# marian42/shapegan

Measured on AMD Instinct MI355X. Metric: GAN train steps/sec @32^3 voxels (train_wgan.py 5 critic + 1 generator updates, batch 64/GPU), higher is better.
Workload: dtype f32; 1 GPU; train_wgan.py 32^3 voxel WGAN, fp32, batch=64 synthetic SDF grids (BASELINE configs[1]); global_batch=64, per_gpu_batch=64, parallelism=dp1

## Files before the change

### include/shapegan_hip.h

```cpp
#ifndef SHAPEGAN_HIP_H
#define SHAPEGAN_HIP_H

#include <stddef.h>
#include <stdint.h>

#ifdef __cplusplus
extern "C" {
#endif

#define SG_ABI_VERSION 8

typedef struct ihipStream_t* hipStream_t;

#define SG_ACT_NONE_C 0
#define SG_ACT_LEAKY_C 1
#define SG_ACT_RELU_C 2
#define SG_ACT_TANH_C 3
#define SG_ACT_SIGMOID_C 4

int sg_abi_version(void);
const char* sg_last_error(void);

size_t sg_conv3d_k4s2p1_fwd_workspace_bytes(int batch, int Cin, int Cout, int OD, int OH, int OW);
int sg_conv3d_k4s2p1_fwd(const float* x, const float* w, const float* bias, float* y, int batch, int Cin, int Cin_total,
                         int Cx, int Cout, int ID, int IH, int IW, int act, float slope, void* workspace,
                         size_t workspace_bytes, hipStream_t stream);
int sg_conv3d_k4s2p1_fwd_keep(const float* x, const float* w, const float* bias, float* y, int batch, int Cin, int Cin_total,
                              int Cx, int Cout, int ID, int IH, int IW, int act, float slope, void* workspace,
                              size_t workspace_bytes, int weights_unchanged, hipStream_t stream);
long long sg_conv3d_k4s2p1_image_layout(int kind, const int* dims, size_t workspace_bytes);
int sg_conv3d_k4s2p1_pack_images(int n, const int* kinds, const float* const* weights, void* const* workspaces,
                                 const size_t* workspace_bytes, const int* dims, int* served, hipStream_t stream);
int sg_conv3d_k4s2p1_fwd_impl(const float* x, const float* w, const float* bias, float* y, int batch, int Cin,
                              int Cin_total, int Cx, int Cout, int ID, int IH, int IW, int act, float slope,
                              void* workspace, size_t workspace_bytes, int impl, int debug, hipStream_t stream);
size_t sg_conv3d_k4s2p1_dgrad_workspace_bytes(int Cout, int Cin);
size_t sg_conv3d_k4s2p1_dgrad_workspace_bytes_for(int batch, int Cin, int Cout, int OD, int OH, int OW);
int sg_conv3d_k4s2p1_dgrad(const float* dy, const float* w, const float* bias, float* dx, int batch, int Cin,
                           int Cin_total, int Cx, int Cout, int ID, int IH, int IW, int act, float slope,
                           void* workspace, size_t workspace_bytes, hipStream_t stream);
int sg_conv3d_k4s2p1_dgrad_keep(const float* dy, const float* w, const float* bias, float* dx, int batch, int Cin,
                                int Cin_total, int Cx, int Cout, int ID, int IH, int IW, int act, float slope,
                                void* workspace, size_t workspace_bytes, int weights_unchanged, hipStream_t stream);
int sg_conv3d_k4s2p1_dgrad_impl(const float* dy, const float* w, const float* bias, float* dx, int batch, int Cin,
                                int Cin_total, int Cx, int Cout, int ID, int IH, int IW, int act, float slope,
                                void* workspace, size_t workspace_bytes, int impl, hipStream_t stream);
#define SG_DGRAD_FORM_NONE 0
#define SG_DGRAD_FORM_DSKIP4 1
#define SG_DGRAD_FORM_ROWS32_4 2
#define SG_DGRAD_FORM_ROWS64_4 3
#define SG_DGRAD_FORM_ROWS32 4
#define SG_DGRAD_FORM_ROWS64 5
#define SG_DGRAD_FORM_DEPTH_WALK 6
int sg_conv3d_k4s2p1_dgrad_form(int batch, int Cin, int Cout, int OD, int OH, int OW, size_t workspace_bytes);
size_t sg_conv3d_k4s2p1_wgrad_workspace_bytes(int batch, int Cin, int Cout, int OD, int OH, int OW);
int sg_conv3d_k4s2p1_wgrad_impl(const float* dy, const float* x, float* dw, int batch, int Cin, int Cin_total, int Cx,
                                int Cout, int ID, int IH, int IW, void* workspace, size_t workspace_bytes, int impl,
                                hipStream_t stream);
int sg_conv3d_k4s2p1_wgrad(const float* dy, const float* x, float* dw, int batch, int Cin, int Cin_total, int Cx,
                           int Cout, int ID, int IH, int IW, void* workspace, size_t workspace_bytes,
                           hipStream_t stream);
int sg_conv3d_k4s2p1_wgrad_dy_image(int batch, int Cin, int Cout, int OD, int OH, int OW, size_t workspace_bytes, int* mt_total,
                                    long* nslice);
int sg_act_bwd_rowsum_pack8(const float* y, const float* dy, float* dz, float* rowsum, void* dz_image, long N, int C, long nslice,
                            int act, float slope, hipStream_t stream);
int sg_conv3d_k4s2p1_wgrad_prepacked(const float* dy, const float* x, float* dw, int batch, int Cin, int Cin_total, int Cx,
                                     int Cout, int ID, int IH, int IW, void* workspace, size_t workspace_bytes, hipStream_t stream);
int sg_conv3d_k4s2p1_wgrad_act_eligible(int batch, int Cin, int Cout, int OD, int OH, int OW, int act);
int sg_conv3d_k4s2p1_wgrad_act(const float* dy, const float* y, const float* x, float* dw, float* db, int batch, int Cin,
                               int Cin_total, int Cx, int Cout, int ID, int IH, int IW, int act, float slope, void* workspace,
                               size_t workspace_bytes, hipStream_t stream);

int sg_convT3d_k4s2p1_fwd(const float* x, const float* w, const float* bias, float* y, int batch, int Cin_T, int Cout_T,
                          int ID, int IH, int IW, int act, float slope, void* workspace, size_t workspace_bytes,
                          hipStream_t stream);
int sg_convT3d_k4s2p1_to1_pre_eligible(int batch, int C, int ID, int IH, int IW);
int sg_convT3d_k4s2p1_to1_pre(const float* x, const float* w, const float* bias, float* y, const float* in_scale,
                              const float* in_shift, int in_act, float in_slope, int batch, int C, int ID, int IH, int IW, int act,
                              float slope, hipStream_t stream);
int sg_convT3d_k4s2p1_to1_pre_impl(const float* x, const float* w, const float* bias, float* y, const float* in_scale,
                                   const float* in_shift, int in_act, float in_slope, int batch, int C, int ID, int IH, int IW,
                                   int act, float slope, int form, hipStream_t stream);
int sg_convT3d_k4s2p1_to1_pre_grouped(const float* x, const float* w, const float* bias, float* y, const float* in_scale,
                                      const float* in_shift, int in_act, float in_slope, int batch, int C, int ID, int IH, int IW,
                                      int act, float slope, int samples_per_group, long y_group_stride, hipStream_t stream);
int sg_convT3d_k4s2p1_dgrad(const float* dy, const float* w, float* dx, int batch, int Cin_T, int Cout_T, int ID, int IH,
                            int IW, void* workspace, size_t workspace_bytes, hipStream_t stream);
int sg_convT3d_k4s2p1_wgrad(const float* dy, const float* x, float* dw, int batch, int Cin_T, int Cout_T, int ID, int IH,
                            int IW, void* workspace, size_t workspace_bytes, hipStream_t stream);

size_t sg_gemm_workspace_bytes(int M, int N);
int sg_gemm(const float* A, long sai, long sak, const float* B, long sbk, long sbj, float* C, long sci, long scj,
            const float* bias_i, const float* bias_j, int bias_j_shift, int M, int N, int K, int act, float slope,
            void* workspace, size_t workspace_bytes, hipStream_t stream);
#define SG_GEMM_KIND_SKELETON 0
#define SG_GEMM_KIND_GEMM128 1
#define SG_GEMM_KIND_GEMM128_SPLIT 2
#define SG_GEMM_KIND_PERSISTENT 3
#define SG_GEMM_FINALIZE_NONE 0
#define SG_GEMM_FINALIZE_FLAT 1
#define SG_GEMM_FINALIZE_DEEP 2
int sg_gemm_plan(const void* A, long sai, long sak, const void* B, long sbk, long sbj, long sci, long scj, int has_bias_i, int M, int N,
                 int K, const void* workspace, size_t workspace_bytes, long* plan);
int sg_gemm_nt_plan(int batch, int M, int N, long K, long* plan);
size_t sg_gemm_nt_workspace_bytes(int M, int N, long K);
int sg_gemm_nt(const float* A, long lda, const float* B, long ldb, float* C, long ldc, int M, int N, long K, void* workspace,
               size_t workspace_bytes, hipStream_t stream);
size_t sg_gemm_nt_batched_workspace_bytes(int batch, int M, int N, long K);
int sg_gemm_nt_batched(const float* A, const long* a_off, long lda, const float* B, const long* b_off, long ldb, float* C,
                       const long* c_off, const long* ldc, int batch, int M, int N, long K, void* workspace,
                       size_t workspace_bytes, hipStream_t stream);
int sg_gemm_nt_batched_lnrelu(const float* A, const long* a_off, long lda, const float* B, const long* b_off, long ldb,
                              const float* gamma, const float* beta, const long* g_off, float* C, const long* c_off, const long* ldc,
                              int batch, int M, int N, long K, void* workspace, size_t workspace_bytes, hipStream_t stream);
int sg_colsum(const float* x, float* out, int rows, int cols, long ld, hipStream_t stream);
int sg_rowsum(const float* x, float* out, long rows, long len, long ld, hipStream_t stream);
int sg_rowsum_multi(const float* x, float* const* outs, const long* out_strides, int ndst, long rows_per_dst, long len, long ld,
                    hipStream_t stream);
int sg_segsum(const float* x, float* out, long rows, long ld, const int64_t* seg_off, long nseg, hipStream_t stream);

size_t sg_bn_workspace_bytes(int C);
int sg_bn_plan(int N, int C, long S, int* nsplit, int* napply);
int sg_bn_train_fwd(const float* x, const float* gamma, const float* beta, float* y, float* save_mean, float* save_invstd,
                    float* running_mean, float* running_var, long long* num_batches_tracked, int N, int C, long S,
                    float eps, float momentum, int act, float slope, void* workspace, size_t workspace_bytes,
                    hipStream_t stream);
int sg_bn_train_stats(const float* x, const float* gamma, const float* beta, float* save_mean, float* save_invstd,
                      float* running_mean, float* running_var, long long* num_batches_tracked, float* scale, float* shift, int N,
                      int C, long S, float eps, float momentum, void* workspace, size_t workspace_bytes, hipStream_t stream);
int sg_bn_train_fwd_grouped(const float* x, const float* gamma, const float* beta, float* y, float* save_mean, float* save_invstd,
                            float* running_mean, float* running_var, long long* num_batches_tracked, int groups, int N, int C,
                            long S, float eps, float momentum, int act, float slope, void* workspace, size_t workspace_bytes,
                            hipStream_t stream);
int sg_bn_train_stats_grouped(const float* x, const float* gamma, const float* beta, float* save_mean, float* save_invstd,
                              float* running_mean, float* running_var, long long* num_batches_tracked, float* scale, float* shift,
                              int groups, int N, int C, long S, float eps, float momentum, void* workspace, size_t workspace_bytes,
                              hipStream_t stream);
int sg_bn_eval_fwd(const float* x, const float* gamma, const float* beta, float* y, const float* running_mean,
                   const float* running_var, float* save_mean, float* save_invstd, int N, int C, long S, float eps,
                   int act, float slope, hipStream_t stream);
int sg_bn_bwd(const float* dy, const float* x, const float* gamma, const float* beta, const float* save_mean,
              const float* save_invstd, float* dx, float* dgamma, float* dbeta, int N, int C, long S, int train, int act,
              float slope, void* workspace, size_t workspace_bytes, hipStream_t stream);

int sg_act_fwd(const float* x, float* y, long n, int act, float slope, hipStream_t stream);
int sg_act_bwd(const float* y, const float* dy, float* dx, long n, int act, float slope, hipStream_t stream);
int sg_act_bwd_rowsum(const float* y, const float* dy, float* dx, float* rowsum, long rows, long S, int act, float slope,
                      hipStream_t stream);

size_t sg_sdfnet_packed_floats(int kin_used);
size_t sg_sdfnet_acts_floats(long ldn);
int sg_sdfnet_pack(const float* const* params, int latent, int kin_used, float* packed, hipStream_t stream);
int sg_sdfnet_fwd(const float* points, long points_period, const float* latent, const int64_t* latent_idx,
                  int latent_size, const float* packed, int kin_used, const float* zb1, const float* zb5,
                  long points_per_shape, const int* shape_index, float* out, float* acts, long ldn, long N,
                  hipStream_t stream);
long sg_sdfnet_bwd_blocks(long N);
long sg_sdfnet_bwd_tile_start(long N, long t);
#define SG_SDFNET_PARTIAL_ROW 3616
#define SG_SDFGEN_PARTIAL_ROW 7200
int sg_sdfnet_bwd(const float* dout, const float* out, const float* acts, float* dz, float* dz8, float* bias_partials,
                  const float* points, long points_period, float* dx, long dx_ld, const float* packed, int kin_used, long ldn,
                  long N, hipStream_t stream);
int sg_sdfnet_shape_bias(const float* z, long nshapes, int latent, const float* W1, const float* b1, const float* W5, const float* b5,
                         float* zb1, float* zb5, hipStream_t stream);
int sg_sdfnet_pack_shape_bias(const float* const* params, int latent, float* packed, const float* z, long nshapes, float* zb1,
                              float* zb5, hipStream_t stream);
int sg_sdfnet_shape_bias_bwd(const float* t1, const float* t5, long nshapes, const float* z, int latent, const float* W1,
                             const float* W5, float* dW1, float* dW5, float* gz, const float* reg_weight, float reg_scale,
                             hipStream_t stream);
size_t sg_sdfnet_bwd_finish_workspace_bytes(long N);
int sg_sdfnet_bwd_finish(const float* dz, const float* bias_partials, long ldn, long N, int extended, float* const* bias_grads,
                         float* w8_grad, float* b8_grad, float* w1_cols, long w1_ld, float* w5_cols, long w5_ld,
                         const int64_t* seg_off, long nseg, float* t1, float* t5, void* workspace, size_t workspace_bytes,
                         unsigned* tickets, hipStream_t stream);

#ifndef SG_SDFNET_LATENT_TILE
#define SG_SDFNET_LATENT_TILE 32
#endif
#define SG_SDFNET_LATENT_PARTIAL_ROW 513
int sg_sdfnet_latent_grad(const float* points, const float* target, const int64_t* seg_off, long nshapes, const float* zb1,
                          const float* zb5, const float* packed, float cutoff, long win_start, long win_count, const int* tiles,
                          long ntiles, float* partials, hipStream_t stream);
int sg_sdfnet_latent_reduce(const float* partials, const int64_t* tile_off, const int64_t* seg_off, long nshapes, long win_count,
                            float* t1, float* t5, float* loss, hipStream_t stream);

#define SG_SDFNET_POSE_PARTIAL_ROW 528
int sg_sdfnet_latent_pose_grad(const float* points, const float* target, const int64_t* seg_off, long nshapes, const float* zb1,
                               const float* zb5, const float* packed, const float* pose, float cutoff, long win_start,
                               long win_count, const int* tiles, long ntiles, float* partials, hipStream_t stream);
int sg_sdfnet_latent_pose_reduce(const float* partials, const int64_t* tile_off, const int64_t* seg_off, long nshapes,
                                 long win_count, float* t1, float* t5, float* loss, float* gpose, hipStream_t stream);

#define SG_SDFNET_PROJECT_TILE 32
int sg_sdfnet_project(const float* points, const int64_t* seg_off, long nshapes, const float* zb1, const float* zb5,
                      const float* packed, float level, int iterations, int rule, float max_step, const int* tiles, long ntiles,
                      float* out_points, float* value, float* grad, hipStream_t stream);

size_t sg_sdfgen_acts_floats(long ldn);
long sg_sdfgen_packed_norm_offset(int which);
int sg_sdfgen_pack(const float* const* params, const float* const* norm_params, float* packed, hipStream_t stream);
int sg_sdfgen_fwd(const float* points, const float* packed, const float* zb1, const float* zb5, long points_per_shape,
                  const int* shape_index, float eps, float* out, float* acts, long ldn, long N, hipStream_t stream);
long sg_sdfgen_bwd_blocks(long N);
int sg_sdfgen_bwd(const float* dout, const float* acts, float* dz, float* dz8, float* partials, const float* points,
                  const float* packed, long ldn, long N, hipStream_t stream);
size_t sg_sdfgen_bwd_finish_workspace_bytes(long N);
int sg_sdfgen_bwd_finish(const float* dz, const float* partials, long ldn, long N, float* const* bias_grads, float* w8_grad,
                         float* b8_grad, float* w1_cols, long w1_ld, float* w5_cols, long w5_ld, float* const* norm_grads,
                         const int64_t* seg_off, long nseg, float* t1, float* t5, void* workspace, size_t workspace_bytes,
                         unsigned* tickets, hipStream_t stream);

int sg_axpby(const float* x, const float* y, float* out, long n, float a, float b, hipStream_t stream);
size_t sg_reduce_workspace_bytes(void);
int sg_reduce_sum(const float* x, float* out, long n, float scale, void* workspace, size_t workspace_bytes,
                  hipStream_t stream);
int sg_gather_rows(const float* table, const int64_t* idx, float* out, long n, int L, hipStream_t stream);
int sg_scatter_add_rows(const float* rows, long rows_ld, const int64_t* idx, float* table_grad, long n, int L,
                        hipStream_t stream);
int sg_sdf_batch_sort_max_shapes(void);
size_t sg_sdf_batch_sort_workspace_bytes(long n, long nshapes);
int sg_sdf_batch_sort(const int64_t* indices, long n, long pointcloud_size, long nshapes, const float* points,
                      const float* sdf, float* out_points, float* out_sdf, int* out_shape, int64_t* seg_off, float* counts,
                      int* bad_index_flag, int* bad_index_device, int bad_index_value, void* workspace, size_t workspace_bytes,
// ... 304 lines not shown
```

### shapegan_amd/csrc/conv3d.hip

```cpp
#include "mfma_tile.h"
#include <stdlib.h>

#include "conv_common.h"
#include "../../include/shapegan_hip.h"

namespace sg {

struct PatchCtx {
    int base;
    int mask;
    __device__ __forceinline__ void set(const ConvGeom& g, uint32_t pos) {
        int n, od, oh, ow;
        decode_pos(g, pos, n, od, oh, ow);
        const int id0 = 2 * od - 1, ih0 = 2 * oh - 1, iw0 = 2 * ow - 1;
        base = n * g.Cx * g.ID * g.IH * g.IW + (id0 * g.IH + ih0) * g.IW + iw0;
        int m = 0;
#pragma unroll
        for (int t = 0; t < 4; ++t) {
            if ((unsigned)(id0 + t) < (unsigned)g.ID) m |= 1 << t;
            if ((unsigned)(ih0 + t) < (unsigned)g.IH) m |= 1 << (4 + t);
            if ((unsigned)(iw0 + t) < (unsigned)g.IW) m |= 1 << (8 + t);
        }
        mask = m;
    }
// ... 659 lines not shown

static bool kept_image_of_call(int kind, int batch, int Cin, int Cout, const ConvGeom& g, size_t workspace_bytes, ImageJob* image) {
    if (kind == 0) {
        const HaloFwdPlan p = halo_fwd_plan(batch, Cin, Cout, g, workspace_bytes);
        *image = p.image;
        return p.served;
    }
    const HaloDgradPlan p = halo_dgrad_plan(batch, Cin, Cout, g, workspace_bytes);
    *image = p.image;
    return p.served;
}

int sg_conv3d_k4s2p1_pack_images(int n, const int* kinds, const float* const* weights, void* const* workspaces,
                                 const size_t* workspace_bytes, const int* dims, int* served, hipStream_t stream) {
    SG_CHECK_ARG(n > 0 && n <= 8 && kinds && weights && workspaces && workspace_bytes && dims && served);
    PackJobs jobs;
    for (int i = 0; i < n; ++i) {
        const int* d = dims + 8 * i;
        const int batch = d[0], Cin = d[1], Cin_total = d[2], Cx = d[3], Cout = d[4];
        served[i] = 0;
        SG_CHECK_ARG(weights[i] && batch > 0 && Cin > 0 && Cin <= Cin_total && Cin <= Cx && Cout > 0 && (kinds[i] == 0 || kinds[i] == 1));
        ConvGeom g;
        if (make_geom(g, d[5], d[6], d[7], Cx, Cout)) SG_FAIL(SG_ERR_ARG, "sg_conv3d_k4s2p1_pack_images: bad spatial dims");
        if (check_sizes(g, batch, "sg_conv3d_k4s2p1_pack_images")) return SG_ERR_ARG;
        ImageJob image;
        if (!kept_image_of_call(kinds[i], batch, Cin, Cout, g, workspaces[i] ? workspace_bytes[i] : 0, &image)) continue;
        served[i] = jobs.add(image, weights[i], workspaces[i], Cout, Cin_total, Cin);
    }
    halo_pack_jobs_launch(jobs, stream);
    SG_CHECK_LAUNCH();
    return SG_OK;
}

long long sg_conv3d_k4s2p1_image_layout(int kind, const int* dims, size_t workspace_bytes) {
    if (!dims || (kind != 0 && kind != 1)) return 0;
    const int batch = dims[0], Cin = dims[1], Cin_total = dims[2], Cx = dims[3], Cout = dims[4];
    if (batch <= 0 || Cin <= 1 || Cin > Cin_total || Cin > Cx || Cout <= 0) return 0;
    ConvGeom g;
    if (make_geom(g, dims[5], dims[6], dims[7], Cx, Cout)) return 0;
    if ((long)batch * g.O3() >= (1L << 31) || (long)batch * g.I3() >= (1L << 31)) return 0;
    ImageJob j;
    if (!kept_image_of_call(kind, batch, Cin, Cout, g, workspace_bytes, &j)) return 0;
    unsigned long long h = 1469598103934665603ull;
    const long long f[7] = {j.kind + 1, Cout, Cin_total, Cin, j.nt, (long long)j.offset, 0x5347};
    for (long long v : f)
        for (int b = 0; b < 8; ++b) {
            h ^= (unsigned long long)(v >> (8 * b)) & 0xffull;
            h *= 1099511628211ull;
        }
    h &= 0x7fffffffffffffffull;
    return h ? (long long)h : 1;
}

int sg_conv3d_k4s2p1_dgrad_form(int batch, int Cin, int Cout, int OD, int OH, int OW, size_t workspace_bytes) {
    static_assert((int)HaloDgradKernel::dskip4 + 1 == SG_DGRAD_FORM_DSKIP4 && (int)HaloDgradKernel::rows32_4 + 1 == SG_DGRAD_FORM_ROWS32_4 &&
                  (int)HaloDgradKernel::rows64_4 + 1 == SG_DGRAD_FORM_ROWS64_4 && (int)HaloDgradKernel::rows32 + 1 == SG_DGRAD_FORM_ROWS32 &&
                  (int)HaloDgradKernel::rows64 + 1 == SG_DGRAD_FORM_ROWS64 && (int)HaloDgradKernel::rows64_dwalk + 1 == SG_DGRAD_FORM_DEPTH_WALK,
                  "SG_DGRAD_FORM_* mirror HaloDgradKernel");
    ConvGeom g;
    if (batch <= 0 || Cin <= 1 || Cout <= 0 || !query_geom(g, Cin, Cout, OD, OH, OW)) return SG_DGRAD_FORM_NONE;
    if ((long)batch * g.O3() >= (1L << 31) || (long)batch * g.I3() >= (1L << 31)) return SG_DGRAD_FORM_NONE;
    if (edge_dgrad_plan(batch, Cin, Cout, g, workspace_bytes).served) return SG_DGRAD_FORM_NONE;
    const HaloDgradPlan hp = halo_dgrad_plan(batch, Cin, Cout, g, workspace_bytes);
    return hp.served ? 1 + (int)hp.kernel : SG_DGRAD_FORM_NONE;
}

int sg_conv3d_k4s2p1_dgrad_impl(const float* dy, const float* w, const float* bias, float* dx, int batch, int Cin,
                                int Cin_total, int Cx, int Cout, int ID, int IH, int IW, int act, float slope,
                                void* workspace, size_t workspace_bytes, int impl, hipStream_t stream) {
    HaloDgradForm form;
    SG_CHECK_ARG(dy && w && dx && batch > 0 && Cin > 0 && Cin <= Cin_total && Cin <= Cx && Cout > 0 &&
                 halo_dgrad_form_decode(impl, &form) && form.forced &&
                 (form.ppw == 0 || (!form.one_parity && (form.ppw == 2 || form.ppw == 4 || form.ppw == 8))));
    ConvGeom g;
    if (make_geom(g, ID, IH, IW, Cx, Cout)) SG_FAIL(SG_ERR_ARG, "sg_conv3d_k4s2p1_dgrad_impl: bad spatial dims");
    if (check_sizes(g, batch, "sg_conv3d_k4s2p1_dgrad_impl")) return SG_ERR_ARG;
    const HaloDgradPlan hp = halo_dgrad_plan(batch, Cin, Cout, g, workspace ? workspace_bytes : 0, form);
    if (!hp.served) SG_FAIL(SG_ERR_ARG, "sg_conv3d_k4s2p1_dgrad_impl: shape not eligible for the LDS-halo kernel");
    halo_dgrad_pack(hp, w, Cin, Cin_total, Cout, workspace, stream);
    halo_dgrad_launch(hp, dy, bias, dx, batch, Cin, Cout, g, act, slope, workspace, stream);
    SG_CHECK_LAUNCH();
    return SG_OK;
}

int sg_conv3d_k4s2p1_wgrad_impl(const float* dy, const float* x, float* dw, int batch, int Cin, int Cin_total, int Cx,
                                int Cout, int ID, int IH, int IW, void* workspace, size_t workspace_bytes, int impl,
                                hipStream_t stream) {
    SG_CHECK_ARG(dy && x && dw && batch > 0 && Cin > 0 && Cin <= Cin_total && Cin <= Cx && Cout > 0 && impl == 1);
    ConvGeom g;
    if (make_geom(g, ID, IH, IW, Cx, Cout)) SG_FAIL(SG_ERR_ARG, "sg_conv3d_k4s2p1_wgrad_impl: bad spatial dims");
    if (check_sizes(g, batch, "sg_conv3d_k4s2p1_wgrad_impl")) return SG_ERR_ARG;
    const HaloWgradPlan hp = halo_wgrad_plan(batch, Cin, Cout, g, workspace ? workspace_bytes : 0, true);
    if (!hp.served) SG_FAIL(SG_ERR_ARG, "sg_conv3d_k4s2p1_wgrad_impl: shape not eligible for the LDS-halo kernel");
    halo_wgrad_pack(hp, dy, Cout, g, workspace, stream);
    halo_wgrad_launch(hp, x, dw, Cin, Cin_total, Cout, g, workspace, stream);
    SG_CHECK_LAUNCH();
    return SG_OK;
}

int sg_conv3d_k4s2p1_wgrad_dy_image(int batch, int Cin, int Cout, int OD, int OH, int OW, size_t workspace_bytes, int* mt_total,
                                    long* nslice) {
    if (batch <= 0 || Cin <= 0 || Cout <= 0 || !mt_total || !nslice) return 0;
    ConvGeom g;
    if (make_geom(g, 2 * OD, 2 * OH, 2 * OW, Cin, Cout)) return 0;
    const HaloWgradPlan hp = halo_wgrad_plan(batch, Cin, Cout, g, workspace_bytes, false);
    if (!hp.producer_image) return 0;
    *mt_total = hp.dy_image.nt;
    *nslice = hp.nslice;
    return 1;
}
int sg_act_bwd_rowsum_pack8(const float* y, const float* dy, float* dz, float* rowsum, void* dz_image, long N, int C, long nslice,
                            int act, float slope, hipStream_t stream) {
    SG_CHECK_ARG(y && dy && dz && rowsum && dz_image && N > 0 && C > 0 && C % 128 == 0 && nslice == N * 8);
    SG_CHECK_ARG(act == SG_ACT_LEAKY || act == SG_ACT_RELU);
    SG_CHECK_ARG((((uintptr_t)y | (uintptr_t)dy | (uintptr_t)dz | (uintptr_t)dz_image) & 15) == 0);
    halo_act_bwd_pack8_launch(y, dy, dz, rowsum, dz_image, N * C, C, nslice, act, slope, stream);
    SG_CHECK_LAUNCH();
    return SG_OK;
}
int sg_conv3d_k4s2p1_wgrad_prepacked(const float* dy, const float* x, float* dw, int batch, int Cin, int Cin_total, int Cx,
                                     int Cout, int ID, int IH, int IW, void* workspace, size_t workspace_bytes, hipStream_t stream) {
    SG_CHECK_ARG(dy && x && dw && batch > 0 && Cin > 0 && Cin <= Cin_total && Cin <= Cx && Cout > 0);
    ConvGeom g;
    if (make_geom(g, ID, IH, IW, Cx, Cout)) SG_FAIL(SG_ERR_ARG, "sg_conv3d_k4s2p1_wgrad_prepacked: bad spatial dims");
    if (check_sizes(g, batch, "sg_conv3d_k4s2p1_wgrad_prepacked")) return SG_ERR_ARG;
    const HaloWgradPlan hp = halo_wgrad_plan(batch, Cin, Cout, g, workspace ? workspace_bytes : 0, false);
    if (!hp.producer_image)
        SG_FAIL(SG_ERR_ARG, "sg_conv3d_k4s2p1_wgrad_prepacked: this call is not served with a producer-written image");
    halo_wgrad_launch(hp, x, dw, Cin, Cin_total, Cout, g, workspace, stream);
    SG_CHECK_LAUNCH();
    return SG_OK;
}

int sg_conv3d_k4s2p1_wgrad_act_eligible(int batch, int Cin, int Cout, int OD, int OH, int OW, int act) {
    ConvGeom g;
    return batch > 0 && act != SG_ACT_NONE && query_geom(g, 1, Cout, OD, OH, OW) &&
           edge_wgrad_plan(batch, Cin, Cout, g, kAnyWorkspace, act).served;
}
int sg_conv3d_k4s2p1_wgrad_act(const float* dy, const float* y, const float* x, float* dw, float* db, int batch, int Cin,
                               int Cin_total, int Cx, int Cout, int ID, int IH, int IW, int act, float slope, void* workspace,
                               size_t workspace_bytes, hipStream_t stream) {
    SG_CHECK_ARG(dy && y && x && dw && db && batch > 0 && Cin > 0 && Cin <= Cin_total && Cin <= Cx && Cout > 0);
    ConvGeom g;
    if (make_geom(g, ID, IH, IW, Cx, Cout)) SG_FAIL(SG_ERR_ARG, "sg_conv3d_k4s2p1_wgrad_act: spatial dims must be even and >= 2");
    if (check_sizes(g, batch, "sg_conv3d_k4s2p1_wgrad_act")) return SG_ERR_ARG;
    const EdgeWgradPlan ep = edge_wgrad_plan(batch, Cin, Cout, g, workspace ? workspace_bytes : 0, act);
    if (act == SG_ACT_NONE || !ep.served)
        SG_FAIL(SG_ERR_ARG, "sg_conv3d_k4s2p1_wgrad_act: shape not served (see sg_conv3d_k4s2p1_wgrad_act_eligible) or workspace too small");
    edge_wgrad_launch(ep, dy, y, x, dw, db, batch, Cin_total, Cout, g, slope, workspace, stream);
    SG_CHECK_LAUNCH();
    return SG_OK;
}

int sg_conv3d_k4s2p1_wgrad(const float* dy, const float* x, float* dw, int batch, int Cin, int Cin_total, int Cx,
                           int Cout, int ID, int IH, int IW, void* workspace, size_t workspace_bytes,
                           hipStream_t stream) {
    SG_CHECK_ARG(dy && x && dw && batch > 0 && Cin > 0 && Cin <= Cin_total && Cin <= Cx && Cout > 0);
    ConvGeom g;
    if (make_geom(g, ID, IH, IW, Cx, Cout)) SG_FAIL(SG_ERR_ARG, "sg_conv3d_k4s2p1_wgrad: spatial dims must be even and >= 2");
    if (check_sizes(g, batch, "sg_conv3d_k4s2p1_wgrad")) return SG_ERR_ARG;
    const long npos = (long)batch * g.O3();
    const EdgeWgradPlan ep = edge_wgrad_plan(batch, Cin, Cout, g, workspace ? workspace_bytes : 0, 0);
    if (ep.served) {
        edge_wgrad_launch(ep, dy, nullptr, x, dw, nullptr, batch, Cin_total, Cout, g, 0.f, workspace, stream);
        SG_CHECK_LAUNCH();
        return SG_OK;
    }
    const HaloWgradPlan hp = halo_wgrad_plan(batch, Cin, Cout, g, workspace ? workspace_bytes : 0, false);
    if (hp.served) {
        halo_wgrad_pack(hp, dy, Cout, g, workspace, stream);
        halo_wgrad_launch(hp, x, dw, Cin, Cin_total, Cout, g, workspace, stream);
        SG_CHECK_LAUNCH();
        return SG_OK;
    }
    WgradDyLoader la;
    la.dy = dy;
    la.O3 = (int)g.O3();
    la.Cy = Cout;
    la.dO3 = FastDiv((uint32_t)g.O3());
    WgradPatchLoader lb;
    lb.x = x;
    lb.g = g;
    WgradEpi epi{dw, (long)Cin_total * 64};
    launch_tile_gemm(la, lb, epi, Cout, Cin * 64, (int)npos, (float*)workspace, workspace ? workspace_bytes : 0, stream);
    SG_CHECK_LAUNCH();
    return SG_OK;
}

int sg_convT3d_k4s2p1_fwd(const float* x, const float* w, const float* bias, float* y, int batch, int Cin_T, int Cout_T,
                          int ID, int IH, int IW, int act, float slope, void* workspace, size_t workspace_bytes,
                          hipStream_t stream) {
    return sg_conv3d_k4s2p1_dgrad(x, w, bias, y, batch, Cout_T, Cout_T, Cout_T, Cin_T, 2 * ID, 2 * IH, 2 * IW, act,
                                  slope, workspace, workspace_bytes, stream);
}
int sg_convT3d_k4s2p1_to1_pre_eligible(int batch, int C, int ID, int IH, int IW) {
    ConvGeom g;
    return batch > 0 && C > 0 && query_geom(g, 1, C, ID, IH, IW) && (long)batch * g.I3() < (1L << 31) &&
           edge_dgrad_walk_plan(0, batch, 1, C, g).served;
}
static int convT_to1_pre(const float* x, const float* w, const float* bias, float* y, const float* in_scale,
                         const float* in_shift, int in_act, float in_slope, int batch, int C, int ID, int IH, int IW,
                         int act, float slope, int samples_per_group, long y_group_stride, int form, hipStream_t stream) {
    SG_CHECK_ARG(x && w && y && in_scale && in_shift && samples_per_group > 0 && batch % samples_per_group == 0 && form >= 0 && form <= 8);
    SG_CHECK_ARG(y_group_stride >= (long)samples_per_group * 8 * ID * IH * IW);
    if (!sg_convT3d_k4s2p1_to1_pre_eligible(batch, C, ID, IH, IW))
        SG_FAIL(SG_ERR_ARG, "sg_convT3d_k4s2p1_to1_pre: shape not served (C <= 64, IH * IW <= 256)");
    SG_CHECK_ARG(in_act == SG_ACT_NONE || in_act == SG_ACT_RELU || (in_act == SG_ACT_LEAKY && in_slope >= 0.f && in_slope <= 1.f));
    ConvGeom g;
    if (make_geom(g, 2 * ID, 2 * IH, 2 * IW, 1, C)) SG_FAIL(SG_ERR_ARG, "sg_convT3d_k4s2p1_to1_pre: bad spatial dims");
    if (form == 3 || form == 4)
        SG_FAIL(SG_ERR_ARG, "sg_convT3d_k4s2p1_to1_pre_impl: forms 3 and 4 (both h parities per workgroup) were retired");
    const EdgeDgradPlan ep = edge_dgrad_walk_plan(form, batch, 1, C, g);
    if (!ep.served) SG_FAIL(SG_ERR_ARG, "sg_convT3d_k4s2p1_to1_pre: not served");
    edge_dgrad_launch(ep, x, w, bias, y, batch, 1, C, g, act, slope, nullptr, stream, in_scale, in_shift, in_act, in_slope,
                      samples_per_group, y_group_stride);
    SG_CHECK_LAUNCH();
    return SG_OK;
}
int sg_convT3d_k4s2p1_to1_pre_grouped(const float* x, const float* w, const float* bias, float* y, const float* in_scale,
                                      const float* in_shift, int in_act, float in_slope, int batch, int C, int ID, int IH, int IW,
                                      int act, float slope, int samples_per_group, long y_group_stride, hipStream_t stream) {
    return convT_to1_pre(x, w, bias, y, in_scale, in_shift, in_act, in_slope, batch, C, ID, IH, IW, act, slope, samples_per_group,
                         y_group_stride, 0, stream);
}
int sg_convT3d_k4s2p1_to1_pre_impl(const float* x, const float* w, const float* bias, float* y, const float* in_scale,
                                   const float* in_shift, int in_act, float in_slope, int batch, int C, int ID, int IH, int IW,
                                   int act, float slope, int form, hipStream_t stream) {
    return convT_to1_pre(x, w, bias, y, in_scale, in_shift, in_act, in_slope, batch, C, ID, IH, IW, act, slope, batch,
                         (long)batch * 8 * ID * IH * IW, form, stream);
}
int sg_convT3d_k4s2p1_to1_pre(const float* x, const float* w, const float* bias, float* y, const float* in_scale,
                              const float* in_shift, int in_act, float in_slope, int batch, int C, int ID, int IH, int IW, int act,
                              float slope, hipStream_t stream) {
    return sg_convT3d_k4s2p1_to1_pre_grouped(x, w, bias, y, in_scale, in_shift, in_act, in_slope, batch, C, ID, IH, IW, act, slope,
                                             batch, (long)batch * 8 * ID * IH * IW, stream);
}
int sg_convT3d_k4s2p1_dgrad(const float* dy, const float* w, float* dx, int batch, int Cin_T, int Cout_T, int ID, int IH,
                            int IW, void* workspace, size_t workspace_bytes, hipStream_t stream) {
    return sg_conv3d_k4s2p1_fwd(dy, w, nullptr, dx, batch, Cout_T, Cout_T, Cout_T, Cin_T, 2 * ID, 2 * IH, 2 * IW,
                                SG_ACT_NONE, 0.f, workspace, workspace_bytes, stream);
}
int sg_convT3d_k4s2p1_wgrad(const float* dy, const float* x, float* dw, int batch, int Cin_T, int Cout_T, int ID, int IH,
                            int IW, void* workspace, size_t workspace_bytes, hipStream_t stream) {
    return sg_conv3d_k4s2p1_wgrad(x, dy, dw, batch, Cout_T, Cout_T, Cout_T, Cin_T, 2 * ID, 2 * IH, 2 * IW, workspace,
                                  workspace_bytes, stream);
}

}
```

### shapegan_amd/csrc/conv3d_edge.hip

```cpp
#include <stdlib.h>

#include "conv_common.h"
#include "../../include/shapegan_hip.h"

namespace sg {

struct EdgeFwdArgs {
    const float* x;
    const float* w;
    const float* bias;
    float* y;
    int OD, OH, OW, IH, IW, Cout, Cy, Cin_total;
    long x_sample;
    int tiles_per_sample, total_tiles;
    FastDiv dtps, dOW, dOH;
    int act;
    float slope;
};

__device__ __forceinline__ void buf_store4(__amdgpu_buffer_rsrc_t r, unsigned voff, unsigned soff, float x, float y, float z,
                                           float w) {
    typedef unsigned u32x4 __attribute__((ext_vector_type(4)));
    u32x4 v;
    v.x = __builtin_bit_cast(unsigned, x);
// ... 45 lines not shown
            wfr[nt][g][1] = wl[co * kWL + g * 4 + kw1];
        }
    }
    const __amdgpu_buffer_rsrc_t xres = make_rsrc(a.x - ((long)a.IH * a.IW + a.IW));
    const __amdgpu_buffer_rsrc_t yres = make_rsrc(a.y);
    const unsigned O3 = (unsigned)(a.OD * a.OH * a.OW);
    unsigned soff[16];
#pragma unroll
    for (int g = 0; g < 16; ++g) soff[g] = (unsigned)(((g >> 2) * a.IH + (g & 3)) * a.IW) * 4u;

    const int nwaves = gridDim.x * 4;
    const int per_wave = (a.total_tiles + nwaves - 1) / nwaves;
    int t = (blockIdx.x * 4 + wave) * per_wave;
    const int t_end = min(a.total_tiles, t + per_wave);
    if (t >= t_end) return;

    struct TileLane {
        unsigned o0, o1;
        bool d0, d3, h0, h3;
    };
    auto lane_offsets = [&](int tile, TileLane& L, unsigned (&yoff)[1]) __attribute__((always_inline)) {
        uint32_t n, tp, q1, ow, oh, od;
        a.dtps.divmod((uint32_t)tile, n, tp);
        const uint32_t p = tp * 32 + r;
        a.dOW.divmod(p, q1, ow);
        a.dOH.divmod(q1, od, oh);
        const unsigned base = (unsigned)((long)n * a.x_sample + ((long)(2 * od) * a.IH + 2 * oh) * a.IW + 2 * ow) * 4u;
        const bool left = ow == 0, right = (int)ow == a.OW - 1;
        L.o0 = kh2 ? (right ? kBufOutside : base + 8u) : base;
        L.o1 = kh2 ? (left ? kBufOutside : base - 4u) : base + 4u;
        L.d0 = od == 0;
        L.d3 = (int)od == a.OD - 1;
        L.h0 = oh == 0;
        L.h3 = (int)oh == a.OH - 1;
        yoff[0] = (unsigned)(((long)n * a.Cy + (lane >> 3)) * O3 + tp * 32 + 4 * (lane & 7)) * 4u;
    };
    auto load_patch = [&](const TileLane& L, float (&b0)[16], float (&b1)[16]) __attribute__((always_inline)) {
#pragma unroll
        for (int g = 0; g < 16; ++g) {
            const int kd = g >> 2, kh = g & 3;
            bool out = false;
            if (kd == 0) out = out || L.d0;
            if (kd == 3) out = out || L.d3;
            if (kh == 0) out = out || L.h0;
            if (kh == 3) out = out || L.h3;
            b0[g] = buf_load(xres, out ? kBufOutside : L.o0, soff[g]);
            b1[g] = buf_load(xres, out ? kBufOutside : L.o1, soff[g]);
        }
    };
    TileLane L;
    unsigned yoff[1];
    lane_offsets(t, L, yoff);
    float* const tw = tl[wave];
    float c0[16], c1[16];
    load_patch(L, c0, c1);

    float pv[NT][16];
    unsigned yprev = kBufOutside;
    auto epilogue_slice = [&](int sl) __attribute__((always_inline)) {
        if (sl < NT * 4) {
            const int nt = sl >> 2, c = sl & 3;
            f32x4 v = {pv[nt][4 * c], pv[nt][4 * c + 1], pv[nt][4 * c + 2], pv[nt][4 * c + 3]};
            v = v + bl[nt];
            if (ACT == 1) {
                const f32x4 sv = v * a.slope;
                v = __builtin_elementwise_max(v, sv);
            } else if (ACT == 2) {
#pragma unroll
                for (int i = 0; i < 4; ++i) v[i] = sg_apply_act(v[i], a.act, a.slope);
            }
            *reinterpret_cast<f32x4*>(tw + (nt * 32 + r) * kTL + 8 * c + 4 * kh2) = v;
        } else if (sl >= 8 && sl < 8 + NT * 4) {
            const int i = sl - 8;
            const int row = 8 * i + (lane >> 3);
            const f32x4 v = *reinterpret_cast<const f32x4*>(tw + row * kTL + 4 * (lane & 7));
            buf_store4(yres, row < a.Cout && !(SG_FWDC1_ABL & 1) ? yprev : kBufOutside, (unsigned)(8 * i) * O3 * 4u, v[0], v[1], v[2], v[3]);
        }
    };
    auto tile_mfma = [&](auto with_epilogue, const float (&c0)[16], const float (&c1)[16]) __attribute__((always_inline)) {
        f32x16 acc[NT];
#pragma unroll
        for (int nt = 0; nt < NT; ++nt)
#pragma unroll
            for (int q = 0; q < 16; ++q) acc[nt][q] = 0.f;
#pragma unroll
        for (int g = 0; g < 16; ++g) {
            if (SG_FWDC1_ABL & 2) {
#pragma unroll
                for (int nt = 0; nt < NT; ++nt) acc[nt][g] += c0[g] * wfr[nt][g][0] + c1[g] * wfr[nt][g][1];
            } else {
#pragma unroll
                for (int nt = 0; nt < NT; ++nt) acc[nt] = __builtin_amdgcn_mfma_f32_32x32x2f32(c0[g], wfr[nt][g][0], acc[nt], 0, 0, 0);
#pragma unroll
                for (int nt = 0; nt < NT; ++nt) acc[nt] = __builtin_amdgcn_mfma_f32_32x32x2f32(c1[g], wfr[nt][g][1], acc[nt], 0, 0, 0);
            }
            if (decltype(with_epilogue)::value) {
                __builtin_amdgcn_sched_barrier(0);
                epilogue_slice(g);
                __builtin_amdgcn_sched_barrier(0);
            }
        }
#pragma unroll
        for (int nt = 0; nt < NT; ++nt)
#pragma unroll
            for (int q = 0; q < 16; ++q) pv[nt][q] = acc[nt][q];
    };
    auto advance = [&](int tcur, float (&n0)[16], float (&n1)[16]) __attribute__((always_inline)) {
        TileLane Ln;
        unsigned yn[1];
        lane_offsets(tcur + 1 < t_end ? tcur + 1 : tcur, Ln, yn);
        if (tcur + 1 >= t_end || (SG_FWDC1_ABL & 4)) Ln.o0 = Ln.o1 = kBufOutside;
        load_patch(Ln, n0, n1);
        yprev = yoff[0];
        L = Ln;
        yoff[0] = yn[0];
    };
    auto tile_step = [&](int tt, auto with_epilogue, const float (&c0)[16], const float (&c1)[16], float (&n0)[16],
                         float (&n1)[16]) __attribute__((always_inline)) {
        const unsigned ydone = yprev;
        advance(tt, n0, n1);
        const unsigned ynext = yprev;
        yprev = ydone;
        __builtin_amdgcn_sched_barrier(0);
        tile_mfma(with_epilogue, c0, c1);
        yprev = ynext;
    };
    float d0[16], d1[16];
    tile_step(t, IntTag<0>(), c0, c1, d0, d1);
    for (++t; t < t_end; t += 2) {
        tile_step(t, IntTag<1>(), d0, d1, c0, c1);
        if (t + 1 < t_end) tile_step(t + 1, IntTag<1>(), c0, c1, d0, d1);
    }
#pragma unroll
    for (int sl = 0; sl < 16; ++sl) epilogue_slice(sl);
}

template <int IWT>
struct FwdLds {
    static constexpr int OWT = IWT / 2, BH = 256 / OWT, R = 2 * BH + 2, RS = IWT + 8, PLANE = R * RS, BUF = 4 * PLANE;
    static constexpr int PW = IWT / 4, PIECES = 4 * R * PW, NP = (PIECES + 255) / 256;
    static constexpr int TILE_ROWS = IWT == 32 ? 4 : 2;
};
struct EdgeFwdLdsArgs {
    const float* x;
    const float* w;
    const float* bias;
    float* y;
    int OD, OH, IH, Cout, Cy, Cin_total;
    long x_sample;
    int units, units_per_wg, blocks_per_plane;
    FastDiv dbpp, dOD;
    int act;
    float slope;
};

template <int NT, int ACT, int IWT>
__global__ void __launch_bounds__(256) conv_fwd_c1_lds_kernel(EdgeFwdLdsArgs a) {
    using G = FwdLds<IWT>;
    constexpr int kWL = 65, kTL = 36;
    __shared__ __attribute__((aligned(16))) float xs[2 * G::BUF];
    __shared__ __attribute__((aligned(16))) float tl[4][32 * kTL];
    const int tid = threadIdx.x, lane = tid & 63, wave = tid >> 6;
    const int r = lane & 31, kh2 = lane >> 5;
    int u = blockIdx.x * a.units_per_wg;
    const int u_end = min(a.units, u + a.units_per_wg);
    if (u >= u_end) return;
    const __amdgpu_buffer_rsrc_t xres = make_rsrc(a.x - ((long)a.IH * IWT + IWT));
    const __amdgpu_buffer_rsrc_t yres = make_rsrc(a.y);
    unsigned pword[G::NP];
    lds_f32x4* pdst[G::NP];
#pragma unroll
    for (int f = 0; f < G::NP; ++f) {
        const int e = tid + 256 * f;
        const int p = e / (G::R * G::PW), rem = e - p * (G::R * G::PW), rr = rem / G::PW, c4 = rem - rr * G::PW;
        const unsigned cls = e >= G::PIECES ? 16u : ((p == 0 ? 1u : 0u) | (p == 3 ? 2u : 0u) | (rr == 0 ? 4u : 0u) | (rr == G::R - 1 ? 8u : 0u));
        pword[f] = (unsigned)(((p * a.IH + rr) * IWT + 4 * c4) * 4) | (cls << 26);
        pdst[f] = (lds_f32x4*)((lds_float*)xs + (e >= G::PIECES ? 0 : p * G::PLANE + rr * G::RS + 4 + 4 * c4));
    }
    const unsigned O3 = (unsigned)(a.OD * a.OH * G::OWT);
    f32x4 sv[G::NP];
    unsigned ybase = 0;
    auto stage_issue = [&](int uu, bool real) __attribute__((always_inline)) {
        uint32_t q, ohb, n, od;
        a.dbpp.divmod((uint32_t)uu, q, ohb);
        a.dOD.divmod(q, n, od);
        const unsigned mask = 0x03ffffffu | ((16u | (od == 0 ? 1u : 0u) | ((int)od == a.OD - 1 ? 2u : 0u) | (ohb == 0 ? 4u : 0u) |
                                              ((int)ohb == a.blocks_per_plane - 1 ? 8u : 0u)) << 26);
        const unsigned sbase = (unsigned)(((long)n * a.x_sample + ((long)(2 * od) * a.IH + 2 * ohb * G::BH) * IWT) * 4);
#pragma unroll
        for (int f = 0; f < G::NP; ++f) {
            const unsigned t = pword[f] & mask;
            sv[f] = buf_load4v(xres, (!real || (t >> 26) || (SG_FWDC1_ABL & 4)) ? kBufOutside : t, sbase);
        }
    };
    stage_issue(u, true);
    {
        float* wl = xs;
        const __amdgpu_buffer_rsrc_t wres = make_rsrc(a.w);
        f32x4 wv[NT * 2];
#pragma unroll
        for (int i = 0; i < NT * 2; ++i) {
            const int e4 = tid + 256 * i, co = e4 >> 4, t4 = e4 & 15;
            wv[i] = buf_load4v(wres, co < a.Cout ? (unsigned)(((long)co * a.Cin_total * 64 + t4 * 4) * 4) : kBufOutside, 0);
        }
#pragma unroll
        for (int i = 0; i < NT * 2; ++i) {
            const int e4 = tid + 256 * i, co = e4 >> 4, t4 = e4 & 15;
#pragma unroll
            for (int j = 0; j < 4; ++j) wl[co * kWL + t4 * 4 + j] = wv[i][j];
        }
    }
    __syncthreads();
    float wfr[NT][16][2], bl[NT];
#pragma unroll
    for (int nt = 0; nt < NT; ++nt) {
        const int co = nt * 32 + r;
        bl[nt] = (a.bias && co < a.Cout) ? a.bias[co] : 0.f;
#pragma unroll
        for (int g = 0; g < 16; ++g) {
            wfr[nt][g][0] = xs[co * kWL + g * 4 + 2 * kh2];
            wfr[nt][g][1] = xs[co * kWL + g * 4 + 2 * kh2 + 1];
        }
    }
    __syncthreads();
    for (int e = tid; e < 2 * 4 * G::R * 2; e += 256) {
        const int row = e >> 1;
        xs[row * G::RS + ((e & 1) ? 4 + IWT : 3)] = 0.f;
    }
    auto stage_write = [&](int buf) __attribute__((always_inline)) {
#pragma unroll
        for (int f = 0; f < G::NP; ++f)
            if (f + 1 < G::NP || tid < G::PIECES - 256 * (G::NP - 1)) pdst[f][buf * (G::BUF / 4)] = sv[f];
    };
    auto unit_ybase = [&](int uu) __attribute__((always_inline)) {
        uint32_t q, ohb, n, od;
        a.dbpp.divmod((uint32_t)uu, q, ohb);
        a.dOD.divmod(q, n, od);
        return (unsigned)(((long)n * a.Cy * O3 + ((long)od * a.OH + ohb * G::BH) * G::OWT) * 4);
    };
    const int oh_in = IWT == 32 ? 2 * (r >> 4) : 0, ow = IWT == 32 ? (r & 15) : r;
    const lds_float* const abase = (const lds_float*)xs + (2 * wave * G::TILE_ROWS + oh_in) * G::RS + 3 + 2 * ow + 2 * kh2;
    const unsigned ylane = (unsigned)(((lane >> 3) * O3 + 64 * wave + 4 * (lane & 7)) * 4);
    float* const tw = tl[wave];

    float pv[NT][16];
    unsigned yprev = kBufOutside;
    auto epilogue_slice = [&](int sl) __attribute__((always_inline)) {
        const int nt = sl >> 3, k = sl & 7;
        if (nt >= NT) return;
        if (k < 4) {
            f32x4 v = {pv[nt][4 * k], pv[nt][4 * k + 1], pv[nt][4 * k + 2], pv[nt][4 * k + 3]};
            v = v + bl[nt];
            if (ACT == 1) {
                const f32x4 sv2 = v * a.slope;
                v = __builtin_elementwise_max(v, sv2);
            } else if (ACT == 2) {
#pragma unroll
                for (int i = 0; i < 4; ++i) v[i] = sg_apply_act(v[i], a.act, a.slope);
            }
            *reinterpret_cast<f32x4*>(tw + r * kTL + 8 * k + 4 * kh2) = v;
        } else {
            const int i = k - 4;
            const int row = nt * 32 + 8 * i + (lane >> 3);
            const f32x4 v = *reinterpret_cast<const f32x4*>(tw + (8 * i + (lane >> 3)) * kTL + 4 * (lane & 7));
            buf_store4(yres, row < a.Cout && !(SG_FWDC1_ABL & 1) ? yprev : kBufOutside, (unsigned)(nt * 32 + 8 * i) * O3 * 4u, v[0], v[1], v[2], v[3]);
        }
    };
    auto tile = [&](auto with_epilogue, int buf, int j) __attribute__((always_inline)) {
        const lds_float* ap = abase + buf * G::BUF + j * G::TILE_ROWS * G::RS;
        float ca[3], cb[3];
#pragma unroll
        for (int g = 0; g < 2; ++g) {
            ca[g] = ap[(g >> 2) * G::PLANE + (g & 3) * G::RS];
            cb[g] = ap[(g >> 2) * G::PLANE + (g & 3) * G::RS + 1];
        }
        f32x16 acc[NT];
#pragma unroll
        for (int nt = 0; nt < NT; ++nt)
#pragma unroll
            for (int q = 0; q < 16; ++q) acc[nt][q] = 0.f;
#pragma unroll
        for (int g = 0; g < 16; ++g) {
            if (g + 2 < 16) {
                ca[(g + 2) % 3] = ap[((g + 2) >> 2) * G::PLANE + ((g + 2) & 3) * G::RS];
                cb[(g + 2) % 3] = ap[((g + 2) >> 2) * G::PLANE + ((g + 2) & 3) * G::RS + 1];
            }
            __builtin_amdgcn_sched_barrier(0);
            if (SG_FWDC1_ABL & 2) {
#pragma unroll
                for (int nt = 0; nt < NT; ++nt) acc[nt][g] += ca[g % 3] * wfr[nt][g][0] + cb[g % 3] * wfr[nt][g][1];
            } else {
#pragma unroll
                for (int nt = 0; nt < NT; ++nt) acc[nt] = __builtin_amdgcn_mfma_f32_32x32x2f32(ca[g % 3], wfr[nt][g][0], acc[nt], 0, 0, 0);
#pragma unroll
                for (int nt = 0; nt < NT; ++nt) acc[nt] = __builtin_amdgcn_mfma_f32_32x32x2f32(cb[g % 3], wfr[nt][g][1], acc[nt], 0, 0, 0);
            }
            if (decltype(with_epilogue)::value) {
                __builtin_amdgcn_sched_barrier(0);
                epilogue_slice(g);
                __builtin_amdgcn_sched_barrier(0);
            }
        }
#pragma unroll
        for (int nt = 0; nt < NT; ++nt)
#pragma unroll
            for (int q = 0; q < 16; ++q) pv[nt][q] = acc[nt][q];
    };

    stage_write(0);
    __syncthreads();
    int buf = 0;
    ybase = unit_ybase(u);
    stage_issue(u + 1, u + 1 < u_end);
    tile(IntTag<0>(), buf, 0);
    yprev = ybase + ylane;
    tile(IntTag<1>(), buf, 1);
    yprev = ybase + ylane + 128u;
    stage_write(buf ^ 1);
    __syncthreads();
    for (++u; u < u_end; ++u) {
        buf ^= 1;
        ybase = unit_ybase(u);
        stage_issue(u + 1, u + 1 < u_end);
        tile(IntTag<1>(), buf, 0);
        yprev = ybase + ylane;
        tile(IntTag<1>(), buf, 1);
        yprev = ybase + ylane + 128u;
        stage_write(buf ^ 1);
        __syncthreads();
    }
#pragma unroll
    for (int sl = 0; sl < 16; ++sl) epilogue_slice(sl);
}

constexpr int kEdgePartial = 4096 + 64;
struct EdgeWgradArgs {
    const float* dy;
    const float* y;
    float slope;
    const float* x;
    float* partial;
    int OD, OH, OW, IH, IW, Cout, Cy;
    long x_sample;
    int passes_per_sample, total_passes;
    FastDiv dpps, dOW16, dOH;
};

#ifndef SG_WGRAD_C1_WAVES
#define SG_WGRAD_C1_WAVES 1
#endif
template <int MT, int FUSE>
__global__ void __launch_bounds__(256, SG_WGRAD_C1_WAVES) conv_wgrad_c1_kernel(EdgeWgradArgs a) {
    constexpr int kLd = 36;
    constexpr int kStage = MT * 32 * kLd;
    __shared__ __attribute__((aligned(16))) float lds[4 * 4096];
    const int lane = threadIdx.x & 63, wave = threadIdx.x >> 6;
    const int r = lane & 31, kh2 = lane >> 5;
    const __amdgpu_buffer_rsrc_t dres = make_rsrc(a.dy);
    const __amdgpu_buffer_rsrc_t yres = make_rsrc(FUSE ? a.y : a.dy);
    const __amdgpu_buffer_rsrc_t xres = make_rsrc(a.x - ((long)a.IH * a.IW + a.IW + 1));
    const unsigned O3 = (unsigned)(a.OD * a.OH * a.OW);
    float* stage = lds + wave * kStage;
    __shared__ float bsh[4][64];
    const int crow = lane >> 3, ccol = (lane & 7) * 4;
    unsigned tapoff[2];
#pragma unroll
    for (int nt = 0; nt < 2; ++nt) {
        const int tap = nt * 32 + r, kd = tap >> 4, kh = (tap >> 2) & 3, kw = tap & 3;
        tapoff[nt] = (unsigned)((kd * a.IH + kh) * a.IW + kw) * 4u;
    }
    const int lkh = (r >> 2) & 3, lkw = r & 3, lkd0 = r >> 4;
    const int nseg = a.OW >> 4;
    f32x16 acc[MT][2];
#pragma unroll
    for (int mt = 0; mt < MT; ++mt)
#pragma unroll
        for (int nt = 0; nt < 2; ++nt)
#pragma unroll
            for (int q = 0; q < 16; ++q) acc[mt][nt][q] = 0.f;

    const int nwaves = gridDim.x * 4;
    f32x4 cv[MT * 4];
    f32x4 yv[FUSE ? MT * 4 : 1];
    float rs[MT * 4];
#pragma unroll
    for (int i = 0; i < MT * 4; ++i) rs[i] = 0.f;
    float bv[2][16];
    unsigned xo[2], xl[2], xr[2];
    auto issue_dy = [&](int ps, bool valid) __attribute__((always_inline)) {
        uint32_t n, pp;
        a.dpps.divmod((uint32_t)(valid ? ps : 0), n, pp);
        const unsigned dbase = (unsigned)((long)n * a.Cy * O3 + pp * 32 + ccol) * 4u;
        unsigned inval = valid ? 0u : kBufOutside;
        asm volatile("" : "+v"(inval));
#pragma unroll
        for (int i = 0; i < MT * 4; ++i) {
            const int co = i * 8 + crow;
            const unsigned off = (co < a.Cout ? dbase + (unsigned)co * O3 * 4u : kBufOutside) | inval;
            cv[i] = buf_load4v(dres, off, 0);
            if (FUSE) yv[i] = buf_load4v(yres, off, 0);
        }
    };
    auto plan_x = [&](int ps, bool valid) __attribute__((always_inline)) {
        uint32_t n, pp, seg, q1, od, oh;
        a.dpps.divmod((uint32_t)ps, n, pp);
        const uint32_t p0 = pp * 32 + 16 * kh2;
        a.dOW16.divmod(p0 >> 4, q1, seg);
        a.dOH.divmod(q1, od, oh);
        const unsigned xbase = (unsigned)((long)n * a.x_sample + ((long)(2 * od) * a.IH + 2 * oh) * a.IW + 32 * seg) * 4u;
        const bool hout = !valid || (lkh == 0 && oh == 0) || (lkh == 3 && (int)oh == a.OH - 1);
#pragma unroll
        for (int nt = 0; nt < 2; ++nt) {
            const int kd = 2 * nt + lkd0;
            const bool out = hout || (kd == 0 && od == 0) || (kd == 3 && (int)od == a.OD - 1);
            xo[nt] = out ? kBufOutside : xbase + tapoff[nt];
            xl[nt] = (lkw == 0 && seg == 0) ? kBufOutside : xo[nt];
            xr[nt] = (lkw == 3 && (int)seg == nseg - 1) ? kBufOutside : xo[nt];
        }
    };
    auto load_x = [&](int j) __attribute__((always_inline)) {
#pragma unroll
        for (int nt = 0; nt < 2; ++nt) bv[nt][j] = buf_load(xres, j == 0 ? xl[nt] : (j == 15 ? xr[nt] : xo[nt]), 8u * j);
    };
    int ps = blockIdx.x * 4 + wave;
    if (ps < a.total_passes) {
        issue_dy(ps, true);
        plan_x(ps, true);
#pragma unroll
        for (int j = 0; j < 16; ++j) load_x(j);
    }
    for (; ps < a.total_passes; ps += nwaves) {
        if (FUSE) {
            const float neg = FUSE == SG_ACT_LEAKY ? a.slope : 0.f;
#pragma unroll
            for (int i = 0; i < MT * 4; ++i) {
#pragma unroll
                for (int j = 0; j < 4; ++j) cv[i][j] = yv[i][j] > 0.f ? cv[i][j] : cv[i][j] * neg;
                rs[i] += (cv[i][0] + cv[i][1]) + (cv[i][2] + cv[i][3]);
            }
        }
#pragma unroll
        for (int i = 0; i < MT * 4; ++i) *reinterpret_cast<f32x4*>(stage + (i * 8 + crow) * kLd + ccol) = cv[i];
        const bool more = ps + nwaves < a.total_passes;
        issue_dy(ps + nwaves, more);
        plan_x(more ? ps + nwaves : ps, more);
        f32x4 avc[MT], avn[MT];
#pragma unroll
        for (int mt = 0; mt < MT; ++mt) avc[mt] = *reinterpret_cast<const f32x4*>(stage + (mt * 32 + r) * kLd + 16 * kh2);
        __builtin_amdgcn_sched_barrier(0);
#pragma unroll
        for (int c = 0; c < 4; ++c) {
            if (c < 3) {
#pragma unroll
                for (int mt = 0; mt < MT; ++mt)
                    avn[mt] = *reinterpret_cast<const f32x4*>(stage + (mt * 32 + r) * kLd + 16 * kh2 + 4 * (c + 1));
            }
#pragma unroll
            for (int jj = 0; jj < 4; ++jj) {
                const int j = 4 * c + jj;
#pragma unroll
                for (int mt = 0; mt < MT; ++mt)
#pragma unroll
                    for (int nt = 0; nt < 2; ++nt)
                        acc[mt][nt] = __builtin_amdgcn_mfma_f32_32x32x2f32(avc[mt][jj], bv[nt][j], acc[mt][nt], 0, 0, 0);
                load_x(j);
            }
#pragma unroll
            for (int mt = 0; mt < MT; ++mt) avc[mt] = avn[mt];
        }
        __builtin_amdgcn_sched_barrier(0);
    }
    __syncthreads();
#pragma unroll
    for (int mt = 0; mt < MT; ++mt)
#pragma unroll
        for (int nt = 0; nt < 2; ++nt)
#pragma unroll
            for (int q = 0; q < 16; ++q) {
                const int row = mt * 32 + (q & 3) + 8 * (q >> 2) + 4 * kh2;
                lds[wave * 4096 + row * 64 + nt * 32 + r] = acc[mt][nt][q];
            }
    if (FUSE) {
#pragma unroll
        for (int i = 0; i < MT * 4; ++i) {
            float v = rs[i];
            v += __builtin_bit_cast(float, __builtin_amdgcn_update_dpp(0, __builtin_bit_cast(int, v), 0xB1, 0xf, 0xf, false));
            v += __builtin_bit_cast(float, __builtin_amdgcn_update_dpp(0, __builtin_bit_cast(int, v), 0x4E, 0xf, 0xf, false));
            v += __builtin_bit_cast(float, __builtin_amdgcn_update_dpp(0, __builtin_bit_cast(int, v), 0x141, 0xf, 0xf, false));
            if ((lane & 7) == 0) bsh[wave][i * 8 + crow] = v;
        }
    }
    __syncthreads();
    float* out = a.partial + (long)blockIdx.x * kEdgePartial;
    for (int e = threadIdx.x; e < MT * 32 * 64; e += 256)
        out[e] = (lds[e] + lds[4096 + e]) + (lds[2 * 4096 + e] + lds[3 * 4096 + e]);
    if (FUSE && threadIdx.x < MT * 32) out[4096 + threadIdx.x] = (bsh[0][threadIdx.x] + bsh[1][threadIdx.x]) + (bsh[2][threadIdx.x] + bsh[3][threadIdx.x]);
}

__global__ void __launch_bounds__(256) wgrad_c1_finalize_kernel(const float* __restrict__ partial, float* __restrict__ dw,
                                                                int nparts, int Cout, int Cin_total, float* __restrict__ db) {
    __shared__ float red[16][17];
    const int o = threadIdx.x & 15, grp = threadIdx.x >> 4;
    const int e = blockIdx.x * 16 + o;
    float s[8];
#pragma unroll
    for (int u = 0; u < 8; ++u) s[u] = 0.f;
    for (int p0 = grp; p0 < nparts; p0 += 128) {
#pragma unroll
        for (int u = 0; u < 8; ++u) {
            const int p = p0 + 16 * u;
            s[u] += p < nparts ? partial[(long)p * kEdgePartial + e] : 0.f;
        }
    }
    red[grp][o] = ((s[0] + s[1]) + (s[2] + s[3])) + ((s[4] + s[5]) + (s[6] + s[7]));
    __syncthreads();
    if (grp == 0) {
        float t = 0.f;
#pragma unroll
        for (int g2 = 0; g2 < 16; ++g2) t += red[g2][o];
        const int co = e >> 6, tap = e & 63;
        if (e >= 4096) {
            if (e - 4096 < Cout) db[e - 4096] = t;
        } else if (co < Cout) {
            dw[((long)co * Cin_total) * 64 + tap] = t;
        }
    }
}

struct TapPlaneArgs {
    const float* dy;
    const float* w;
    float* S;
    int Cout, Cy, Cin_total;
    unsigned O3;
    int tiles_per_sample, total_tiles;
    FastDiv dtps;
};

template <int NS>
__global__ void __launch_bounds__(256) tapplane_gemm_kernel(TapPlaneArgs a) {
    const int lane = threadIdx.x & 63, wave = threadIdx.x >> 6;
    const int r = lane & 31, kh2 = lane >> 5;
    float wfr[2][NS];
#pragma unroll
    for (int s = 0; s < NS; ++s) {
        const int co = 2 * s + kh2, coc = co < a.Cout ? co : a.Cout - 1;
        const float keep = co < a.Cout ? 1.f : 0.f;
#pragma unroll
        for (int nt = 0; nt < 2; ++nt) wfr[nt][s] = keep * a.w[(long)coc * a.Cin_total * 64 + nt * 32 + r];
    }
    const __amdgpu_buffer_rsrc_t dres = make_rsrc(a.dy);
    const __amdgpu_buffer_rsrc_t sres = make_rsrc(a.S);
    const int nwaves = gridDim.x * 4;
    for (int t = blockIdx.x * 4 + wave; t < a.total_tiles; t += nwaves) {
        uint32_t n, tp;
        a.dtps.divmod((uint32_t)t, n, tp);
        const unsigned doff = (unsigned)(((long)n * a.Cy + kh2) * a.O3 + tp * 32 + r) * 4u;
        float av[NS];
#pragma unroll
        for (int s = 0; s < NS; ++s) av[s] = buf_load(dres, 2 * s + kh2 < a.Cout ? doff : kBufOutside, (unsigned)(2 * s) * a.O3 * 4u);
        f32x16 acc[2];
#pragma unroll
        for (int nt = 0; nt < 2; ++nt)
#pragma unroll
            for (int q = 0; q < 16; ++q) acc[nt][q] = 0.f;
#pragma unroll
        for (int s = 0; s < NS; ++s) {
            acc[0] = __builtin_amdgcn_mfma_f32_32x32x2f32(av[s], wfr[0][s], acc[0], 0, 0, 0);
            acc[1] = __builtin_amdgcn_mfma_f32_32x32x2f32(av[s], wfr[1][s], acc[1], 0, 0, 0);
        }
        const unsigned soff = (unsigned)(((long)n * 64 + r) * a.O3 + tp * 32 + 4 * kh2) * 4u;
#pragma unroll
        for (int nt = 0; nt < 2; ++nt)
#pragma unroll
            for (int c = 0; c < 4; ++c)
                buf_store4(sres, soff, (unsigned)(nt * 32) * a.O3 * 4u + 32u * c, acc[nt][4 * c], acc[nt][4 * c + 1],
                           acc[nt][4 * c + 2], acc[nt][4 * c + 3]);
    }
}

__global__ void __launch_bounds__(256) col2im_c1_kernel(const float* __restrict__ S, const float* __restrict__ bias,
                                                        float* __restrict__ dx, ConvGeom g, long dx_sample, int total, int act,
                                                        float slope) {
    const int j = blockIdx.x * 256 + threadIdx.x;
    if (j >= total) return;
    int n, qd, qh, qw;
    decode_pos(g, (uint32_t)j, n, qd, qh, qw);
    const int OHW = g.OH * g.OW;
    const long O3 = (long)g.OD * OHW;
    const float* Sn = S + (long)n * 64 * O3;
// ... 430 lines not shown
        const __amdgpu_buffer_rsrc_t sres = make_rsrc(PRE ? a.in_scale + grow : a.w), hres = make_rsrc(PRE ? a.in_shift + grow : a.w);
        unsigned wtap[4];
#pragma unroll
        for (int set = 0; set < 4; ++set) {
            const int pd = set >> 1, ph = set & 1;
            const int kd = g2 == 0 ? (pd == 0 ? 1 : 2) : (pd == 0 ? 3 : 0);
            const int kh = khi == 0 ? (ph == 0 ? 1 : 2) : (ph == 0 ? 3 : 0);
            wtap[set] = (unsigned)(kd * 16 + kh * 4 + kw) * 4u;
        }
        const unsigned wrow = (unsigned)a.Cin_total * 256u;
#pragma unroll
        for (int s = 0; s < 16; ++s) {
            const int co = 4 * s + kq;
            const bool have = s < nks && co < a.Cout;
#pragma unroll
            for (int set = 0; set < 4; ++set) wfr[set][s] = buf_load(wres, have ? (unsigned)co * wrow + wtap[set] : kBufOutside, 0);
            if (PRE) {
                psc[s] = buf_load(sres, have ? (unsigned)co * 4u : kBufOutside, 0);
                psh[s] = buf_load(hres, have ? (unsigned)co * 4u : kBufOutside, 0);
            }
        }
    }
    const int q = tid >> 1, pw = tid & 1;
    const int qh = q / OW, qw = q - qh * OW;
    const bool gather_on = q < P2;
    const int dw = pw == 0 ? -1 : 1;
    const int kp_same = pw == 0 ? 0 : 2, kp_nb = pw == 0 ? 1 : 3;
    const bool col_nb = (unsigned)(qw + dw) < (unsigned)OW;
    const int qc = gather_on ? q : 0;
    const int qcol = col_nb ? dw : 0;
    int goff[2][4];
    float gmul[2][4];
#pragma unroll
    for (int ph = 0; ph < 2; ++ph) {
        const int dh = ph == 0 ? -1 : 1;
        const bool row_nb = (unsigned)(qh + dh) < (unsigned)OH;
        const int qrow = row_nb ? dh * OW : 0;
        const int base = ph * 16 * stride;
        goff[ph][0] = base + (0 + kp_same) * stride + convT_slot(qc);
        goff[ph][1] = base + (0 + kp_nb) * stride + convT_slot(qc + qcol);
        goff[ph][2] = base + (4 + kp_same) * stride + convT_slot(qc + qrow);
        goff[ph][3] = base + (4 + kp_nb) * stride + convT_slot(qc + qrow + qcol);
        gmul[ph][0] = 1.f;
        gmul[ph][1] = col_nb ? 1.f : 0.f;
        gmul[ph][2] = row_nb ? 1.f : 0.f;
        gmul[ph][3] = (row_nb && col_nb) ? 1.f : 0.f;
    }
    const float b0 = a.bias ? a.bias[0] : 0.f;
    const int IH = 2 * OH, IW = 2 * OW;
    const __amdgpu_buffer_rsrc_t ores = make_rsrc(a.dx + (long)(n / a.spg) * a.out_group_stride + (long)(n % a.spg) * a.dx_sample);
    const unsigned ovoff = gather_on ? (unsigned)((2 * qh) * IW + 2 * qw + pw) * 4u : kBufOutside;
    const unsigned oplane = (unsigned)(IH * IW) * 4u;
    float carry[2][2] = {{0.f, 0.f}, {0.f, 0.f}};
    float etc[2][4], etf[2][4], eval[2] = {0.f, 0.f};
    auto epi_read = [&](int p, int pd) __attribute__((always_inline)) {
        const lds_float* pb = Sl + ((p & 1) * 64 + pd * 32) * stride;
#pragma unroll
        for (int ph = 0; ph < 2; ++ph)
#pragma unroll
            for (int g = 0; g < 4; ++g) {
                etc[ph][g] = pb[goff[ph][g]];
                etf[ph][g] = pb[goff[ph][g] + 8 * stride];
            }
    };
    auto epi_sum = [&](int pd) __attribute__((always_inline)) {
#pragma unroll
        for (int ph = 0; ph < 2; ++ph)
            eval[ph] = convT_out_act<EPI>(convT_tap_sum(etc[ph], etf[ph], gmul[ph], pd, carry[pd][ph], b0), a.act, a.slope);
    };
    auto epi_store = [&](int p, int pd) __attribute__((always_inline)) {
        const bool skip = p == qs && (pd == 1 || qs > 0);
#pragma unroll
        for (int ph = 0; ph < 2; ++ph)
            __builtin_amdgcn_raw_buffer_store_b32(__builtin_bit_cast(unsigned, eval[ph]), ores, (int)(skip ? kBufOutside : ovoff),
                                                  (int)((unsigned)(2 * p - pd) * oplane + (unsigned)(ph * IW) * 4u), 0);
    };

    auto plane = [&](int qd, auto with_epi, float (&cur)[2][16], float (&nxt)[2][16]) __attribute__((always_inline)) {
        lds_float* const buf = Sl + (qd & 1) * 64 * stride;
        f32x4v c4[2][4];
#pragma unroll
        for (int t = 0; t < 2; ++t)
#pragma unroll
            for (int set = 0; set < 4; ++set) c4[t][set] = f32x4v{0.f, 0.f, 0.f, 0.f};
#pragma unroll
        for (int s = 0; s < 16; ++s) {
            if (decltype(with_epi)::value && s == 1) {
                __syncthreads();
                __builtin_amdgcn_sched_barrier(0);
            }
            load_step(qd + 1, s, nxt);
            if (decltype(with_epi)::value) {
                if (s == 1) epi_read(qd - 1, 0);
                if (s == 3) epi_sum(0);
                if (s == 5) {
                    epi_store(qd - 1, 0);
                    epi_read(qd - 1, 1);
                }
                if (s == 7) epi_sum(1);
                if (s == 9) epi_store(qd - 1, 1);
            }
#pragma unroll
            for (int t = 0; t < 2; ++t) {
                float v = cur[t][s];
                if (PRE) {
                    v = fmaf(v, psc[s], psh[s]);
                    v = fmaxf(v, v * a.in_slope);
                }
#pragma unroll
                for (int set = 0; set < 4; ++set) c4[t][set] = __builtin_amdgcn_mfma_f32_16x16x4f32(v, wfr[set][s], c4[t][set], 0, 0, 0);
            }
            __builtin_amdgcn_sched_group_barrier(0x020, 1, 0);
#pragma unroll
            for (int i = 0; i < 8; ++i) {
                __builtin_amdgcn_sched_group_barrier(0x096, SG_CONVT_ALL_ILV, 0);
                __builtin_amdgcn_sched_group_barrier(0x008, 1, 0);
            }
            __builtin_amdgcn_sched_barrier(0);
        }
        if (FULL || block_on) {
#pragma unroll
            for (int t = 0; t < 2; ++t)
#pragma unroll
                for (int set = 0; set < 4; ++set)
                    *(__attribute__((address_space(3))) f32x4v*)(buf + (set * 16 + i16) * stride + wave * 32 + t * 16 + 4 * kq) = c4[t][set];
        }
    };
    plane(qs, IntTag<0>(), A0, A1);
    int qd = qs + 1;
    for (; qd + 1 < qe; qd += 2) {
        plane(qd, IntTag<1>(), A1, A0);
        plane(qd + 1, IntTag<1>(), A0, A1);
    }
    if (qd < qe) plane(qd, IntTag<1>(), A1, A0);
    __syncthreads();
#pragma unroll
    for (int pd = 0; pd < 2; ++pd) {
        epi_read(qe - 1, pd);
        epi_sum(pd);
        epi_store(qe - 1, pd);
    }
    if (qe == OD) {
#pragma unroll
        for (int ph = 0; ph < 2; ++ph)
            convT_store_last<EPI>(carry[1][ph], b0, a.act, a.slope, ores, ovoff, OD, oplane, (unsigned)(ph * IW) * 4u);
    }
}

static bool edge_buffers_in_range(int batch, const ConvGeom& g) {
    return ((size_t)batch * g.Cx * g.I3() + (size_t)(g.IH + 1) * g.IW + 4) * 4 < (size_t)kBufRange &&
           (size_t)batch * g.Cy * g.O3() * 4 < (size_t)kBufRange;
}

EdgeFwdPlan edge_fwd_plan(int batch, int Cin, int Cout, const ConvGeom& g, int act, float slope) {
    EdgeFwdPlan p = EdgeFwdPlan();
    const long O3 = g.O3();
    if (Cin != 1 || Cout > 64 || O3 % 32 != 0) return p;
    if ((long)batch * O3 < 65536) return p;
    if (!edge_buffers_in_range(batch, g)) return p;
    p.served = true;
    p.block = 256;
    p.nt = Cout > 32 ? 2 : 1;
    p.actk = act == SG_ACT_NONE ? 0 : ((act == SG_ACT_LEAKY && slope >= 0.f && slope <= 1.f) ? 1 : 2);
    p.bh = g.IW == 32 ? 16 : 8;
    if ((g.IW == 32 || g.IW == 64) && g.OH % p.bh == 0) {
        const int units = batch * g.OD * (g.OH / p.bh);
        const int lwgs = units < 512 ? units : 512;
        p.kernel = EdgeFwdKernel::lds_staged;
        p.units_per_wg = (units + lwgs - 1) / lwgs;
        p.grid = dim3((units + p.units_per_wg - 1) / p.units_per_wg);
        return p;
    }
    const int wgs = (int)(batch * (O3 / 32) + 3) / 4;
    p.kernel = EdgeFwdKernel::gather;
    p.grid = dim3(wgs > 512 ? 512 : wgs);
    return p;
}

static EdgeFwdArgs edge_fwd_args(const float* x, const float* w, const float* bias, float* y, int batch, int Cin_total, int Cout,
                                 const ConvGeom& g, int act, float slope) {
    EdgeFwdArgs a;
    a.x = x;
    a.w = w;
    a.bias = bias;
    a.y = y;
    a.OD = g.OD;
    a.OH = g.OH;
    a.OW = g.OW;
    a.IH = g.IH;
    a.IW = g.IW;
    a.Cout = Cout;
    a.Cy = g.Cy;
    a.Cin_total = Cin_total;
    a.x_sample = (long)g.Cx * g.I3();
    a.tiles_per_sample = (int)(g.O3() / 32);
    a.total_tiles = batch * a.tiles_per_sample;
    a.dtps = FastDiv((uint32_t)a.tiles_per_sample);
    a.dOW = FastDiv((uint32_t)g.OW);
    a.dOH = FastDiv((uint32_t)g.OH);
    a.act = act;
    a.slope = slope;
    return a;
}
static EdgeFwdLdsArgs edge_fwd_lds_args(const EdgeFwdPlan& p, const float* x, const float* w, const float* bias, float* y, int batch,
                                        int Cin_total, int Cout, const ConvGeom& g, int act, float slope) {
    EdgeFwdLdsArgs l;
    l.x = x;
    l.w = w;
    l.bias = bias;
    l.y = y;
    l.OD = g.OD;
    l.OH = g.OH;
    l.IH = g.IH;
    l.Cout = Cout;
    l.Cy = g.Cy;
    l.Cin_total = Cin_total;
    l.x_sample = (long)g.Cx * g.I3();
    l.blocks_per_plane = g.OH / p.bh;
    l.units = batch * g.OD * l.blocks_per_plane;
    l.units_per_wg = p.units_per_wg;
    l.dbpp = FastDiv((uint32_t)l.blocks_per_plane);
    l.dOD = FastDiv((uint32_t)g.OD);
    l.act = act;
    l.slope = slope;
    return l;
}

typedef void (*EdgeFwdLdsFn)(EdgeFwdLdsArgs);
typedef void (*EdgeFwdFn)(EdgeFwdArgs);
template <int NT, int IWT>
static EdgeFwdLdsFn edge_fwd_lds_kernel_act(int actk) {
    if (actk == 0) return conv_fwd_c1_lds_kernel<NT, 0, IWT>;
    if (actk == 1) return conv_fwd_c1_lds_kernel<NT, 1, IWT>;
    return conv_fwd_c1_lds_kernel<NT, 2, IWT>;
}
static EdgeFwdLdsFn edge_fwd_lds_kernel(int IW, int nt, int actk) {
    if (IW == 32) return nt == 2 ? edge_fwd_lds_kernel_act<2, 32>(actk) : edge_fwd_lds_kernel_act<1, 32>(actk);
    return nt == 2 ? edge_fwd_lds_kernel_act<2, 64>(actk) : edge_fwd_lds_kernel_act<1, 64>(actk);
}
template <int NT>
static EdgeFwdFn edge_fwd_kernel_act(int actk) {
    if (actk == 0) return conv_fwd_c1_kernel<NT, 0>;
    if (actk == 1) return conv_fwd_c1_kernel<NT, 1>;
    return conv_fwd_c1_kernel<NT, 2>;
}

void edge_fwd_launch(const EdgeFwdPlan& p, const float* x, const float* w, const float* bias, float* y, int batch, int Cin_total,
                     int Cout, const ConvGeom& g, int act, float slope, hipStream_t stream) {
    if (p.kernel == EdgeFwdKernel::lds_staged)
        hipLaunchKernelGGL(edge_fwd_lds_kernel(g.IW, p.nt, p.actk), p.grid, dim3(p.block), p.lds, stream,
                           edge_fwd_lds_args(p, x, w, bias, y, batch, Cin_total, Cout, g, act, slope));
    else
        hipLaunchKernelGGL(p.nt == 2 ? edge_fwd_kernel_act<2>(p.actk) : edge_fwd_kernel_act<1>(p.actk), p.grid, dim3(p.block), p.lds,
                           stream, edge_fwd_args(x, w, bias, y, batch, Cin_total, Cout, g, act, slope));
}

EdgeWgradPlan edge_wgrad_plan(int batch, int Cin, int Cout, const ConvGeom& g, size_t workspace_bytes, int fuse_act) {
    EdgeWgradPlan p = EdgeWgradPlan();
    if (Cin != 1 || Cout > 64) return p;
    p.workspace_need = (size_t)512 * kEdgePartial * sizeof(float);
    if (g.OW % 16 != 0) return p;
    if (fuse_act != 0 && fuse_act != SG_ACT_LEAKY && fuse_act != SG_ACT_RELU) return p;
    if ((long)batch * g.O3() < 65536) return p;
    if (workspace_bytes < p.workspace_need) return p;
    if (!edge_buffers_in_range(batch, g)) return p;
    const int wgs = (int)(batch * (g.O3() / 32) + 3) / 4;
    p.served = true;
    p.grid = dim3(wgs > 512 ? 512 : wgs);
    p.block = 256;
    p.nt = Cout > 32 ? 2 : 1;
    p.fuse = fuse_act;
    return p;
}

static EdgeWgradArgs edge_wgrad_args(const float* dy, const float* y, const float* x, int batch, int Cout, const ConvGeom& g,
                                     float slope, void* workspace) {
    EdgeWgradArgs a;
    a.dy = dy;
    a.y = y;
    a.slope = slope;
    a.x = x;
    a.partial = (float*)workspace;
    a.OD = g.OD;
    a.OH = g.OH;
    a.OW = g.OW;
    a.IH = g.IH;
    a.IW = g.IW;
    a.Cout = Cout;
    a.Cy = g.Cy;
    a.x_sample = (long)g.Cx * g.I3();
    a.passes_per_sample = (int)(g.O3() / 32);
    a.total_passes = batch * a.passes_per_sample;
    a.dpps = FastDiv((uint32_t)a.passes_per_sample);
    a.dOW16 = FastDiv((uint32_t)(g.OW / 16));
    a.dOH = FastDiv((uint32_t)g.OH);
    return a;
}

typedef void (*EdgeWgradFn)(EdgeWgradArgs);
template <int MT>
static EdgeWgradFn edge_wgrad_kernel_fuse(int fuse) {
    if (fuse == SG_ACT_LEAKY) return conv_wgrad_c1_kernel<MT, SG_ACT_LEAKY>;
    if (fuse == SG_ACT_RELU) return conv_wgrad_c1_kernel<MT, SG_ACT_RELU>;
    return conv_wgrad_c1_kernel<MT, 0>;
}

void edge_wgrad_launch(const EdgeWgradPlan& p, const float* dy, const float* y, const float* x, float* dw, float* db, int batch,
                       int Cin_total, int Cout, const ConvGeom& g, float slope, void* workspace, hipStream_t stream) {
    hipLaunchKernelGGL(p.nt == 2 ? edge_wgrad_kernel_fuse<2>(p.fuse) : edge_wgrad_kernel_fuse<1>(p.fuse), p.grid, dim3(p.block), p.lds,
                       stream, edge_wgrad_args(dy, p.fuse ? y : nullptr, x, batch, Cout, g, slope, workspace));
    hipLaunchKernelGGL(wgrad_c1_finalize_kernel, dim3(p.fuse ? 260 : 256), dim3(256), 0, stream, (const float*)workspace, dw, (int)p.grid.x,
                       Cout, Cin_total, db);
}


typedef void (*ConvTWalkFn)(ConvTStreamArgs);
struct ConvTOnePair {
    static constexpr int kTapRows = 16;
    static constexpr bool kLdsAttr = false;
    template <bool ALLCH, bool PRE, bool FULL, int EPI> static ConvTWalkFn kernel() { return convT_c1_stream_kernel<ALLCH, PRE, FULL, EPI>; }
};
struct ConvTAllTaps {
    static constexpr int kTapRows = 64;
    static constexpr bool kLdsAttr = true;
    template <bool ALLCH, bool PRE, bool FULL, int EPI> static ConvTWalkFn kernel() { return convT_c1_all_kernel<ALLCH, PRE, FULL, EPI>; }
};

template <class K, bool ALLCH, bool PRE, bool FULL>
static ConvTWalkFn convT_walk_kernel_epi(int act) {
    return act == SG_ACT_TANH ? K::template kernel<ALLCH, PRE, FULL, SG_ACT_TANH>()
                              : (act == SG_ACT_NONE ? K::template kernel<ALLCH, PRE, FULL, SG_ACT_NONE>() : K::template kernel<ALLCH, PRE, FULL, -1>());
}
template <class K>
static ConvTWalkFn convT_walk_kernel(bool full, bool pre, int act) {
    if (full) return pre ? convT_walk_kernel_epi<K, true, true, true>(act) : convT_walk_kernel_epi<K, true, false, true>(act);
    return pre ? convT_walk_kernel_epi<K, false, true, false>(act) : convT_walk_kernel_epi<K, false, false, false>(act);
}

template <class K>
static void convT_walk_launch(const EdgeDgradPlan& p, const ConvTStreamArgs& f, bool pre, hipStream_t stream) {
    if (K::kLdsAttr) {
        static SgPerDeviceOnce once;
        if (once.begin()) {
            const int acts[3] = {SG_ACT_TANH, SG_ACT_NONE, SG_ACT_SIGMOID};
            for (int full = 0; full < 2; ++full)
                for (int p = 0; p < 2; ++p)
                    for (int e = 0; e < 3; ++e)
                        (void)hipFuncSetAttribute(reinterpret_cast<const void*>(convT_walk_kernel<K>(full, p, acts[e])),
                                                  hipFuncAttributeMaxDynamicSharedMemorySize, 2 * K::kTapRows * 260 * 4);
            once.end();
        }
    }
    hipLaunchKernelGGL(convT_walk_kernel<K>(f.Cout == 64 && f.P2 == 256, pre, f.act), p.grid, dim3(p.block), p.lds, stream, f);
}

struct ConvTPlan {
    bool all_taps;
    int splits;
};
static ConvTPlan convT_plan(int form, int batch, int OD) {
    const long padded = (long)(batch + 7) / 8 * 8;
    if (form >= 5 || (form == 0 && padded >= 192)) {
        int splits = form == 6 ? 1 : (form == 7 ? 2 : (form == 8 ? 4 : (padded >= 192 ? 1 : (padded >= 96 ? 2 : 4))));
        while (splits > 1 && (OD % splits != 0 || OD / splits < 2)) splits >>= 1;
        return {true, splits};
    }
    return {false, form == 2 && OD >= 4 && OD % 2 == 0 ? 2 : 1};
}

EdgeDgradPlan edge_dgrad_walk_plan(int form, int batch, int Cin, int Cout, const ConvGeom& g) {
    EdgeDgradPlan p = EdgeDgradPlan();
    if (Cin != 1 || Cout > 64 || g.OH * g.OW > 256 || (size_t)g.Cy * g.O3() * 4 >= (size_t)kBufRange) return p;
    if (form == 3 || form == 4) return p;
    const ConvTPlan walk = convT_plan(form, batch, g.OD);
    const unsigned padded = (unsigned)((batch + 7) / 8 * 8);
    const int tap_rows = walk.all_taps ? ConvTAllTaps::kTapRows : ConvTOnePair::kTapRows;
    p.served = true;
    p.kernel = walk.all_taps ? EdgeDgradKernel::walk_all_taps : EdgeDgradKernel::walk_one_pair;
    p.grid = dim3(walk.all_taps ? padded * walk.splits : padded * 4 * walk.splits);
    p.block = 512;
    p.lds = (size_t)2 * tap_rows * ((g.OH * g.OW + 31) / 32 * 32 + 4) * sizeof(float);
    p.splits = walk.splits;
    return p;
}

constexpr int kConvTWalkMinBatch = 48;

EdgeDgradPlan edge_dgrad_plan(int batch, int Cin, int Cout, const ConvGeom& g, size_t workspace_bytes) {
    EdgeDgradPlan p = EdgeDgradPlan();
    const long O3 = g.O3();
    if (Cin != 1 || Cout > 64) return p;
    if (g.OH * g.OW <= 256 && (long)batch * O3 >= 512) {
        if (batch >= kConvTWalkMinBatch) p = edge_dgrad_walk_plan(0, batch, Cin, Cout, g);
        if (!p.served && (size_t)g.Cy * O3 * 4 < (size_t)kBufRange) {
            p.served = true;
            p.kernel = EdgeDgradKernel::plane_fused;
            p.grid = dim3((unsigned)((batch + 7) / 8 * 8 * g.OD));
            p.block = 512;
            p.lds = (size_t)(2 * kFusedGroup + 64 * kFusedWStride) * sizeof(float);
        }
    }
    p.workspace_need = (size_t)batch * 64 * O3 * sizeof(float);
    if (p.served) return p;
    if (O3 % 32 != 0) return p;
    if ((long)batch * O3 < 65536) return p;
    if (workspace_bytes < p.workspace_need) return p;
    if ((size_t)batch * 64 * O3 * 4 >= (size_t)kBufRange || (size_t)batch * g.Cy * O3 * 4 >= (size_t)kBufRange) return p;
    const int wgs = (int)(batch * (O3 / 32) + 3) / 4;
    p.served = true;
    p.kernel = EdgeDgradKernel::tap_planes;
    p.grid = dim3(wgs > 1024 ? 1024 : wgs);
    p.block = 256;
    return p;
}

static ConvTStreamArgs convT_stream_args(const EdgeDgradPlan& p, const float* dy, const float* w, const float* bias, float* dx,
                                         int batch, int Cin_total, int Cout, const ConvGeom& g, int act, float slope,
                                         const float* in_scale, const float* in_shift, int in_act, float in_slope,
                                         int samples_per_group, long out_group_stride) {
    ConvTStreamArgs f;
    f.dy = dy;
    f.w = w;
    f.bias = bias;
    f.dx = dx;
    f.in_scale = in_scale;
    f.in_shift = in_shift;
    f.in_slope = in_act == SG_ACT_LEAKY ? in_slope : (in_act == SG_ACT_RELU ? 0.f : 1.f);
    f.Cout = Cout;
    f.Cy = g.Cy;
    f.Cin_total = Cin_total;
    f.OD = g.OD;
    f.OH = g.OH;
    f.OW = g.OW;
    f.P2 = g.OH * g.OW;
    f.dx_sample = (long)g.Cx * g.I3();
    f.batch = batch;
    f.act = act;
    f.slope = slope;
    f.spg = samples_per_group > 0 ? samples_per_group : batch;
    f.out_group_stride = samples_per_group > 0 ? out_group_stride : (long)batch * f.dx_sample;
    f.splits = p.splits;
    return f;
}
static ConvTFusedArgs convT_fused_args(const float* dy, const float* w, const float* bias, float* dx, int batch, int Cin_total,
                                       int Cout, const ConvGeom& g, int act, float slope) {
    ConvTFusedArgs f;
    f.dy = dy;
    f.w = w;
    f.bias = bias;
    f.dx = dx;
    f.Cout = Cout;
    f.Cy = g.Cy;
    f.Cin_total = Cin_total;
    f.OD = g.OD;
    f.OH = g.OH;
    f.OW = g.OW;
    f.P2 = g.OH * g.OW;
    f.dx_sample = (long)g.Cx * g.I3();
    f.batch = batch;
    f.act = act;
    f.slope = slope;
    return f;
}
// ... 63 lines not shown
```

### shapegan_amd/csrc/conv_common.h

```cpp
#pragma once
#include "common.h"

namespace sg {

struct FastDiv {
    uint32_t m, s, d;
    FastDiv() : m(0), s(0), d(1) {}
    explicit FastDiv(uint32_t dd) : d(dd) {
        s = 0;
        while ((1u << s) < dd) ++s;
        m = (uint32_t)((((uint64_t)1 << 32) * (((uint64_t)1 << s) - dd)) / dd + 1);
    }
    __device__ __forceinline__ uint32_t div(uint32_t n) const { return (__umulhi(n, m) + n) >> s; }
    __device__ __forceinline__ void divmod(uint32_t n, uint32_t& q, uint32_t& r) const {
        q = div(n);
        r = n - q * d;
    }
};

struct ConvGeom {
    int ID, IH, IW;
    int OD, OH, OW;
    int Cx, Cy;
    FastDiv dOW, dOH, dOD;
    long I3() const { return (long)ID * IH * IW; }
    long O3() const { return (long)OD * OH * OW; }
};

__device__ __forceinline__ void decode_pos(const ConvGeom& g, uint32_t j, int& n, int& od, int& oh, int& ow) {
    uint32_t t1, t2, t3, a, b, c;
    g.dOW.divmod(j, t1, a);
    g.dOH.divmod(t1, t2, b);
    g.dOD.divmod(t2, t3, c);
    ow = (int)a;
    oh = (int)b;
    od = (int)c;
    n = (int)t3;
}

static inline int make_geom(ConvGeom& g, int ID, int IH, int IW, int Cx, int Cy) {
    if (ID < 2 || IH < 2 || IW < 2 || (ID & 1) || (IH & 1) || (IW & 1)) return -1;
    g.ID = ID;
    g.IH = IH;
    g.IW = IW;
    g.OD = ID / 2;
    g.OH = IH / 2;
    g.OW = IW / 2;
    g.Cx = Cx;
    g.Cy = Cy;
    g.dOW = FastDiv(g.OW);
    g.dOH = FastDiv(g.OH);
    g.dOD = FastDiv(g.OD);
    return 0;
}



struct KernelPlan {
    bool served;
    dim3 grid;
    unsigned block;
    size_t lds;
    size_t workspace_need;
};
template <class T>
static inline T* workspace_at(void* workspace, size_t offset) { return reinterpret_cast<T*>(static_cast<char*>(workspace) + offset); }

struct ImageJob {
    int kind;
    int nt;
    size_t offset;
};

struct PackJob {
    const float* w;
    float4* wp;
    int kind, Cout, Cin_total, Cin, nt;
};
struct PackJobs {
    PackJob job[8];
    int n = 0;
    int add(const ImageJob& image, const float* w, void* workspace, int Cout, int Cin_total, int Cin) {
        if (n >= 8) return 0;
        job[n++] = PackJob{w, workspace_at<float4>(workspace, image.offset), image.kind, Cout, Cin_total, Cin, image.nt};
        return 1;
    }
};
int halo_pack_jobs_launch(const PackJobs& jobs, hipStream_t stream);

struct HaloFwdForm {
    bool forced;
    int variant;
    bool keep_lds;
    bool keep_rows128;
    bool dskip;
};
HaloFwdForm halo_fwd_form_decode(int debug);
struct HaloDgradForm {
    bool forced;
    bool one_parity;
    int ppw;
    bool rows64_dskip;
    bool depth_walk;
};
bool halo_dgrad_form_decode(int impl, HaloDgradForm* form);

size_t halo_fwd_workspace_bytes(int Cin, int Cout);
constexpr int kHaloFwd4MaxSplit = 8;
enum class HaloFwdKernel { halo4, halo4_dskip, rows128_w8, rows128_w4, rows64 };
struct HaloFwdPlan : KernelPlan {
    HaloFwdKernel kernel;
    ImageJob image;
    int nth, ntw;
    int csplit;
    size_t partial_offset;
};
HaloFwdPlan halo_fwd_plan(int batch, int Cin, int Cout, const ConvGeom& g, size_t workspace_bytes, HaloFwdForm form = HaloFwdForm());
void halo_fwd_pack(const HaloFwdPlan& p, const float* w, int Cin, int Cin_total, int Cout, void* workspace, hipStream_t stream);
void halo_fwd_launch(const HaloFwdPlan& p, const float* x, const float* bias, float* y, int batch, int Cin, int Cout, const ConvGeom& g,
                     int act, float slope, void* workspace, hipStream_t stream);

size_t halo_dgrad_workspace_bytes(int Cin, int Cout);
enum class HaloDgradKernel { dskip4, rows32_4, rows64_4, rows32, rows64, rows64_dwalk };
struct HaloDgradPlan : KernelPlan {
    HaloDgradKernel kernel;
    ImageJob image;
    int mtiles, ppw;
    int ntd, nth, ntw;
};
HaloDgradPlan halo_dgrad_plan(int batch, int Cin, int Cout, const ConvGeom& g, size_t workspace_bytes, HaloDgradForm form = HaloDgradForm());
void halo_dgrad_pack(const HaloDgradPlan& p, const float* w, int Cin, int Cin_total, int Cout, void* workspace, hipStream_t stream);
void halo_dgrad_launch(const HaloDgradPlan& p, const float* dy, const float* bias, float* dx, int batch, int Cin, int Cout,
                       const ConvGeom& g, int act, float slope, void* workspace, hipStream_t stream);

enum class HaloWgradKernel { halo4, rows64, rows128_skip_h, rows128 };
struct HaloWgradPlan : KernelPlan {
    HaloWgradKernel kernel;
    ImageJob dy_image;
    bool producer_image;
    int nslice, nsplit, per_split, mtiles;
    size_t partial_offset;
};
HaloWgradPlan halo_wgrad_plan(int batch, int Cin, int Cout, const ConvGeom& g, size_t workspace_bytes, bool forced);
void halo_wgrad_pack(const HaloWgradPlan& p, const float* dy, int Cout, const ConvGeom& g, void* workspace, hipStream_t stream);
void halo_wgrad_launch(const HaloWgradPlan& p, const float* x, float* dw, int Cin, int Cin_total, int Cout, const ConvGeom& g,
                       void* workspace, hipStream_t stream);
int halo_act_bwd_pack8_launch(const float* y, const float* dy, float* dz, float* rowsum, void* ap, long rows, int C, long nslice,
                              int act, float slope, hipStream_t stream);

enum class EdgeFwdKernel { lds_staged, gather };
struct EdgeFwdPlan : KernelPlan {
    EdgeFwdKernel kernel;
    int nt, actk;
    int bh, units_per_wg;
};
EdgeFwdPlan edge_fwd_plan(int batch, int Cin, int Cout, const ConvGeom& g, int act, float slope);
void edge_fwd_launch(const EdgeFwdPlan& p, const float* x, const float* w, const float* bias, float* y, int batch, int Cin_total,
                     int Cout, const ConvGeom& g, int act, float slope, hipStream_t stream);

struct EdgeWgradPlan : KernelPlan {
    int nt, fuse;
};
EdgeWgradPlan edge_wgrad_plan(int batch, int Cin, int Cout, const ConvGeom& g, size_t workspace_bytes, int fuse_act);
void edge_wgrad_launch(const EdgeWgradPlan& p, const float* dy, const float* y, const float* x, float* dw, float* db, int batch,
                       int Cin_total, int Cout, const ConvGeom& g, float slope, void* workspace, hipStream_t stream);

enum class EdgeDgradKernel { walk_one_pair, walk_all_taps, plane_fused, tap_planes };
struct EdgeDgradPlan : KernelPlan {
    EdgeDgradKernel kernel;
    int splits;
};
EdgeDgradPlan edge_dgrad_walk_plan(int form, int batch, int Cin, int Cout, const ConvGeom& g);
EdgeDgradPlan edge_dgrad_plan(int batch, int Cin, int Cout, const ConvGeom& g, size_t workspace_bytes);
void edge_dgrad_launch(const EdgeDgradPlan& p, const float* dy, const float* w, const float* bias, float* dx, int batch, int Cin_total,
                       int Cout, const ConvGeom& g, int act, float slope, void* workspace, hipStream_t stream,
                       const float* in_scale = nullptr, const float* in_shift = nullptr, int in_act = 0, float in_slope = 0.f,
                       int samples_per_group = 0, long out_group_stride = 0);

}
```

### shapegan_amd/csrc/elementwise.hip

```cpp
#include "common.h"
#include "../../include/shapegan_hip.h"

namespace sg {

static int ew_grid(long n, int per_thread) {
    long b = (n + 256L * per_thread - 1) / (256L * per_thread);
    if (b > 2048) b = 2048;
    if (b < 1) b = 1;
    return (int)b;
}

__device__ __forceinline__ float sg_clamp_keep_nan(float v, float lo, float hi) { return v < lo ? lo : (v > hi ? hi : v); }

__device__ __forceinline__ float act_grad_from_output(float y, float dy, int act, float slope) {
    switch (act) {
        case SG_ACT_LEAKY: return y > 0.f ? dy : dy * slope;
        case SG_ACT_RELU: return y > 0.f ? dy : 0.f;
        case SG_ACT_TANH: return dy * (1.f - y * y);
        case SG_ACT_SIGMOID: return dy * y * (1.f - y);
        default: return dy;
    }
}

__global__ void __launch_bounds__(256) act_bwd_rowsum_kernel(const float* __restrict__ y, const float* __restrict__ dy,
                                                             float* __restrict__ dx, float* __restrict__ rowsum, long S,
                                                             int act, float slope) {
    __shared__ float red[4];
    const long base = (long)blockIdx.x * S;
    float s = 0.f;
    if ((S & 3) == 0) {
        const float4* y4 = reinterpret_cast<const float4*>(y + base);
        const float4* g4 = reinterpret_cast<const float4*>(dy + base);
        float4* d4 = reinterpret_cast<float4*>(dx + base);
        for (long e = threadIdx.x; e < (S >> 2); e += 256) {
            const float4 a = y4[e], g = g4[e];
            float4 v;
            v.x = act_grad_from_output(a.x, g.x, act, slope);
            v.y = act_grad_from_output(a.y, g.y, act, slope);
            v.z = act_grad_from_output(a.z, g.z, act, slope);
            v.w = act_grad_from_output(a.w, g.w, act, slope);
            d4[e] = v;
            s += (v.x + v.y) + (v.z + v.w);
        }
    } else {
        for (long e = threadIdx.x; e < S; e += 256) {
            const float v = act_grad_from_output(y[base + e], dy[base + e], act, slope);
            dx[base + e] = v;
            s += v;
        }
    }
    s = sg_wave_sum(s);
    if ((threadIdx.x & 63) == 0) red[threadIdx.x >> 6] = s;
    __syncthreads();
    if (threadIdx.x == 0) rowsum[blockIdx.x] = (red[0] + red[1]) + (red[2] + red[3]);
}

__global__ void __launch_bounds__(256) act_fwd_kernel(const float* __restrict__ x, float* __restrict__ y, long n, int act,
                                                      float slope) {
    const long n4 = n >> 2;
    for (long e = (long)blockIdx.x * 256 + threadIdx.x; e < n4; e += (long)gridDim.x * 256) {
        float4 v = reinterpret_cast<const float4*>(x)[e];
        v.x = sg_apply_act(v.x, act, slope);
        v.y = sg_apply_act(v.y, act, slope);
        v.z = sg_apply_act(v.z, act, slope);
        v.w = sg_apply_act(v.w, act, slope);
        reinterpret_cast<float4*>(y)[e] = v;
    }
    for (long e = (n4 << 2) + (long)blockIdx.x * 256 + threadIdx.x; e < n; e += (long)gridDim.x * 256)
        y[e] = sg_apply_act(x[e], act, slope);
}

__global__ void __launch_bounds__(256) act_bwd_kernel(const float* __restrict__ y, const float* __restrict__ dy,
                                                      float* __restrict__ dx, long n, int act, float slope) {
    const long n4 = n >> 2;
    for (long e = (long)blockIdx.x * 256 + threadIdx.x; e < n4; e += (long)gridDim.x * 256) {
        const float4 a = reinterpret_cast<const float4*>(y)[e];
        const float4 g = reinterpret_cast<const float4*>(dy)[e];
        float4 v;
        v.x = act_grad_from_output(a.x, g.x, act, slope);
        v.y = act_grad_from_output(a.y, g.y, act, slope);
        v.z = act_grad_from_output(a.z, g.z, act, slope);
        v.w = act_grad_from_output(a.w, g.w, act, slope);
        reinterpret_cast<float4*>(dx)[e] = v;
    }
    for (long e = (n4 << 2) + (long)blockIdx.x * 256 + threadIdx.x; e < n; e += (long)gridDim.x * 256)
        dx[e] = act_grad_from_output(y[e], dy[e], act, slope);
}

__global__ void __launch_bounds__(256) rmsprop_kernel(float* __restrict__ p, const float* __restrict__ g,
                                                      float* __restrict__ sq, long n, float lr, float alpha, float eps,
                                                      float gscale, float clip) {
    for (long e = (long)blockIdx.x * 256 + threadIdx.x; e < n; e += (long)gridDim.x * 256) {
        const float gg = g[e] * gscale;
        const float s = alpha * sq[e] + (1.f - alpha) * gg * gg;
        sq[e] = s;
        float v = p[e] - lr * (gg / (sqrtf(s) + eps));
        if (clip > 0.f) v = sg_clamp_keep_nan(v, -clip, clip);
        p[e] = v;
    }
}

__global__ void __launch_bounds__(256) adam_kernel(float* __restrict__ p, const float* __restrict__ g,
                                                   float* __restrict__ m, float* __restrict__ v, long n, float lr,
                                                   float b1, float b2, float eps, float bc1, float bc2_sqrt,
                                                   float gscale, const int* __restrict__ skip) {
    if (skip && *skip) return;
    const float step = lr / bc1, c1 = 1.f - b1, c2 = 1.f - b2;
    for (long e = (long)blockIdx.x * 256 + threadIdx.x; e < n; e += (long)gridDim.x * 256) {
        const float gg = __fmul_rn(g[e], gscale);
        const float mm = __fmaf_rn(b1, m[e], __fmul_rn(c1, gg));
        const float vv = __fmaf_rn(b2, v[e], __fmul_rn(__fmul_rn(c2, gg), gg));
        m[e] = mm;
        v[e] = vv;
        const float denom = __fadd_rn(__fdiv_rn(__fsqrt_rn(vv), bc2_sqrt), eps);
        p[e] = __fsub_rn(p[e], __fmul_rn(step, __fdiv_rn(mm, denom)));
    }
}

struct AdamDevSet {
    float* p;
    const float* g;
    float* m;
    float* v;
    long n;
    float lr, b1, b2, eps, gscale;
    long long* step_dev;
    float* corr;
    unsigned nblocks;
};
__device__ __forceinline__ void adam_dev_body(const AdamDevSet& a, const unsigned bx, const unsigned nb) {
    __shared__ long long t_shared;
    if (threadIdx.x == 0) t_shared = *a.step_dev + 1;
    __syncthreads();
    const long long t = t_shared;
    double p1 = 1.0, p2 = 1.0, q1 = (double)a.b1, q2 = (double)a.b2;
    for (long long e = t; e > 0; e >>= 1) {
        if (e & 1) {
            p1 *= q1;
            p2 *= q2;
        }
        q1 *= q1;
        q2 *= q2;
    }
    const float bc1 = (float)(1.0 - p1), bc2_sqrt = (float)sqrt(1.0 - p2);
    if (threadIdx.x == 0) {
        unsigned one = 1u;
        asm volatile("" : "+v"(one) : "v"((unsigned)t));
        unsigned* master = reinterpret_cast<unsigned*>(a.corr + 2);
        const unsigned w = bx & 15u, nw = nb < 16u ? nb : 16u;
        unsigned* mine = reinterpret_cast<unsigned*>(a.corr + 32 + 32 * w);
        if (atomicAdd(mine, one) == (nb - w + 15u) / 16u - 1u) {
            *mine = 0u;
            if (atomicAdd(master, one) == nw - 1u) {
                *a.step_dev = t;
                a.corr[0] = bc1;
                a.corr[1] = bc2_sqrt;
                *master = 0u;
            }
        }
    }
    const float step = a.lr / bc1, b1 = a.b1, b2 = a.b2;
    float* __restrict__ p = a.p;
    float* __restrict__ m = a.m;
    float* __restrict__ v = a.v;
    const float* __restrict__ g = a.g;
    const float c1 = 1.f - b1, c2 = 1.f - b2;
    for (long e = (long)bx * 256 + threadIdx.x; e < a.n; e += (long)nb * 256) {
        const float gg = __fmul_rn(g[e], a.gscale);
        const float mm = __fmaf_rn(b1, m[e], __fmul_rn(c1, gg));
        const float vv = __fmaf_rn(b2, v[e], __fmul_rn(__fmul_rn(c2, gg), gg));
        m[e] = mm;
        v[e] = vv;
        const float denom = __fadd_rn(__fdiv_rn(__fsqrt_rn(vv), bc2_sqrt), a.eps);
        p[e] = __fsub_rn(p[e], __fmul_rn(step, __fdiv_rn(mm, denom)));
    }
}
__global__ void __launch_bounds__(256) adam_dev_kernel(AdamDevSet a, const int* __restrict__ skip) {
    if (skip && *skip) return;
    adam_dev_body(a, blockIdx.x, gridDim.x);
}
struct AdamDevMulti {
    AdamDevSet s[4];
};
__global__ void __launch_bounds__(256) adam_dev_multi_kernel(AdamDevMulti a, const int* __restrict__ skip) {
    if (skip && *skip) return;
    const AdamDevSet& s = a.s[blockIdx.y];
    if (blockIdx.x >= s.nblocks) return;
    adam_dev_body(s, blockIdx.x, s.nblocks);
}

__global__ void __launch_bounds__(256) clamp_kernel(float* __restrict__ p, long n, float lo, float hi) {
    for (long e = (long)blockIdx.x * 256 + threadIdx.x; e < n; e += (long)gridDim.x * 256)
        p[e] = sg_clamp_keep_nan(p[e], lo, hi);
}

struct ClampMulti {
    float* p[16];
    long n[16];
};
__global__ void __launch_bounds__(256) clamp_multi_kernel(ClampMulti t, float lo, float hi) {
    float* __restrict__ p = t.p[blockIdx.y];
    const long n = t.n[blockIdx.y];
    for (long e = (long)blockIdx.x * 256 + threadIdx.x; e < n; e += (long)gridDim.x * 256) p[e] = sg_clamp_keep_nan(p[e], lo, hi);
}

__global__ void __launch_bounds__(256) voxel_prepare_kernel(const float* __restrict__ x, float* __restrict__ out, long n,
                                                            float c, float divisor) {
    for (long e = (long)blockIdx.x * 256 + threadIdx.x; e < n; e += (long)gridDim.x * 256) {
        const float v = sg_clamp_keep_nan(x[e], -c, c);
        out[e] = divisor > 0.f ? v / divisor : v;
    }
}

__global__ void __launch_bounds__(256) axpby_kernel(const float* __restrict__ x, const float* __restrict__ y,
                                                    float* __restrict__ out, long n, float a, float b) {
    for (long e = (long)blockIdx.x * 256 + threadIdx.x; e < n; e += (long)gridDim.x * 256)
        out[e] = y ? fmaf(a, x[e], b * y[e]) : a * x[e];
}

__global__ void __launch_bounds__(256) gather_rows_kernel(const float* __restrict__ table, const int64_t* __restrict__ idx,
                                                          float* __restrict__ out, long n, int L) {
    const long total = n * L;
    for (long e = (long)blockIdx.x * 256 + threadIdx.x; e < total; e += (long)gridDim.x * 256) {
        const long i = e / L;
        const int k = (int)(e - i * L);
        out[e] = table[idx[i] * L + k];
    }
}
__global__ void __launch_bounds__(256) scatter_add_rows_kernel(const float* __restrict__ rows, long rows_ld,
                                                               const int64_t* __restrict__ idx,
                                                               float* __restrict__ table_grad, long n, int L) {
    const long total = n * L;
    for (long e = (long)blockIdx.x * 256 + threadIdx.x; e < total; e += (long)gridDim.x * 256) {
        const long i = e / L;
        const int k = (int)(e - i * L);
        atomicAdd(&table_grad[idx[i] * L + k], rows[i * rows_ld + k]);
    }
}

__global__ void __launch_bounds__(256) sum_partial_kernel(const float* __restrict__ x, double* __restrict__ partial, long n) {
    double s0 = 0, s1 = 0;
    const long stride = (long)gridDim.x * 256;
    long done = 0;
    if ((((uintptr_t)x) & 15) == 0) {
        const f32x4* x4 = reinterpret_cast<const f32x4*>(x);
        const long n4 = n >> 2;
        long e = (long)blockIdx.x * 256 + threadIdx.x;
        for (; e + 3 * stride < n4; e += 4 * stride) {
            const f32x4 v0 = __builtin_nontemporal_load(x4 + e), v1 = __builtin_nontemporal_load(x4 + e + stride);
            const f32x4 v2 = __builtin_nontemporal_load(x4 + e + 2 * stride), v3 = __builtin_nontemporal_load(x4 + e + 3 * stride);
            s0 += ((double)v0[0] + (double)v0[1]) + ((double)v0[2] + (double)v0[3]);
            s1 += ((double)v1[0] + (double)v1[1]) + ((double)v1[2] + (double)v1[3]);
            s0 += ((double)v2[0] + (double)v2[1]) + ((double)v2[2] + (double)v2[3]);
            s1 += ((double)v3[0] + (double)v3[1]) + ((double)v3[2] + (double)v3[3]);
        }
        for (; e < n4; e += stride) {
            const f32x4 v = x4[e];
            s0 += ((double)v[0] + (double)v[1]) + ((double)v[2] + (double)v[3]);
        }
        done = n4 << 2;
    }
    for (long e = done + (long)blockIdx.x * 256 + threadIdx.x; e < n; e += stride) s1 += (double)x[e];
    double s = sg_wave_sum_d(s0 + s1);
    __shared__ double red[4];
    if ((threadIdx.x & 63) == 0) red[threadIdx.x >> 6] = s;
    __syncthreads();
    if (threadIdx.x == 0) partial[blockIdx.x] = red[0] + red[1] + red[2] + red[3];
}
__global__ void __launch_bounds__(64) sum_final_kernel(const double* __restrict__ partial, float* __restrict__ out, int nb,
                                                       float scale) {
    double s = 0;
    for (int i = threadIdx.x; i < nb; i += 64) s += partial[i];
    s = sg_wave_sum_d(s);
    if (threadIdx.x == 0) out[0] = (float)(s * (double)scale);
}

}

using namespace sg;

extern "C" {

int sg_act_fwd(const float* x, float* y, long n, int act, float slope, hipStream_t stream) {
    SG_CHECK_ARG(x && y && n > 0);
    hipLaunchKernelGGL(act_fwd_kernel, dim3(ew_grid(n, 4)), dim3(256), 0, stream, x, y, n, act, slope);
    SG_CHECK_LAUNCH();
    return SG_OK;
}
int sg_act_bwd(const float* y, const float* dy, float* dx, long n, int act, float slope, hipStream_t stream) {
    SG_CHECK_ARG(y && dy && dx && n > 0);
    hipLaunchKernelGGL(act_bwd_kernel, dim3(ew_grid(n, 4)), dim3(256), 0, stream, y, dy, dx, n, act, slope);
    SG_CHECK_LAUNCH();
    return SG_OK;
}
int sg_act_bwd_rowsum(const float* y, const float* dy, float* dx, float* rowsum, long rows, long S, int act, float slope,
                      hipStream_t stream) {
    SG_CHECK_ARG(y && dy && dx && rowsum && rows > 0 && rows < (1L << 31) && S > 0);
    hipLaunchKernelGGL(act_bwd_rowsum_kernel, dim3((unsigned)rows), dim3(256), 0, stream, y, dy, dx, rowsum, S, act, slope);
    SG_CHECK_LAUNCH();
    return SG_OK;
}
int sg_rmsprop_step(float* p, const float* g, float* square_avg, long n, float lr, float alpha, float eps,
                    float grad_scale, float clip, hipStream_t stream) {
    SG_CHECK_ARG(p && g && square_avg && n > 0);
    hipLaunchKernelGGL(rmsprop_kernel, dim3(ew_grid(n, 2)), dim3(256), 0, stream, p, g, square_avg, n, lr, alpha, eps,
                       grad_scale, clip);
    SG_CHECK_LAUNCH();
    return SG_OK;
}
int sg_adam_step(float* p, const float* g, float* exp_avg, float* exp_avg_sq, long n, float lr, float beta1, float beta2,
                 float eps, long step, float grad_scale, hipStream_t stream) {
    return sg_adam_step_guarded(p, g, exp_avg, exp_avg_sq, n, lr, beta1, beta2, eps, step, grad_scale, nullptr, stream);
}
int sg_adam_step_guarded(float* p, const float* g, float* exp_avg, float* exp_avg_sq, long n, float lr, float beta1, float beta2,
                         float eps, long step, float grad_scale, const int* skip_if_nonzero, hipStream_t stream) {
    SG_CHECK_ARG(p && g && exp_avg && exp_avg_sq && n > 0 && step > 0);
    const double bc1 = 1.0 - pow((double)beta1, (double)step);
    const double bc2 = 1.0 - pow((double)beta2, (double)step);
    hipLaunchKernelGGL(adam_kernel, dim3(ew_grid(n, 2)), dim3(256), 0, stream, p, g, exp_avg, exp_avg_sq, n, lr, beta1,
                       beta2, eps, (float)bc1, (float)sqrt(bc2), grad_scale, skip_if_nonzero);
    SG_CHECK_LAUNCH();
    return SG_OK;
}
int sg_adam_step_dev(float* p, const float* g, float* exp_avg, float* exp_avg_sq, long n, float lr, float beta1, float beta2,
                     float eps, long long* step_dev, float* corr_dev, float grad_scale, hipStream_t stream) {
    return sg_adam_step_dev_guarded(p, g, exp_avg, exp_avg_sq, n, lr, beta1, beta2, eps, step_dev, corr_dev, grad_scale, nullptr,
                                    stream);
}
int sg_adam_step_dev_guarded(float* p, const float* g, float* exp_avg, float* exp_avg_sq, long n, float lr, float beta1,
                             float beta2, float eps, long long* step_dev, float* corr_dev, float grad_scale,
                             const int* skip_if_nonzero, hipStream_t stream) {
    SG_CHECK_ARG(p && g && exp_avg && exp_avg_sq && n > 0 && step_dev && corr_dev);
    AdamDevSet a{p, g, exp_avg, exp_avg_sq, n, lr, beta1, beta2, eps, grad_scale, step_dev, corr_dev, (unsigned)ew_grid(n, 2)};
    hipLaunchKernelGGL(adam_dev_kernel, dim3(a.nblocks), dim3(256), 0, stream, a, skip_if_nonzero);
    SG_CHECK_LAUNCH();
    return SG_OK;
}
int sg_adam_step_dev_multi(int nsets, float* const* p, const float* const* g, float* const* exp_avg, float* const* exp_avg_sq,
                           const long* n, const float* lr, const float* beta1, const float* beta2, const float* eps,
                           long long* const* step_dev, float* const* corr_dev, const float* grad_scale, const int* skip_if_nonzero,
                           hipStream_t stream) {
    SG_CHECK_ARG(nsets > 0 && nsets <= 4 && p && g && exp_avg && exp_avg_sq && n && lr && beta1 && beta2 && eps && step_dev && corr_dev &&
                 grad_scale);
    AdamDevMulti a;
    unsigned most = 0;
    for (int i = 0; i < 4; ++i) {
        const int k = i < nsets ? i : 0;
        SG_CHECK_ARG(p[k] && g[k] && exp_avg[k] && exp_avg_sq[k] && n[k] > 0 && step_dev[k] && corr_dev[k]);
        a.s[i] = AdamDevSet{p[k], g[k], exp_avg[k], exp_avg_sq[k], n[k], lr[k], beta1[k], beta2[k], eps[k], grad_scale[k], step_dev[k],
                            corr_dev[k], (unsigned)ew_grid(n[k], 2)};
        if (i < nsets && a.s[i].nblocks > most) most = a.s[i].nblocks;
    }
    hipLaunchKernelGGL(adam_dev_multi_kernel, dim3(most, nsets), dim3(256), 0, stream, a, skip_if_nonzero);
    SG_CHECK_LAUNCH();
    return SG_OK;
}
int sg_clamp(float* p, long n, float lo, float hi, hipStream_t stream) {
    SG_CHECK_ARG(p && n > 0);
    hipLaunchKernelGGL(clamp_kernel, dim3(ew_grid(n, 2)), dim3(256), 0, stream, p, n, lo, hi);
    SG_CHECK_LAUNCH();
    return SG_OK;
}
int sg_clamp_multi(float* const* tensors, const long* counts, int ntensors, float lo, float hi, hipStream_t stream) {
    SG_CHECK_ARG(tensors && counts && ntensors > 0);
    for (int i0 = 0; i0 < ntensors; i0 += 16) {
        ClampMulti t;
        const int m = ntensors - i0 < 16 ? ntensors - i0 : 16;
        long most = 0;
        for (int i = 0; i < 16; ++i) {
            const int k = i < m ? i0 + i : i0;
            SG_CHECK_ARG(tensors[k] != nullptr && counts[k] > 0);
            t.p[i] = tensors[k];
            t.n[i] = counts[k];
            if (i < m && counts[k] > most) most = counts[k];
        }
        hipLaunchKernelGGL(clamp_multi_kernel, dim3(ew_grid(most, 2), m), dim3(256), 0, stream, t, lo, hi);
    }
    SG_CHECK_LAUNCH();
    return SG_OK;
}
int sg_voxel_prepare(const float* x, float* out, long n, float clamp, float divisor, hipStream_t stream) {
    SG_CHECK_ARG(x && out && n > 0 && clamp >= 0.f);
    hipLaunchKernelGGL(voxel_prepare_kernel, dim3(ew_grid(n, 2)), dim3(256), 0, stream, x, out, n, clamp, divisor);
    SG_CHECK_LAUNCH();
    return SG_OK;
}
int sg_axpby(const float* x, const float* y, float* out, long n, float a, float b, hipStream_t stream) {
    SG_CHECK_ARG(x && out && n > 0);
    hipLaunchKernelGGL(axpby_kernel, dim3(ew_grid(n, 2)), dim3(256), 0, stream, x, y, out, n, a, b);
    SG_CHECK_LAUNCH();
    return SG_OK;
}
int sg_gather_rows(const float* table, const int64_t* idx, float* out, long n, int L, hipStream_t stream) {
    SG_CHECK_ARG(table && idx && out && n > 0 && L > 0);
    hipLaunchKernelGGL(gather_rows_kernel, dim3(ew_grid(n * L, 2)), dim3(256), 0, stream, table, idx, out, n, L);
    SG_CHECK_LAUNCH();
    return SG_OK;
}
int sg_scatter_add_rows(const float* rows, long rows_ld, const int64_t* idx, float* table_grad, long n, int L,
                        hipStream_t stream) {
    SG_CHECK_ARG(rows && idx && table_grad && n > 0 && L > 0 && rows_ld >= L);
    hipLaunchKernelGGL(scatter_add_rows_kernel, dim3(ew_grid(n * L, 2)), dim3(256), 0, stream, rows, rows_ld, idx,
                       table_grad, n, L);
    SG_CHECK_LAUNCH();
    return SG_OK;
}
size_t sg_reduce_workspace_bytes(void) { return 1024 * sizeof(double); }
int sg_reduce_sum(const float* x, float* out, long n, float scale, void* workspace, size_t workspace_bytes,
                  hipStream_t stream) {
    SG_CHECK_ARG(x && out && n > 0);
    if (!workspace || workspace_bytes < sg_reduce_workspace_bytes()) SG_FAIL(SG_ERR_WORKSPACE, "sg_reduce_sum: workspace too small");
    int nb = ew_grid(n, 8);
    if (nb > 1024) nb = 1024;
    hipLaunchKernelGGL(sum_partial_kernel, dim3(nb), dim3(256), 0, stream, x, (double*)workspace, n);
    hipLaunchKernelGGL(sum_final_kernel, dim3(1), dim3(64), 0, stream, (const double*)workspace, out, nb, scale);
    SG_CHECK_LAUNCH();
    return SG_OK;
}

static thread_local char g_err[512];
const char* sg_last_error(void) { return g_err; }
int sg_abi_version(void) { return SG_ABI_VERSION; }

}

char* sg_err_buf() { return g_err; }
```

### shapegan_amd/csrc_cpu/shapegan_cpu.cpp

```cpp
#include <math.h>
#include <stdint.h>
#include <stdio.h>
#include <string.h>

#include <algorithm>
#include <vector>

#include "../../include/shapegan_hip.h"

typedef void* hipStream_t_;
#define SG_OK 0
#define SG_ERR_ARG (-1)
#define SG_ERR_WORKSPACE (-3)
enum { ACT_NONE = 0, ACT_LEAKY = 1, ACT_RELU = 2, ACT_TANH = 3, ACT_SIGMOID = 4 };

static thread_local char g_err[512];
#define CPU_CHECK(cond)                                                                  \
    do {                                                                                 \
        if (!(cond)) {                                                                   \
            snprintf(g_err, sizeof(g_err), "%s: bad argument: %s", __func__, #cond);     \
            return SG_ERR_ARG;                                                           \
        }                                                                                \
    } while (0)

// ... 477 lines not shown
                                  float* shift, int groups, int N, int C, long S, float eps, float momentum, void* ws, size_t wb,
                                  void* st) {
    CPU_CHECK(groups > 0 && groups <= 64);
    for (int g = 0; g < groups; ++g) {
        const int rc = sg_bn_train_stats_cpu(x + (long)g * N * C * S, gamma, beta, save_mean + (long)g * C, save_invstd + (long)g * C,
                                             running_mean, running_var, num_batches_tracked, scale + (long)g * C,
                                             shift + (long)g * C, N, C, S, eps, momentum, ws, wb, st);
        if (rc) return rc;
    }
    return SG_OK;
}
int sg_bn_eval_fwd_cpu(const float* x, const float* gamma, const float* beta, float* y, const float* running_mean,
                       const float* running_var, float* save_mean, float* save_invstd, int N, int C, long S, float eps, int act,
                       float slope, void*) {
    CPU_CHECK(x && gamma && beta && y && running_mean && running_var && save_mean && save_invstd && N > 0 && C > 0 && S > 0);
#pragma omp parallel for schedule(static)
    for (int c = 0; c < C; ++c) {
        const float mu = running_mean[c], is = 1.f / sqrtf(running_var[c] + eps);
        save_mean[c] = mu;
        save_invstd[c] = is;
        for (int n = 0; n < N; ++n) {
            const float* p = x + ((long)n * C + c) * S;
            float* q = y + ((long)n * C + c) * S;
            for (long e = 0; e < S; ++e) q[e] = apply_act(gamma[c] * ((p[e] - mu) * is) + beta[c], act, slope);
        }
    }
    return SG_OK;
}
int sg_bn_bwd_cpu(const float* dy, const float* x, const float* gamma, const float* beta, const float* save_mean,
                  const float* save_invstd, float* dx, float* dgamma, float* dbeta, int N, int C, long S, int train, int act,
                  float slope, void*, size_t, void*) {
    CPU_CHECK(dy && x && gamma && beta && save_mean && save_invstd && dx && dgamma && dbeta && N > 0 && C > 0 && S > 0);
    const long total = (long)N * S;
    const int ns = sg_bn_nsplit(N, C, S), na = sg_bn_apply_split(N, C, S);
#pragma omp parallel for schedule(static)
    for (int c = 0; c < C; ++c) {
        const float mu = save_mean[c], is = save_invstd[c], g = gamma[c], b = beta[c];
        auto grad = [&](float xh, float d) { return act_grad_out(apply_act(fmaf(g, xh, b), act, slope), d, act, slope); };
        double t1 = 0, t2 = 0;
        for (int sp = 0; sp < ns; ++sp) {
            long beg, end;
            sg_bn_slice(total, ns, sp, &beg, &end);
            for (int lane = 0; lane < 256; ++lane) {
                float s1 = 0.f, s2 = 0.f;
                if ((S & 3) == 0 && (beg & 3) == 0) {
                    SgChanWalk w(beg + (long)lane * 4, c, C, S);
                    long e = beg + (long)lane * 4;
                    for (; e + 1024 < end; e += 2048) {
                        const long a0 = w.addr();
                        w.advance(1024);
                        const long a1 = w.addr();
                        w.advance(1024);
                        for (int j = 0; j < 4; ++j) {
                            const float xh0 = (x[a0 + j] - mu) * is, xh1 = (x[a1 + j] - mu) * is;
                            const float g0 = grad(xh0, dy[a0 + j]), g1 = grad(xh1, dy[a1 + j]);
                            s1 += g0 + g1;
                            s2 += g0 * xh0 + g1 * xh1;
                        }
                    }
                    if (e < end) {
                        const long a0 = w.addr();
                        for (int j = 0; j < 4; ++j) {
                            const float xh0 = (x[a0 + j] - mu) * is;
                            const float g0 = grad(xh0, dy[a0 + j]);
                            s1 += g0;
                            s2 += g0 * xh0;
                        }
                    }
                } else {
                    for (long e = beg + lane; e < end; e += 256) {
                        const long ad = sg_bn_chan_addr(e, c, C, S);
                        const float xh = (x[ad] - mu) * is;
                        const float gg = grad(xh, dy[ad]);
                        s1 += gg;
                        s2 += gg * xh;
                    }
                }
                t1 += s1;
                t2 += s2;
            }
        }
        dbeta[c] = (float)t1;
        dgamma[c] = (float)t2;
        const float inv_n = 1.f / ((float)N * (float)S);
        const float db = (float)t1 * inv_n, dg = (float)t2 * inv_n;
        for (int sp = 0; sp < na; ++sp) {
            long beg, end;
            sg_bn_slice(total, na, sp, &beg, &end);
            if ((S & 3) == 0 && (beg & 3) == 0) {
                for (int lane = 0; lane < 256; ++lane) {
                    SgChanWalk w(beg + (long)lane * 4, c, C, S);
                    for (long e = beg + (long)lane * 4; e < end; e += 1024) {
                        const long ad = w.addr();
                        w.advance(1024);
                        for (int j = 0; j < 4; ++j) {
                            const float xh = (x[ad + j] - mu) * is;
                            const float gg = grad(xh, dy[ad + j]);
                            dx[ad + j] = g * is * (train ? gg - db - xh * dg : gg);
                        }
                    }
                }
                continue;
            }
            for (long e = beg; e < end; ++e) {
                const long ad = sg_bn_chan_addr(e, c, C, S);
                const float xh = (x[ad] - mu) * is;
                const float gg = grad(xh, dy[ad]);
                dx[ad] = g * is * (train ? gg - db - xh * dg : gg);
            }
        }
    }
    return SG_OK;
}

int sg_act_fwd_cpu(const float* x, float* y, long n, int act, float slope, void*) {
    CPU_CHECK(x && y && n > 0);
#pragma omp parallel for schedule(static)
    for (long e = 0; e < n; ++e) y[e] = apply_act(x[e], act, slope);
    return SG_OK;
}
int sg_act_bwd_cpu(const float* y, const float* dy, float* dx, long n, int act, float slope, void*) {
    CPU_CHECK(y && dy && dx && n > 0);
#pragma omp parallel for schedule(static)
    for (long e = 0; e < n; ++e) dx[e] = act_grad_out(y[e], dy[e], act, slope);
    return SG_OK;
}
int sg_act_bwd_rowsum_cpu(const float* y, const float* dy, float* dx, float* rowsum, long rows, long S, int act, float slope, void*) {
    CPU_CHECK(y && dy && dx && rowsum && rows > 0 && S > 0);
#pragma omp parallel for schedule(static)
    for (long r = 0; r < rows; ++r) {
        double s = 0;
        for (long e = r * S; e < (r + 1) * S; ++e) {
            dx[e] = act_grad_out(y[e], dy[e], act, slope);
            s += dx[e];
        }
        rowsum[r] = (float)s;
    }
    return SG_OK;
}
int sg_conv3d_k4s2p1_wgrad_act_cpu(const float* dy, const float* y, const float* x, float* dw, float* db, int batch, int Cin,
                                   int Cin_total, int Cx, int Cout, int ID, int IH, int IW, int act, float slope, void*, size_t,
                                   void*) {
    CPU_CHECK(dy && y && x && dw && db && batch > 0 && Cout > 0 && !(ID & 1) && !(IH & 1) && !(IW & 1));
    const long O3 = (long)(ID / 2) * (IH / 2) * (IW / 2), n = (long)batch * Cout * O3;
    std::vector<float> dz((size_t)n);
    for (long e = 0; e < n; ++e) dz[e] = act_grad_out(y[e], dy[e], act, slope);
    for (int co = 0; co < Cout; ++co) {
        double t = 0;
        for (int b = 0; b < batch; ++b)
            for (long e = 0; e < O3; ++e) t += dz[((long)b * Cout + co) * O3 + e];
        db[co] = (float)t;
    }
    return sg_conv3d_k4s2p1_wgrad_cpu(dz.data(), x, dw, batch, Cin, Cin_total, Cx, Cout, ID, IH, IW, nullptr, 0, nullptr);
}
int sg_act_bwd_dy_cpu(const float* y, const float* dy, const float* ggx, float* out, long n, int act, void*) {
    CPU_CHECK(y && dy && ggx && out && n > 0 && (act == ACT_TANH || act == ACT_SIGMOID));
    for (long e = 0; e < n; ++e) out[e] = ggx[e] * dy[e] * (act == ACT_TANH ? -2.f * y[e] : 1.f - 2.f * y[e]);
    return SG_OK;
}

struct CpuSdf {
    int KU;
    const float *W1k, *W2, *W3, *W4, *W5x, *W5i, *W6, *W7, *w8, *b, *b8;
};
static CpuSdf sdf_view(const float* p, int KU) {
    CpuSdf v;
    v.KU = KU;
    v.W1k = p;
    p += 256L * KU;
    v.W2 = p; p += 65536;
    v.W3 = p; p += 65536;
    v.W4 = p; p += 65536;
    v.W5x = p; p += 65536;
    v.W5i = p; p += 256L * KU;
    v.W6 = p; p += 65536;
    v.W7 = p; p += 65536;
    v.w8 = p; p += 256;
    v.b = p; p += 7 * 256;
    v.b8 = p;
    return v;
}
int sg_sdfnet_pack_cpu(const float* const* params, int latent, int kin_used, float* packed, void*) {
    CPU_CHECK(params && packed && latent >= 0 && kin_used >= 3 && kin_used <= 3 + latent);
    const int kin = 3 + latent;
    float* p = packed;
    for (int o = 0; o < 256; ++o) memcpy(p + (long)o * kin_used, params[0] + (long)o * kin, sizeof(float) * kin_used);
    p += 256L * kin_used;
    for (int l = 1; l <= 3; ++l, p += 65536) memcpy(p, params[2 * l], sizeof(float) * 65536);
    for (int o = 0; o < 256; ++o) memcpy(p + o * 256, params[8] + (long)o * (256 + kin), sizeof(float) * 256);
    p += 65536;
    for (int o = 0; o < 256; ++o) memcpy(p + (long)o * kin_used, params[8] + (long)o * (256 + kin) + 256, sizeof(float) * kin_used);
    p += 256L * kin_used;
    for (int l = 5; l <= 6; ++l, p += 65536) memcpy(p, params[2 * l], sizeof(float) * 65536);
    memcpy(p, params[14], sizeof(float) * 256);
    p += 256;
    for (int l = 0; l < 7; ++l, p += 256) memcpy(p, params[2 * l + 1], sizeof(float) * 256);
    p[0] = params[15][0];
    return SG_OK;
}
static inline void dense(const float* W, int K, const float* in, const float* b, float* out, bool relu, bool accumulate) {
    for (int o = 0; o < 256; ++o) {
        const float* w = W + (long)o * K;
        float s = accumulate ? out[o] : (b ? b[o] : 0.f);
        for (int k = 0; k < K; ++k) s += w[k] * in[k];
        out[o] = s;
    }
    if (relu)
        for (int o = 0; o < 256; ++o) out[o] = out[o] > 0.f ? out[o] : 0.f;
}
int sg_sdfnet_fwd_cpu(const float* points, long points_period, const float* latent, const int64_t* latent_idx, int latent_size,
                      const float* packed, int kin_used, const float* zb1, const float* zb5, long points_per_shape,
                      const int* shape_index, float* out, float* acts, long ldn, long N, void*) {
    CPU_CHECK(points && packed && out && N > 0 && kin_used >= 3 && (kin_used == 3 || latent) && ((zb1 != nullptr) == (zb5 != nullptr)));
    CPU_CHECK(!zb1 || shape_index || (points_per_shape > 0 && (points_per_shape % 128 == 0 || points_per_shape >= N)));
    const CpuSdf v = sdf_view(packed, kin_used);
    const int KU = kin_used, L = latent_size;
#pragma omp parallel for schedule(static)
    for (long p = 0; p < N; ++p) {
        float xin[3 + 1024], h[256], h2[256];
        const long pi = points_period > 0 ? p % points_period : p;
        for (int c = 0; c < 3; ++c) xin[c] = points[pi * 3 + c];
        if (KU > 3) {
            const long row = latent_idx ? latent_idx[p] : p;
            for (int k = 0; k < KU - 3; ++k) xin[3 + k] = latent[row * L + k];
        }
        const long shape = zb1 ? (shape_index ? shape_index[p] : p / points_per_shape) : 0;
        auto save = [&](int layer, const float* a) {
            if (acts)
                for (int o = 0; o < 256; ++o) acts[((long)layer * 256 + o) * ldn + p] = a[o];
        };
        dense(v.W1k, KU, xin, zb1 ? zb1 + shape * 256 : v.b, h, true, false);
        save(0, h);
        dense(v.W2, 256, h, v.b + 256, h2, true, false);
        save(1, h2);
        dense(v.W3, 256, h2, v.b + 512, h, true, false);
        save(2, h);
        dense(v.W4, 256, h, v.b + 768, h2, true, false);
        save(3, h2);
        dense(v.W5x, 256, h2, zb5 ? zb5 + shape * 256 : v.b + 1024, h, false, false);
        dense(v.W5i, KU, xin, nullptr, h, true, true);
        save(4, h);
        dense(v.W6, 256, h, v.b + 1280, h2, true, false);
        save(5, h2);
        dense(v.W7, 256, h2, v.b + 1536, h, true, false);
        save(6, h);
        float s = v.b8[0];
        for (int k = 0; k < 256; ++k) s += v.w8[k] * h[k];
        out[p] = tanhf(s);
    }
    return SG_OK;
}
static inline void dense_t(const float* W, int K, const float* dz, float* dh, bool accumulate) {
    if (!accumulate)
        for (int k = 0; k < K; ++k) dh[k] = 0.f;
    for (int o = 0; o < 256; ++o) {
        const float g = dz[o];
        if (g == 0.f) continue;
        const float* w = W + (long)o * K;
        for (int k = 0; k < K; ++k) dh[k] += w[k] * g;
    }
}
static inline const float* sdf_hidden_w(const CpuSdf& v, int l) {
    const float* W[7] = {nullptr, v.W2, v.W3, v.W4, v.W5x, v.W6, v.W7};
    return W[l];
}
static float sdf_shape_point_fwd(const CpuSdf& v, const float* x, const float* zb1_row, const float* zb5_row, float (*h)[256]) {
    dense(v.W1k, 3, x, zb1_row, h[0], true, false);
    for (int l = 1; l < 7; ++l) {
        if (l == 4) {
            dense(v.W5x, 256, h[3], zb5_row, h[4], false, false);
            dense(v.W5i, 3, x, nullptr, h[4], true, true);
        } else {
            dense(sdf_hidden_w(v, l), 256, h[l - 1], v.b + 256 * l, h[l], true, false);
        }
    }
    float pre = v.b8[0];
    for (int k = 0; k < 256; ++k) pre += v.w8[k] * h[6][k];
    return pre;
}
extern "C++" {
template <class OnDz5>
static void sdf_shape_point_chain(const CpuSdf& v, const float (*h)[256], float d8, float* g, OnDz5 on_dz5) {
    float gn[256];
    for (int r = 0; r < 256; ++r) g[r] = h[6][r] > 0.f ? v.w8[r] * d8 : 0.f;
    for (int layer = 5; layer >= 0; --layer) {
        dense_t(sdf_hidden_w(v, layer + 1), 256, g, gn, false);
        for (int r = 0; r < 256; ++r) g[r] = h[layer][r] > 0.f ? gn[r] : 0.f;
        if (layer == 4) on_dz5(g);
    }
}
template <class OnDz5>
static void sdf_shape_point_grad(const CpuSdf& v, const float (*h)[256], float d8, float* g, float* gp, OnDz5 on_dz5) {
    sdf_shape_point_chain(v, h, d8, g, [&](const float* dz5) {
        on_dz5(dz5);
        dense_t(v.W5i, 3, dz5, gp, false);
    });
    dense_t(v.W1k, 3, g, gp, true);
}
}
static void sdf_bwd_plan(long N, long& nbig, long& nsmall) {
    const long tiles = (N + 63) / 64, rem = tiles % 512, full = tiles - rem;
    if (rem > 256 && rem <= 384) {
        nbig = full + 256;
        nsmall = (N - nbig * 64 + 31) / 32;
    } else if (full == 0 || rem == 0 || rem > 384) {
        nbig = tiles;
// ... 2815 lines not shown
```

### shapegan_amd/ops.py

```python
import contextlib
import ctypes
import weakref

import numpy as np
import torch
from torch.autograd import Function
from torch.autograd.function import once_differentiable

from . import lib as L
from .lib import ACT_LEAKY, ACT_NONE, ACT_RELU, ACT_SIGMOID, ACT_TANH, check, f32c, ptr, stream, workspace


def _lib():
    return L.load()


def conv_fwd_raw(x, w, bias, act=ACT_NONE, slope=0.0, keep=False):
    N, Cx, D, H, W = x.shape
    Co, Ct = w.shape[0], w.shape[1]
    if Cx > Ct:
        raise RuntimeError("conv: input has %d channels, weight expects %d" % (Cx, Ct))
    ptr(x)
    L.reset_call_state()
    y = torch.empty((N, Co, D // 2, H // 2, W // 2), dtype=torch.float32, device=x.device)
    lib = _lib()
    nb = lib.sg_conv3d_k4s2p1_fwd_workspace_bytes(N, Cx, Co, D // 2, H // 2, W // 2)
    if keep and Cx > 1 and x.is_cuda and L.writers_known(w) and not torch.cuda.is_current_stream_capturing():
        ws, unchanged = _KEPT.get(w, nb, (N, Cx, Ct, Cx, Co, D, H, W), kind=0)
        check(lib.sg_conv3d_k4s2p1_fwd_keep(ptr(x), ptr(w), ptr(bias), ptr(y), N, Cx, Ct, Cx, Co, D, H, W, act, slope, ptr(ws),
                                            ws.numel(), int(unchanged), stream()), "conv3d_fwd_keep")
        return y
    ws = workspace("splitk", nb, x.device) if nb else None
    check(lib.sg_conv3d_k4s2p1_fwd(ptr(x), ptr(w), ptr(bias), ptr(y), N, Cx, Ct, Cx, Co, D, H, W, act, slope, ptr(ws),
                                   ws.numel() if ws is not None else 0, stream()), "conv3d_fwd")
    return y


def conv_fwd_impl_raw(x, w, bias, act, slope, impl, debug=0):
    N, Cx, D, H, W = x.shape
    Co, Ct = w.shape[0], w.shape[1]
    y = torch.empty((N, Co, D // 2, H // 2, W // 2), dtype=torch.float32, device=x.device)
    lib = _lib()
    nb = max(lib.sg_conv3d_k4s2p1_fwd_workspace_bytes(N, Cx, Co, D // 2, H // 2, W // 2), 1 << 20)
    ws = workspace("splitk", nb, x.device)
    check(lib.sg_conv3d_k4s2p1_fwd_impl(ptr(x), ptr(w), ptr(bias), ptr(y), N, Cx, Ct, Cx, Co, D, H, W, act, slope,
                                        ptr(ws), ws.numel(), impl, debug, stream()), "conv3d_fwd_impl")
    return y


class _KeptWeightImages(object):

    def __init__(self, cap=64):
        self.cap, self.entries, self.groups, self.layouts = cap, {}, {}, {}

    def _key(self, w, kind, dims, nbytes):
        if w.device.type != "cuda":
            return dims
        q = (kind, dims, int(nbytes))
        key = self.layouts.get(q)
        if key is None:
            if len(self.layouts) > 4096:
                self.layouts.clear()
            layout = _lib().sg_conv3d_k4s2p1_image_layout(kind, (ctypes.c_int * 8)(*[int(d) for d in dims]), int(nbytes))
            key = self.layouts[q] = ("layout", layout) if layout else dims
        return key

    def _ident(self, w, kind):
        return (w.device.index, stream(), w.data_ptr(), kind)

    def _state(self, w, shape_key):
        return (w._version, L.param_epoch_of(w), shape_key)

    def get(self, w, nbytes, shape_key, kind=1):
        ident = self._ident(w, kind)
        ent = self.entries.pop(ident, None)
        if ent is None or ent[0].numel() < nbytes or ent[2]() is not w:
            ent = [torch.empty(max(int(nbytes), 256), dtype=torch.uint8, device=w.device), None, weakref.ref(w), None]
        state = self._state(w, self._key(w, kind, shape_key, ent[0].numel()))
        unchanged = ent[1] == state
        if not unchanged:
            unchanged = self._pack_group(w, kind, ent, shape_key)
        ent[1], ent[3] = state, shape_key
        self.entries[ident] = ent
        while len(self.entries) > self.cap:
            self.entries.pop(next(iter(self.entries)))
        return ent[0], unchanged

    def _pack_group(self, w, kind, ent, shape_key):
        group = self.groups.get(id(w))
        if group is None or group[1]() is not w:
            return False
        jobs = [(w, kind, ent, shape_key)]
        for ref in group[0]:
            v = ref()
            if v is None or v.device != w.device:
                continue
            for k2 in (0, 1):
                if v is w and k2 == kind:
                    continue
                e2 = self.entries.get(self._ident(v, k2))
                if e2 is None or e2[2]() is not v or e2[1] is None:
                    continue
                if e2[1] != self._state(v, e2[1][2]):
                    jobs.append((v, k2, e2, e2[3]))
        if len(jobs) < 2:
            return False
        jobs = jobs[:8]
        n = len(jobs)
        kinds = (ctypes.c_int * n)(*[j[1] for j in jobs])
        wptr = (ctypes.c_void_p * n)(*[j[0].data_ptr() for j in jobs])
        wsp = (ctypes.c_void_p * n)(*[j[2][0].data_ptr() for j in jobs])
        wsb = (ctypes.c_size_t * n)(*[j[2][0].numel() for j in jobs])
        dims = (ctypes.c_int * (8 * n))(*[int(d) for j in jobs for d in j[3]])
        served = (ctypes.c_int * n)()
        L.note_device(w)
        check(_lib().sg_conv3d_k4s2p1_pack_images(n, kinds, wptr, wsp, wsb, dims, served, stream()), "conv3d_pack_images")
        for j, ok in zip(jobs[1:], list(served)[1:]):
            j[2][1] = self._state(j[0], self._key(j[0], j[1], j[3], j[2][0].numel())) if ok else None
        return bool(served[0])

    def register_group(self, weights):
        refs = [weakref.ref(w) for w in weights]
        for w in weights:
            self.groups[id(w)] = (refs, weakref.ref(w))


_KEPT = _KeptWeightImages()


def invalidate_weight_images():
    L.bump_param_epoch()


def register_pack_group(weights):
    _KEPT.register_group(list(weights))


def conv_dgrad_raw(dy, w, bias, cin, act=ACT_NONE, slope=0.0, keep=False, out=None):
    N, Co, OD, OH, OW = dy.shape
    Ct = w.shape[1]
    if w.shape[0] != Co or cin > Ct:
        raise RuntimeError("conv dgrad: shape mismatch")
    shape = (N, cin, 2 * OD, 2 * OH, 2 * OW)
    if out is not None:
        if tuple(out.shape) != shape or out.dtype != torch.float32 or not out.is_contiguous() or out.device != dy.device:
            raise RuntimeError("conv dgrad: `out` must be a contiguous fp32 tensor of shape %s on %s" % (shape, dy.device))
        dx = out
    else:
        dx = torch.empty(shape, dtype=torch.float32, device=dy.device)
    lib = _lib()
    nb = lib.sg_conv3d_k4s2p1_dgrad_workspace_bytes_for(N, cin, Co, OD, OH, OW)
    if keep and cin > 1 and dy.is_cuda and L.writers_known(w) and not torch.cuda.is_current_stream_capturing():
        ws, unchanged = _KEPT.get(w, nb, (N, cin, Ct, cin, Co, 2 * OD, 2 * OH, 2 * OW), kind=1)
        check(lib.sg_conv3d_k4s2p1_dgrad_keep(ptr(dy), ptr(w), ptr(bias), ptr(dx), N, cin, Ct, cin, Co, 2 * OD, 2 * OH, 2 * OW,
                                              act, slope, ptr(ws), ws.numel(), int(unchanged), stream()), "conv3d_dgrad_keep")
        return dx
    ws = workspace("dgrad", nb, dy.device)
    check(lib.sg_conv3d_k4s2p1_dgrad(ptr(dy), ptr(w), ptr(bias), ptr(dx), N, cin, Ct, cin, Co, 2 * OD, 2 * OH, 2 * OW,
                                     act, slope, ptr(ws), ws.numel(), stream()), "conv3d_dgrad")
    return dx


def conv_dgrad_halo_raw(dy, w, bias, cin, act=ACT_NONE, slope=0.0, impl=1):
    N, Co, OD, OH, OW = dy.shape
    Ct = w.shape[1]
    dx = torch.empty((N, cin, 2 * OD, 2 * OH, 2 * OW), dtype=torch.float32, device=dy.device)
    lib = _lib()
    ws = workspace("dgrad", lib.sg_conv3d_k4s2p1_dgrad_workspace_bytes(Co, cin), dy.device)
    check(lib.sg_conv3d_k4s2p1_dgrad_impl(ptr(dy), ptr(w), ptr(bias), ptr(dx), N, cin, Ct, cin, Co, 2 * OD, 2 * OH,
                                          2 * OW, act, slope, ptr(ws), ws.numel(), impl, stream()), "conv3d_dgrad_impl")
    return dx


def conv_dgrad_form(batch, cin, cout, ogrid):
    lib = L._load_hip()
    nb = lib.sg_conv3d_k4s2p1_dgrad_workspace_bytes_for(batch, cin, cout, *ogrid)
    return lib.sg_conv3d_k4s2p1_dgrad_form(batch, cin, cout, *ogrid, nb)


_WGRAD_WS_CAP = 256 << 20


def _param_grad_out(param, shape, device):
    dst = L.grad_destination(param, shape) if param is not None else None
    return dst if dst is not None else torch.empty(shape, dtype=torch.float32, device=device)


def conv_wgrad_raw(dy, x, ct, out=None):
    N, Co, OD, OH, OW = dy.shape
    Cx = x.shape[1]
    if x.shape[0] != N or x.shape[2] != 2 * OD:
        raise RuntimeError("conv wgrad: shape mismatch")
    if out is not None:
        dw = out
        if Cx < ct:
            dw.zero_()
    elif Cx < ct:
        dw = torch.zeros((Co, ct, 4, 4, 4), dtype=torch.float32, device=dy.device)
    else:
        dw = torch.empty((Co, ct, 4, 4, 4), dtype=torch.float32, device=dy.device)
    lib = _lib()
    nb = min(lib.sg_conv3d_k4s2p1_wgrad_workspace_bytes(N, Cx, Co, OD, OH, OW), _WGRAD_WS_CAP)
    ws = workspace("splitk", nb, dy.device)
    check(lib.sg_conv3d_k4s2p1_wgrad(ptr(dy), ptr(x), ptr(dw), N, Cx, ct, Cx, Co, 2 * OD, 2 * OH, 2 * OW, ptr(ws),
                                     ws.numel(), stream()), "conv3d_wgrad")
    return dw


def _wgrad_dy_image(N, Cx, Co, O, device):
    if device.type != "cuda":
        return None
    lib = _lib()
    nb = min(lib.sg_conv3d_k4s2p1_wgrad_workspace_bytes(N, Cx, Co, O, O, O), _WGRAD_WS_CAP)
    ws = workspace("splitk", nb, device)
    mt, ns = ctypes.c_int(0), ctypes.c_long(0)
    if not lib.sg_conv3d_k4s2p1_wgrad_dy_image(N, Cx, Co, O, O, O, ws.numel(), ctypes.byref(mt), ctypes.byref(ns)):
        return None
    return ws, mt.value, ns.value


def conv_wgrad_prepacked_raw(dy, x, ct, ws, out=None):
    N, Co = dy.shape[0], dy.shape[1]
    Cx = x.shape[1]
    dw = out if out is not None else torch.empty((Co, ct, 4, 4, 4), dtype=torch.float32, device=dy.device)
    if Cx < ct:
        raise RuntimeError("conv_wgrad_prepacked: partial input channels are not served")
    check(_lib().sg_conv3d_k4s2p1_wgrad_prepacked(ptr(dy), ptr(x), ptr(dw), N, Cx, ct, Cx, Co, x.shape[2], x.shape[3], x.shape[4],
                                                  ptr(ws), ws.numel(), stream()), "conv3d_wgrad_prepacked")
    return dw


def act_bwd_rowsum_pack8_raw(y, dy, act, slope, ws, nslice, gb_out=None):
    y, dy = f32c(y), f32c(dy)
    N, C = y.shape[0], y.shape[1]
    lib = _lib()
    dz = torch.empty_like(y)
    rows = torch.empty(N * C, dtype=torch.float32, device=y.device)
    check(lib.sg_act_bwd_rowsum_pack8(ptr(y), ptr(dy), ptr(dz), ptr(rows), ptr(ws), N, C, nslice, act, slope, stream()),
          "act_bwd_rowsum_pack8")
    gb = torch.empty(C, dtype=torch.float32, device=y.device) if gb_out is None else gb_out
    check(lib.sg_colsum(ptr(rows), ptr(gb), N, C, C, stream()), "colsum")
    return dz, gb


def conv_wgrad_act_raw(dy, y, x, act, slope, dw_out=None, db_out=None):
    N, Co, OD, OH, OW = dy.shape
    Cx = x.shape[1]
    dw = dw_out if dw_out is not None else torch.empty((Co, Cx, 4, 4, 4), dtype=torch.float32, device=dy.device)
    db = db_out if db_out is not None else torch.empty(Co, dtype=torch.float32, device=dy.device)
    lib = _lib()
    nb = min(lib.sg_conv3d_k4s2p1_wgrad_workspace_bytes(N, Cx, Co, OD, OH, OW), _WGRAD_WS_CAP)
    ws = workspace("splitk", nb, dy.device)
    check(lib.sg_conv3d_k4s2p1_wgrad_act(ptr(dy), ptr(y), ptr(x), ptr(dw), ptr(db), N, Cx, Cx, Cx, Co, 2 * OD, 2 * OH, 2 * OW, act,
                                         slope, ptr(ws), ws.numel(), stream()), "conv3d_wgrad_act")
    return dw, db


def _wgrad_act_served(x, w, y, act):
    lib = _lib()
    N, Cx, Co = x.shape[0], x.shape[1], w.shape[0]
    if not lib.sg_conv3d_k4s2p1_wgrad_act_eligible(N, Cx, Co, y.shape[2], y.shape[3], y.shape[4], act):
        return False
    return lib.sg_conv3d_k4s2p1_wgrad_workspace_bytes(N, Cx, Co, y.shape[2], y.shape[3], y.shape[4]) <= _WGRAD_WS_CAP


def conv_wgrad_halo_raw(dy, x, ct):
    N, Co, OD, OH, OW = dy.shape
    Cx = x.shape[1]
    dw = torch.zeros((Co, ct, 4, 4, 4), dtype=torch.float32, device=dy.device)
    lib = _lib()
    ws = workspace("splitk", lib.sg_conv3d_k4s2p1_wgrad_workspace_bytes(N, Cx, Co, OD, OH, OW), dy.device)
    check(lib.sg_conv3d_k4s2p1_wgrad_impl(ptr(dy), ptr(x), ptr(dw), N, Cx, ct, Cx, Co, 2 * OD, 2 * OH, 2 * OW, ptr(ws),
                                          ws.numel(), 1, stream()), "conv3d_wgrad_impl")
    return dw


def gemm_raw(a, ta, b, tb, bias_j=None, bias_shift=0, act=ACT_NONE, slope=0.0, out=None, a_off=0, b_off=0, M=None,
             N=None, K=None, lda=None, ldb=None, ldc=None, c_off=0):
    lda = a.shape[-1] if lda is None else lda
    ldb = b.shape[-1] if ldb is None else ldb
    if M is None:
        M = a.shape[1] if ta else a.shape[0]
    if K is None:
        K = a.shape[0] if ta else a.shape[1]
    if N is None:
        N = b.shape[0] if tb else b.shape[1]
    sai, sak = (1, lda) if ta else (lda, 1)
    sbk, sbj = (1, ldb) if tb else (ldb, 1)
    if out is None:
        out = torch.empty((M, N), dtype=torch.float32, device=a.device)
    ldc = out.shape[-1] if ldc is None else ldc
    lib = _lib()
    nb = min(lib.sg_gemm_workspace_bytes(M, N), _WGRAD_WS_CAP)
    ws = workspace("splitk", nb, a.device)
    check(lib.sg_gemm(ptr(a) + 4 * a_off, sai, sak, ptr(b) + 4 * b_off, sbk, sbj, ptr(out) + 4 * c_off, ldc, 1, None,
                      ptr(bias_j), bias_shift, M, N, K, act, slope, ptr(ws), ws.numel(), stream()), "gemm")
    return out


def gemm_nt_raw(a, b, out, M, N, K, lda, ldb, ldc, a_off=0, b_off=0, c_off=0):
    lib = _lib()
    ws = workspace("gemm_nt", lib.sg_gemm_nt_workspace_bytes(M, N, K), a.device)
    check(lib.sg_gemm_nt(ptr(a) + 4 * a_off, lda, ptr(b) + 4 * b_off, ldb, ptr(out) + 4 * c_off, ldc, M, N, K, ptr(ws),
                         ws.numel(), stream()), "gemm_nt")
    return out


def act_bwd_raw(y, dy, act, slope):
    dx = torch.empty_like(y)
    check(_lib().sg_act_bwd(ptr(y), ptr(dy), ptr(dx), y.numel(), act, slope, stream()), "act_bwd")
    return dx


def act_bwd_rowsum_raw(y, dy, act, slope, gb_out=None):
    y, dy = f32c(y), f32c(dy)
    N, C = y.shape[0], y.shape[1]
    S = y.numel() // (N * C)
    lib = _lib()
    dz = torch.empty_like(y)
    rows = torch.empty(N * C, dtype=torch.float32, device=y.device)
    check(lib.sg_act_bwd_rowsum(ptr(y), ptr(dy), ptr(dz), ptr(rows), N * C, S, act, slope, stream()), "act_bwd_rowsum")
    gb = torch.empty(C, dtype=torch.float32, device=y.device) if gb_out is None else gb_out
    check(lib.sg_colsum(ptr(rows), ptr(gb), N, C, C, stream()), "colsum")
    return dz, gb


def act_fwd_raw(x, act, slope):
    y = torch.empty_like(x)
    check(_lib().sg_act_fwd(ptr(x), ptr(y), x.numel(), act, slope, stream()), "act_fwd")
    return y


def channel_sum_raw(g, out=None):
    N, C = g.shape[0], g.shape[1]
    S = g.numel() // (N * C)
    lib = _lib()
    if out is None:
        out = torch.empty(C, dtype=torch.float32, device=g.device)
    if S == 1:
        check(lib.sg_colsum(ptr(g), ptr(out), N, C, C, stream()), "colsum")
        return out
    tmp = torch.empty(N * C, dtype=torch.float32, device=g.device)
    check(lib.sg_rowsum(ptr(g), ptr(tmp), N * C, S, S, stream()), "rowsum")
    check(lib.sg_colsum(ptr(tmp), ptr(out), N, C, C, stream()), "colsum")
    return out


class ActBwd(Function):

    @staticmethod
    def forward(ctx, y, dy, act, slope):
        y, dy = f32c(y), f32c(dy)
        ctx.act, ctx.slope = act, slope
        ctx.save_for_backward(y)
        ctx.dy = dy if act in (ACT_TANH, ACT_SIGMOID) else None
        return act_bwd_raw(y, dy, act, slope)

    @staticmethod
    def backward(ctx, ggx):
        (y,) = ctx.saved_tensors
        g_dy = ActBwd.apply(y, ggx, ctx.act, ctx.slope) if ctx.needs_input_grad[1] else None
        g_y = None
        if ctx.needs_input_grad[0] and ctx.act in (ACT_TANH, ACT_SIGMOID):
            dy, ggc = f32c(ctx.dy.detach()), f32c(ggx.detach())
            g_y = torch.empty_like(y)
            check(_lib().sg_act_bwd_dy(ptr(y), ptr(dy), ptr(ggc), ptr(g_y), y.numel(), ctx.act, stream()), "act_bwd_dy")
        return g_y, g_dy, None, None


class Act(Function):

    @staticmethod
    def forward(ctx, x, act, slope):
        x = f32c(x)
        y = act_fwd_raw(x, act, slope)
        ctx.act, ctx.slope = act, slope
        ctx.save_for_backward(y)
        return y

    @staticmethod
    def backward(ctx, gy):
        (y,) = ctx.saved_tensors
        return ActBwd.apply(y, gy, ctx.act, ctx.slope), None, None


class ChannelSum(Function):
    @staticmethod
    def forward(ctx, g):
        g = f32c(g)
        ctx.shape = g.shape
        return channel_sum_raw(g)

    @staticmethod
    def backward(ctx, gg):
        shape = ctx.shape
        view = [1, shape[1]] + [1] * (len(shape) - 2)
        return gg.reshape(view).expand(shape)


class ConvFwd(Function):

    @staticmethod
    def forward(ctx, x, w, b, act, slope):
        x, w = f32c(x), f32c(w)
        y = conv_fwd_raw(x, w, b, act, slope, keep=True)
        ctx.act, ctx.slope, ctx.has_b = act, slope, b is not None
        ctx.save_for_backward(x, w, y if act != ACT_NONE else None, b)
        return y

    @staticmethod
    def backward(ctx, gy):
        x, w, y, b = ctx.saved_tensors
        gb = None
        want_b = ctx.has_b and ctx.needs_input_grad[2]
        plain = not torch.is_grad_enabled()
        if (ctx.act != ACT_NONE and want_b and plain and ctx.needs_input_grad[1] and not ctx.needs_input_grad[0]
                and w.shape[1] == x.shape[1] and _wgrad_act_served(x, w, y, ctx.act)):
            gw, gb = conv_wgrad_act_raw(f32c(gy), y, x, ctx.act, ctx.slope, L.grad_destination(w, w.shape),
                                        L.grad_destination(b, b.shape))
            return None, gw, gb, None, None
        image = None
        if (ctx.act in (ACT_LEAKY, ACT_RELU) and want_b and plain and ctx.needs_input_grad[1] and tuple(y.shape[2:]) == (8, 8, 8)
                and w.shape[1] == x.shape[1] and y.shape[1] % 128 == 0):
            image = _wgrad_dy_image(x.shape[0], x.shape[1], w.shape[0], 8, y.device)
        if image is not None:
            gz, gb = act_bwd_rowsum_pack8_raw(y, gy, ctx.act, ctx.slope, image[0], image[2], L.grad_destination(b, b.shape))
        elif ctx.act != ACT_NONE and want_b and plain and y.shape[2] * y.shape[3] * y.shape[4] >= 512:
            gz, gb = act_bwd_rowsum_raw(y, gy, ctx.act, ctx.slope, L.grad_destination(b, b.shape))
        else:
            gz = ActBwd.apply(y, gy, ctx.act, ctx.slope) if ctx.act != ACT_NONE else gy
        gx = None
        if ctx.needs_input_grad[0]:
            gx = conv_dgrad_raw(f32c(gz), w, None, x.shape[1], keep=True) if plain else ConvDgrad.apply(gz, w, None, x.shape[1], ACT_NONE, 0.0)
        gw = None
        if ctx.needs_input_grad[1]:
            if image is not None:
                gw = conv_wgrad_prepacked_raw(gz, x, w.shape[1], image[0], L.grad_destination(w, w.shape))
            else:
                gw = conv_wgrad_raw(f32c(gz), x, w.shape[1], L.grad_destination(w, w.shape)) if plain else ConvWgrad.apply(gz, x, w.shape[1])
        if want_b and gb is None:
            gb = channel_sum_raw(f32c(gz), L.grad_destination(b, b.shape)) if plain else ChannelSum.apply(gz)
        return gx, gw, gb, None, None


class ConvDgrad(Function):

    @staticmethod
    def forward(ctx, dy, w, b, cin, act, slope, keep=False):
        dy, w = f32c(dy), f32c(w)
        dx = conv_dgrad_raw(dy, w, b, cin, act, slope, keep)
        ctx.act, ctx.slope, ctx.has_b = act, slope, b is not None
        ctx.save_for_backward(dy, w, dx if act != ACT_NONE else None, b)
        return dx

    @staticmethod
    def backward(ctx, gdx):
        dy, w, dx, b = ctx.saved_tensors
        g_b = None
        want_b = ctx.has_b and ctx.needs_input_grad[2]
        plain = not torch.is_grad_enabled()
        if ctx.act != ACT_NONE and want_b and plain and dx.shape[2] * dx.shape[3] * dx.shape[4] >= 512:
            gz, g_b = act_bwd_rowsum_raw(dx, gdx, ctx.act, ctx.slope, L.grad_destination(b, b.shape))
        else:
            gz = ActBwd.apply(dx, gdx, ctx.act, ctx.slope) if ctx.act != ACT_NONE else gdx
        g_dy = ConvFwd.apply(gz, w, None, ACT_NONE, 0.0) if ctx.needs_input_grad[0] else None
        g_w = None
        if ctx.needs_input_grad[1]:
            g_w = conv_wgrad_raw(dy, f32c(gz), w.shape[1], L.grad_destination(w, w.shape)) if plain else ConvWgrad.apply(dy, gz, w.shape[1])
        if want_b and g_b is None:
            g_b = channel_sum_raw(f32c(gz), L.grad_destination(b, b.shape)) if plain else ChannelSum.apply(gz)
        return g_dy, g_w, g_b, None, None, None, None


class ConvWgrad(Function):

    @staticmethod
    def forward(ctx, dy, x, ct):
        dy, x = f32c(dy), f32c(x)
        ctx.save_for_backward(dy, x)
        return conv_wgrad_raw(dy, x, ct)

    @staticmethod
    def backward(ctx, gdw):
        dy, x = ctx.saved_tensors
        g_dy = ConvFwd.apply(x, gdw, None, ACT_NONE, 0.0) if ctx.needs_input_grad[0] else None
        g_x = ConvDgrad.apply(dy, gdw, None, x.shape[1], ACT_NONE, 0.0) if ctx.needs_input_grad[1] else None
        return g_dy, g_x, None


def conv3d_k4s2p1(x, w, b, act=ACT_NONE, slope=0.0):
    return ConvFwd.apply(x, w, b, act, slope)


def conv_transpose3d_k4s2p1(x, w, b, act=ACT_NONE, slope=0.0, out=None):
    if out is not None and not torch.is_grad_enabled():
        return conv_dgrad_raw(f32c(x), f32c(w), b, w.shape[1], act, slope, True, out)
    return ConvDgrad.apply(x, w, b, w.shape[1], act, slope, True)


def convT_to1_pre_eligible(N, C, D, H, W):
    return bool(_lib().sg_convT3d_k4s2p1_to1_pre_eligible(int(N), int(C), int(D), int(H), int(W)))


def convT_to1_pre_served(x, w):
    return (w.shape[1] == 1 and x.dim() == 5 and
            bool(_lib().sg_convT3d_k4s2p1_to1_pre_eligible(x.shape[0], x.shape[1], x.shape[2], x.shape[3], x.shape[4])))


def bn_plan(N, C, S):
    import ctypes
    nsplit, napply = ctypes.c_int(0), ctypes.c_int(0)
    check(L._load_hip().sg_bn_plan(N, C, S, ctypes.addressof(nsplit), ctypes.addressof(napply)), "bn_plan")
    return nsplit.value, napply.value


def bn_train_stats_affine(x, gamma, beta, running_mean, running_var, num_batches_tracked, eps, momentum, groups=1):
    x = f32c(x)
    N, C = x.shape[0], x.shape[1]
    if N % groups:
        raise RuntimeError("bn_train_stats_affine: %d samples in %d groups" % (N, groups))
    S = x.numel() // (N * C)
    lib = _lib()
    mean = torch.empty((groups, C), dtype=torch.float32, device=x.device)
    invstd, scale, shift = torch.empty_like(mean), torch.empty_like(mean), torch.empty_like(mean)
    ws = workspace("bn", groups * lib.sg_bn_workspace_bytes(C), x.device)
    check(lib.sg_bn_train_stats_grouped(ptr(x), ptr(gamma), ptr(beta), ptr(mean), ptr(invstd), ptr(running_mean), ptr(running_var),
                                        ptr(num_batches_tracked), ptr(scale), ptr(shift), groups, N // groups, C, S, eps, momentum,
                                        ptr(ws), ws.numel(), stream()), "bn_train_stats")
    return (scale, shift) if groups > 1 else (scale[0], shift[0])


def bn_train_fwd_grouped_raw(x, gamma, beta, running_mean, running_var, num_batches_tracked, eps, momentum, act, slope, groups):
    x = f32c(x)
    N, C = x.shape[0], x.shape[1]
    if N % groups:
        raise RuntimeError("bn_train_fwd_grouped: %d samples in %d groups" % (N, groups))
    S = x.numel() // (N * C)
    lib = _lib()
    y = torch.empty_like(x)
    mean = torch.empty((groups, C), dtype=torch.float32, device=x.device)
    invstd = torch.empty_like(mean)
    ws = workspace("bn", groups * lib.sg_bn_workspace_bytes(C), x.device)
    check(lib.sg_bn_train_fwd_grouped(ptr(x), ptr(gamma), ptr(beta), ptr(y), ptr(mean), ptr(invstd), ptr(running_mean),
                                      ptr(running_var), ptr(num_batches_tracked), groups, N // groups, C, S, eps, momentum, act,
                                      slope, ptr(ws), ws.numel(), stream()), "bn_train_fwd_grouped")
    return y


def conv_transpose3d_to1_pre_raw(x, scale, shift, in_act, in_slope, w, b, act=ACT_NONE, slope=0.0, out=None, outs=None, form=0):
    x, w = f32c(x), f32c(w)
    N, C, D, H, W = x.shape
    if outs is not None:
        groups = len(outs)
        per = N // groups
        want = (per, 1, 2 * D, 2 * H, 2 * W)
        stride = (outs[1].data_ptr() - outs[0].data_ptr()) // 4 if groups > 1 else per * 8 * D * H * W
        for g, o in enumerate(outs):
            if (tuple(o.shape) != want or o.dtype != torch.float32 or not o.is_contiguous() or o.device != x.device
                    or o.data_ptr() != outs[0].data_ptr() + 4 * stride * g):
                raise RuntimeError("conv_transpose3d_to1_pre: `outs` must be equally spaced contiguous fp32 tensors of shape %s" % (want,))
        if N % groups or tuple(scale.shape) != (groups, C) or stride < per * 8 * D * H * W:
            raise RuntimeError("conv_transpose3d_to1_pre: %d samples, %d groups, scale %s" % (N, groups, tuple(scale.shape)))
        check(_lib().sg_convT3d_k4s2p1_to1_pre_grouped(ptr(x), ptr(w), ptr(b), ptr(outs[0]), ptr(scale), ptr(shift), in_act, in_slope,
                                                       N, C, D, H, W, act, slope, per, stride, stream()), "convT3d_to1_pre_grouped")
        return outs
    shape = (N, 1, 2 * D, 2 * H, 2 * W)
    if out is not None:
        if tuple(out.shape) != shape or out.dtype != torch.float32 or not out.is_contiguous() or out.device != x.device:
            raise RuntimeError("conv_transpose3d_to1_pre: `out` must be a contiguous fp32 tensor of shape %s on %s" % (shape, x.device))
        y = out
    else:
        y = torch.empty(shape, dtype=torch.float32, device=x.device)
    if form:
        args = (ptr(x), ptr(w), ptr(b), ptr(y), ptr(scale), ptr(shift), in_act, in_slope, N, C, D, H, W, act, slope, int(form), stream())
        L.reset_call_state()
        if not x.is_cuda:
            raise RuntimeError("conv_transpose3d_to1_pre: kernel forms exist on the GPU only")
        check(L._load_hip().sg_convT3d_k4s2p1_to1_pre_impl(*args), "convT3d_to1_pre_impl")
        return y
    check(_lib().sg_convT3d_k4s2p1_to1_pre(ptr(x), ptr(w), ptr(b), ptr(y), ptr(scale), ptr(shift), in_act, in_slope, N, C, D, H, W,
                                           act, slope, stream()), "convT3d_to1_pre")
    return y

# ... 2006 lines not shown
```

Measured before the change: 61.86 steps/s.

## Emit activation sign bitmask in first-layer conv forward for backward passes

```diff
diff --git a/include/shapegan_hip.h b/include/shapegan_hip.h
--- a/include/shapegan_hip.h
+++ b/include/shapegan_hip.h
@@ -70,6 +70,20 @@
 int sg_conv3d_k4s2p1_wgrad_act(const float* dy, const float* y, const float* x, float* dw, float* db, int batch, int Cin,
                                int Cin_total, int Cx, int Cout, int ID, int IH, int IW, int act, float slope, void* workspace,
                                size_t workspace_bytes, hipStream_t stream);
+size_t sg_conv3d_k4s2p1_sign_mask_workspace_bytes(int batch, int Cin, int Cout, int OD, int OH, int OW, int act, float slope);
+int sg_conv3d_k4s2p1_fwd_sign_mask(const float* x, const float* w, const float* bias, float* y, void* mask, size_t mask_bytes, int batch,
+                                   int Cin, int Cin_total, int Cx, int Cout, int ID, int IH, int IW, int act, float slope,
+                                   hipStream_t stream);
+int sg_conv3d_k4s2p1_fwd_sign_mask_impl(const float* x, const float* w, const float* bias, float* y, void* mask, size_t mask_bytes,
+                                        int batch, int Cin, int Cin_total, int Cx, int Cout, int ID, int IH, int IW, int act,
+                                        float slope, hipStream_t stream);
+int sg_conv3d_k4s2p1_wgrad_act_mask(const float* dy, const void* mask, size_t mask_bytes, const float* x, float* dw, float* db, int batch,
+                                    int Cin, int Cin_total, int Cx, int Cout, int ID, int IH, int IW, int act, float slope,
+                                    void* workspace, size_t workspace_bytes, hipStream_t stream);
+int sg_conv3d_k4s2p1_wgrad_act_mask_impl(const float* dy, const float* y, const void* mask, size_t mask_bytes, const float* x, float* dw,
+                                         float* db, int batch, int Cin, int Cin_total, int Cx, int Cout, int ID, int IH, int IW, int act,
+                                         float slope, void* workspace, size_t workspace_bytes, hipStream_t stream);
+int sg_act_bwd_mask(const void* mask, const float* dy, float* dx, long n, int act, float slope, hipStream_t stream);
 
 int sg_convT3d_k4s2p1_fwd(const float* x, const float* w, const float* bias, float* y, int batch, int Cin_T, int Cout_T,
                           int ID, int IH, int IW, int act, float slope, void* workspace, size_t workspace_bytes,
diff --git a/shapegan_amd/csrc/conv3d.hip b/shapegan_amd/csrc/conv3d.hip
--- a/shapegan_amd/csrc/conv3d.hip
+++ b/shapegan_amd/csrc/conv3d.hip
@@ -835,6 +835,75 @@
     return SG_OK;
 }
 
+size_t sg_conv3d_k4s2p1_sign_mask_workspace_bytes(int batch, int Cin, int Cout, int OD, int OH, int OW, int act, float slope) {
+    ConvGeom g;
+    if (batch <= 0 || (act != SG_ACT_LEAKY && act != SG_ACT_RELU) || !query_geom(g, Cin, Cout, OD, OH, OW)) return 0;
+    const EdgeFwdPlan ep = edge_fwd_plan(batch, Cin, Cout, g, act, slope);
+    return ep.served && ep.kernel == EdgeFwdKernel::lds_staged ? edge_sign_mask_bytes(batch, g) : 0;
+}
+}
+
+static int fwd_sign_mask_call(const float* x, const float* w, const float* bias, float* y, void* mask, size_t mask_bytes, int batch,
+                              int Cin, int Cin_total, int Cx, int Cout, int ID, int IH, int IW, int act, float slope,
+                              hipStream_t stream, bool forced) {
+    SG_CHECK_ARG(x && w && y && batch > 0 && Cin > 0 && Cin <= Cin_total && Cin <= Cx && Cout > 0);
+    SG_CHECK_ARG((mask || forced) && (((uintptr_t)mask) & 3) == 0);
+    ConvGeom g;
+    if (make_geom(g, ID, IH, IW, Cx, Cout)) SG_FAIL(SG_ERR_ARG, "sg_conv3d_k4s2p1_fwd_sign_mask: spatial dims must be even and >= 2");
+    if (check_sizes(g, batch, "sg_conv3d_k4s2p1_fwd_sign_mask")) return SG_ERR_ARG;
+    const EdgeFwdPlan ep = edge_fwd_plan(batch, Cin, Cout, g, act, slope, forced);
+    if (!ep.served || ep.kernel != EdgeFwdKernel::lds_staged || (mask && act != SG_ACT_LEAKY && act != SG_ACT_RELU))
+        SG_FAIL(SG_ERR_ARG, "sg_conv3d_k4s2p1_fwd_sign_mask: call not served by the LDS-staged one-channel forward "
+                            "(see sg_conv3d_k4s2p1_sign_mask_workspace_bytes)");
+    if (mask && mask_bytes < edge_sign_mask_bytes(batch, g))
+        SG_FAIL(SG_ERR_ARG, "sg_conv3d_k4s2p1_fwd_sign_mask: the mask buffer is smaller than batch * Cout * O^3 / 8 bytes");
+    edge_fwd_launch(ep, x, w, bias, y, batch, Cin_total, Cout, g, act, slope, stream, (uint32_t*)mask);
+    SG_CHECK_LAUNCH();
+    return SG_OK;
+}
+
+static int wgrad_act_mask_call(const float* dy, const float* y, const void* mask, size_t mask_bytes, const float* x, float* dw, float* db,
+                               int batch, int Cin, int Cin_total, int Cx, int Cout, int ID, int IH, int IW, int act, float slope,
+                               void* workspace, size_t workspace_bytes, hipStream_t stream, bool forced) {
+    SG_CHECK_ARG(dy && x && dw && db && batch > 0 && Cin > 0 && Cin <= Cin_total && Cin <= Cx && Cout > 0);
+    SG_CHECK_ARG((mask != nullptr) != (y != nullptr) && (mask || forced) && (((uintptr_t)mask) & 3) == 0);
+    ConvGeom g;
+    if (make_geom(g, ID, IH, IW, Cx, Cout)) SG_FAIL(SG_ERR_ARG, "sg_conv3d_k4s2p1_wgrad_act_mask: spatial dims must be even and >= 2");
+    if (check_sizes(g, batch, "sg_conv3d_k4s2p1_wgrad_act_mask")) return SG_ERR_ARG;
+    const EdgeWgradPlan ep = edge_wgrad_plan(batch, Cin, Cout, g, workspace ? workspace_bytes : 0, act, forced);
+    if (act == SG_ACT_NONE || !ep.served)
+        SG_FAIL(SG_ERR_ARG, "sg_conv3d_k4s2p1_wgrad_act_mask: shape not served (see sg_conv3d_k4s2p1_wgrad_act_eligible) or workspace too small");
+    if (mask && mask_bytes < edge_sign_mask_bytes(batch, g))
+        SG_FAIL(SG_ERR_ARG, "sg_conv3d_k4s2p1_wgrad_act_mask: the mask buffer is smaller than batch * Cout * O^3 / 8 bytes");
+    edge_wgrad_launch(ep, dy, y, x, dw, db, batch, Cin_total, Cout, g, slope, workspace, stream, (const uint32_t*)mask);
+    SG_CHECK_LAUNCH();
+    return SG_OK;
+}
+
+extern "C" {
+int sg_conv3d_k4s2p1_fwd_sign_mask(const float* x, const float* w, const float* bias, float* y, void* mask, size_t mask_bytes, int batch,
+                                   int Cin, int Cin_total, int Cx, int Cout, int ID, int IH, int IW, int act, float slope,
+                                   hipStream_t stream) {
+    return fwd_sign_mask_call(x, w, bias, y, mask, mask_bytes, batch, Cin, Cin_total, Cx, Cout, ID, IH, IW, act, slope, stream, false);
+}
+int sg_conv3d_k4s2p1_fwd_sign_mask_impl(const float* x, const float* w, const float* bias, float* y, void* mask, size_t mask_bytes,
+                                        int batch, int Cin, int Cin_total, int Cx, int Cout, int ID, int IH, int IW, int act,
+                                        float slope, hipStream_t stream) {
+    return fwd_sign_mask_call(x, w, bias, y, mask, mask_bytes, batch, Cin, Cin_total, Cx, Cout, ID, IH, IW, act, slope, stream, true);
+}
+int sg_conv3d_k4s2p1_wgrad_act_mask(const float* dy, const void* mask, size_t mask_bytes, const float* x, float* dw, float* db, int batch,
+                                    int Cin, int Cin_total, int Cx, int Cout, int ID, int IH, int IW, int act, float slope,
+                                    void* workspace, size_t workspace_bytes, hipStream_t stream) {
+    return wgrad_act_mask_call(dy, nullptr, mask, mask_bytes, x, dw, db, batch, Cin, Cin_total, Cx, Cout, ID, IH, IW, act, slope, workspace,
+                               workspace_bytes, stream, false);
+}
+int sg_conv3d_k4s2p1_wgrad_act_mask_impl(const float* dy, const float* y, const void* mask, size_t mask_bytes, const float* x, float* dw,
+                                         float* db, int batch, int Cin, int Cin_total, int Cx, int Cout, int ID, int IH, int IW, int act,
+                                         float slope, void* workspace, size_t workspace_bytes, hipStream_t stream) {
+    return wgrad_act_mask_call(dy, y, mask, mask_bytes, x, dw, db, batch, Cin, Cin_total, Cx, Cout, ID, IH, IW, act, slope, workspace,
+                               workspace_bytes, stream, true);
+}
+
 int sg_conv3d_k4s2p1_wgrad(const float* dy, const float* x, float* dw, int batch, int Cin, int Cin_total, int Cx,
                            int Cout, int ID, int IH, int IW, void* workspace, size_t workspace_bytes,
                            hipStream_t stream) {
diff --git a/shapegan_amd/csrc/conv3d_edge.hip b/shapegan_amd/csrc/conv3d_edge.hip
--- a/shapegan_amd/csrc/conv3d_edge.hip
+++ b/shapegan_amd/csrc/conv3d_edge.hip
@@ -221,9 +221,11 @@
     FastDiv dbpp, dOD;
     int act;
     float slope;
+    uint32_t* mask;
+    long mask_bytes;
 };
 
-template <int NT, int ACT, int IWT>
+template <int NT, int ACT, int IWT, bool MASK = false>
 __global__ void __launch_bounds__(256) conv_fwd_c1_lds_kernel(EdgeFwdLdsArgs a) {
     using G = FwdLds<IWT>;
     constexpr int kWL = 65, kTL = 36;
@@ -314,6 +316,14 @@
 
     float pv[NT][16];
     unsigned yprev = kBufOutside;
+    const __amdgpu_buffer_rsrc_t mres = make_rsrc_bytes(MASK ? a.mask : nullptr, MASK ? a.mask_bytes : 0);
+    unsigned mprev = kBufOutside, mbits[NT], mother[NT], mrow[NT];
+    const unsigned mskip = (MASK && kh2 == 0) ? 0u : kBufOutside;
+#pragma unroll
+    for (int nt = 0; nt < NT; ++nt) {
+        mbits[nt] = mother[nt] = 0u;
+        mrow[nt] = (unsigned)(nt * 32 + r) * (O3 >> 3);
+    }
     auto epilogue_slice = [&](int sl) __attribute__((always_inline)) {
         const int nt = sl >> 3, k = sl & 7;
         if (nt >= NT) return;
@@ -328,9 +338,20 @@
                 for (int i = 0; i < 4; ++i) v[i] = sg_apply_act(v[i], a.act, a.slope);
             }
             *reinterpret_cast<f32x4*>(tw + r * kTL + 8 * k + 4 * kh2) = v;
+            if (MASK) {
+                const unsigned nib = (v[0] > 0.f ? 1u : 0u) | (v[1] > 0.f ? 2u : 0u) | (v[2] > 0.f ? 4u : 0u) | (v[3] > 0.f ? 8u : 0u);
+                mbits[nt] = k == 0 ? nib : (mbits[nt] | (nib << (8 * k)));
+                if (k == 3) {
+                    mbits[nt] <<= 4 * kh2;
+                    mother[nt] = (unsigned)__builtin_amdgcn_ds_bpermute((lane ^ 32) * 4, (int)mbits[nt]);
+                }
+            }
         } else {
             const int i = k - 4;
             const int row = nt * 32 + 8 * i + (lane >> 3);
+            if (MASK && k == 4)
+                __builtin_amdgcn_raw_buffer_store_b32(mbits[nt] | mother[nt], mres,
+                                                      (int)((mprev + mrow[nt]) | mskip | (nt * 32 + r < a.Cout ? 0u : kBufOutside)), 0, 0);
             const f32x4 v = *reinterpret_cast<const f32x4*>(tw + (8 * i + (lane >> 3)) * kTL + 4 * (lane & 7));
             buf_store4(yres, row < a.Cout && !(SG_FWDC1_ABL & 1) ? yprev : kBufOutside, (unsigned)(nt * 32 + 8 * i) * O3 * 4u, v[0], v[1], v[2], v[3]);
         }
@@ -383,8 +404,10 @@
     stage_issue(u + 1, u + 1 < u_end);
     tile(IntTag<0>(), buf, 0);
     yprev = ybase + ylane;
+    mprev = (ybase >> 5) + 8u * wave;
     tile(IntTag<1>(), buf, 1);
     yprev = ybase + ylane + 128u;
+    mprev = (ybase >> 5) + 8u * wave + 4u;
     stage_write(buf ^ 1);
     __syncthreads();
     for (++u; u < u_end; ++u) {
@@ -393,8 +416,10 @@
         stage_issue(u + 1, u + 1 < u_end);
         tile(IntTag<1>(), buf, 0);
         yprev = ybase + ylane;
+        mprev = (ybase >> 5) + 8u * wave;
         tile(IntTag<1>(), buf, 1);
         yprev = ybase + ylane + 128u;
+        mprev = (ybase >> 5) + 8u * wave + 4u;
         stage_write(buf ^ 1);
         __syncthreads();
     }
@@ -413,12 +438,14 @@
     long x_sample;
     int passes_per_sample, total_passes;
     FastDiv dpps, dOW16, dOH;
+    const uint32_t* mask;
+    long mask_bytes;
 };
 
 #ifndef SG_WGRAD_C1_WAVES
 #define SG_WGRAD_C1_WAVES 1
 #endif
-template <int MT, int FUSE>
+template <int MT, int FUSE, bool MASK = false>
 __global__ void __launch_bounds__(256, SG_WGRAD_C1_WAVES) conv_wgrad_c1_kernel(EdgeWgradArgs a) {
     constexpr int kLd = 36;
     constexpr int kStage = MT * 32 * kLd;
@@ -426,7 +453,7 @@
     const int lane = threadIdx.x & 63, wave = threadIdx.x >> 6;
     const int r = lane & 31, kh2 = lane >> 5;
     const __amdgpu_buffer_rsrc_t dres = make_rsrc(a.dy);
-    const __amdgpu_buffer_rsrc_t yres = make_rsrc(FUSE ? a.y : a.dy);
+    const __amdgpu_buffer_rsrc_t yres = MASK ? make_rsrc_bytes(a.mask, a.mask_bytes) : make_rsrc(FUSE ? a.y : a.dy);
     const __amdgpu_buffer_rsrc_t xres = make_rsrc(a.x - ((long)a.IH * a.IW + a.IW + 1));
     const unsigned O3 = (unsigned)(a.OD * a.OH * a.OW);
     float* stage = lds + wave * kStage;
@@ -450,7 +477,8 @@
 
     const int nwaves = gridDim.x * 4;
     f32x4 cv[MT * 4];
-    f32x4 yv[FUSE ? MT * 4 : 1];
+    f32x4 yv[(FUSE && !MASK) ? MT * 4 : 1];
+    unsigned mv[(FUSE && MASK) ? MT * 4 : 1];
     float rs[MT * 4];
 #pragma unroll
     for (int i = 0; i < MT * 4; ++i) rs[i] = 0.f;
@@ -460,6 +488,7 @@
         uint32_t n, pp;
         a.dpps.divmod((uint32_t)(valid ? ps : 0), n, pp);
         const unsigned dbase = (unsigned)((long)n * a.Cy * O3 + pp * 32 + ccol) * 4u;
+        const unsigned mbase = (n * (unsigned)a.Cy * (unsigned)a.passes_per_sample + pp) * 4u;
         unsigned inval = valid ? 0u : kBufOutside;
         asm volatile("" : "+v"(inval));
 #pragma unroll
@@ -467,7 +496,11 @@
             const int co = i * 8 + crow;
             const unsigned off = (co < a.Cout ? dbase + (unsigned)co * O3 * 4u : kBufOutside) | inval;
             cv[i] = buf_load4v(dres, off, 0);
-            if (FUSE) yv[i] = buf_load4v(yres, off, 0);
+            if (FUSE && !MASK) yv[i] = buf_load4v(yres, off, 0);
+            if (FUSE && MASK) {
+                const unsigned moff = (co < a.Cout ? mbase + (unsigned)co * (unsigned)a.passes_per_sample * 4u : kBufOutside) | inval;
+                mv[i] = (unsigned)__builtin_amdgcn_raw_buffer_load_b32(yres, (int)moff, 0, 0);
+            }
         }
     };
     auto plan_x = [&](int ps, bool valid) __attribute__((always_inline)) {
@@ -503,8 +536,10 @@
             const float neg = FUSE == SG_ACT_LEAKY ? a.slope : 0.f;
 #pragma unroll
             for (int i = 0; i < MT * 4; ++i) {
-#pragma unroll
-                for (int j = 0; j < 4; ++j) cv[i][j] = yv[i][j] > 0.f ? cv[i][j] : cv[i][j] * neg;
+                const unsigned bits = MASK ? mv[MASK ? i : 0] >> ccol : 0u;
+#pragma unroll
+                for (int j = 0; j < 4; ++j)
+                    cv[i][j] = (MASK ? ((bits >> j) & 1u) != 0u : yv[MASK ? 0 : i][j] > 0.f) ? cv[i][j] : cv[i][j] * neg;
                 rs[i] += (cv[i][0] + cv[i][1]) + (cv[i][2] + cv[i][3]);
             }
         }
@@ -1241,11 +1276,11 @@
            (size_t)batch * g.Cy * g.O3() * 4 < (size_t)kBufRange;
 }
 
-EdgeFwdPlan edge_fwd_plan(int batch, int Cin, int Cout, const ConvGeom& g, int act, float slope) {
+EdgeFwdPlan edge_fwd_plan(int batch, int Cin, int Cout, const ConvGeom& g, int act, float slope, bool any_batch) {
     EdgeFwdPlan p = EdgeFwdPlan();
     const long O3 = g.O3();
     if (Cin != 1 || Cout > 64 || O3 % 32 != 0) return p;
-    if ((long)batch * O3 < 65536) return p;
+    if (!any_batch && (long)batch * O3 < 65536) return p;
     if (!edge_buffers_in_range(batch, g)) return p;
     p.served = true;
     p.block = 256;
@@ -1312,6 +1347,8 @@
     l.dOD = FastDiv((uint32_t)g.OD);
     l.act = act;
     l.slope = slope;
+    l.mask = nullptr;
+    l.mask_bytes = 0;
     return l;
 }
 
@@ -1327,6 +1364,15 @@
     if (IW == 32) return nt == 2 ? edge_fwd_lds_kernel_act<2, 32>(actk) : edge_fwd_lds_kernel_act<1, 32>(actk);
     return nt == 2 ? edge_fwd_lds_kernel_act<2, 64>(actk) : edge_fwd_lds_kernel_act<1, 64>(actk);
 }
+template <int NT, int IWT>
+static EdgeFwdLdsFn edge_fwd_lds_mask_kernel_act(int actk) {
+    return actk == 1 ? conv_fwd_c1_lds_kernel<NT, 1, IWT, true> : conv_fwd_c1_lds_kernel<NT, 2, IWT, true>;
+}
+static EdgeFwdLdsFn edge_fwd_lds_mask_kernel(int IW, int nt, int actk) {
+    if (IW == 32) return nt == 2 ? edge_fwd_lds_mask_kernel_act<2, 32>(actk) : edge_fwd_lds_mask_kernel_act<1, 32>(actk);
+    return nt == 2 ? edge_fwd_lds_mask_kernel_act<2, 64>(actk) : edge_fwd_lds_mask_kernel_act<1, 64>(actk);
+}
+size_t edge_sign_mask_bytes(int batch, const ConvGeom& g) { return (size_t)batch * g.Cy * (g.O3() / 32) * sizeof(uint32_t); }
 template <int NT>
 static EdgeFwdFn edge_fwd_kernel_act(int actk) {
     if (actk == 0) return conv_fwd_c1_kernel<NT, 0>;
@@ -1335,8 +1381,13 @@
 }
 
 void edge_fwd_launch(const EdgeFwdPlan& p, const float* x, const float* w, const float* bias, float* y, int batch, int Cin_total,
-                     int Cout, const ConvGeom& g, int act, float slope, hipStream_t stream) {
-    if (p.kernel == EdgeFwdKernel::lds_staged)
+                     int Cout, const ConvGeom& g, int act, float slope, hipStream_t stream, uint32_t* mask) {
+    if (p.kernel == EdgeFwdKernel::lds_staged && mask) {
+        EdgeFwdLdsArgs l = edge_fwd_lds_args(p, x, w, bias, y, batch, Cin_total, Cout, g, act, slope);
+        l.mask = mask;
+        l.mask_bytes = (long)edge_sign_mask_bytes(batch, g);
+        hipLaunchKernelGGL(edge_fwd_lds_mask_kernel(g.IW, p.nt, p.actk), p.grid, dim3(p.block), p.lds, stream, l);
+    } else if (p.kernel == EdgeFwdKernel::lds_staged)
         hipLaunchKernelGGL(edge_fwd_lds_kernel(g.IW, p.nt, p.actk), p.grid, dim3(p.block), p.lds, stream,
                            edge_fwd_lds_args(p, x, w, bias, y, batch, Cin_total, Cout, g, act, slope));
     else
@@ -1344,13 +1395,13 @@
                            stream, edge_fwd_args(x, w, bias, y, batch, Cin_total, Cout, g, act, slope));
 }
 
-EdgeWgradPlan edge_wgrad_plan(int batch, int Cin, int Cout, const ConvGeom& g, size_t workspace_bytes, int fuse_act) {
+EdgeWgradPlan edge_wgrad_plan(int batch, int Cin, int Cout, const ConvGeom& g, size_t workspace_bytes, int fuse_act, bool any_batch) {
     EdgeWgradPlan p = EdgeWgradPlan();
     if (Cin != 1 || Cout > 64) return p;
     p.workspace_need = (size_t)512 * kEdgePartial * sizeof(float);
     if (g.OW % 16 != 0) return p;
     if (fuse_act != 0 && fuse_act != SG_ACT_LEAKY && fuse_act != SG_ACT_RELU) return p;
-    if ((long)batch * g.O3() < 65536) return p;
+    if (!any_batch && (long)batch * g.O3() < 65536) return p;
     if (workspace_bytes < p.workspace_need) return p;
     if (!edge_buffers_in_range(batch, g)) return p;
     const int wgs = (int)(batch * (g.O3() / 32) + 3) / 4;
@@ -1383,6 +1434,8 @@
     a.dpps = FastDiv((uint32_t)a.passes_per_sample);
     a.dOW16 = FastDiv((uint32_t)(g.OW / 16));
     a.dOH = FastDiv((uint32_t)g.OH);
+    a.mask = nullptr;
+    a.mask_bytes = 0;
     return a;
 }
 
@@ -1394,10 +1447,23 @@
     return conv_wgrad_c1_kernel<MT, 0>;
 }
 
+template <int MT>
+static EdgeWgradFn edge_wgrad_mask_kernel_fuse(int fuse) {
+    return fuse == SG_ACT_LEAKY ? conv_wgrad_c1_kernel<MT, SG_ACT_LEAKY, true> : conv_wgrad_c1_kernel<MT, SG_ACT_RELU, true>;
+}
+
 void edge_wgrad_launch(const EdgeWgradPlan& p, const float* dy, const float* y, const float* x, float* dw, float* db, int batch,
-                       int Cin_total, int Cout, const ConvGeom& g, float slope, void* workspace, hipStream_t stream) {
-    hipLaunchKernelGGL(p.nt == 2 ? edge_wgrad_kernel_fuse<2>(p.fuse) : edge_wgrad_kernel_fuse<1>(p.fuse), p.grid, dim3(p.block), p.lds,
-                       stream, edge_wgrad_args(dy, p.fuse ? y : nullptr, x, batch, Cout, g, slope, workspace));
+                       int Cin_total, int Cout, const ConvGeom& g, float slope, void* workspace, hipStream_t stream,
+                       const uint32_t* mask) {
+    if (p.fuse && mask) {
+        EdgeWgradArgs a = edge_wgrad_args(dy, nullptr, x, batch, Cout, g, slope, workspace);
+        a.mask = mask;
+        a.mask_bytes = (long)edge_sign_mask_bytes(batch, g);
+        hipLaunchKernelGGL(p.nt == 2 ? edge_wgrad_mask_kernel_fuse<2>(p.fuse) : edge_wgrad_mask_kernel_fuse<1>(p.fuse), p.grid,
+                           dim3(p.block), p.lds, stream, a);
+    } else
+        hipLaunchKernelGGL(p.nt == 2 ? edge_wgrad_kernel_fuse<2>(p.fuse) : edge_wgrad_kernel_fuse<1>(p.fuse), p.grid, dim3(p.block), p.lds,
+                           stream, edge_wgrad_args(dy, p.fuse ? y : nullptr, x, batch, Cout, g, slope, workspace));
     hipLaunchKernelGGL(wgrad_c1_finalize_kernel, dim3(p.fuse ? 260 : 256), dim3(256), 0, stream, (const float*)workspace, dw, (int)p.grid.x,
                        Cout, Cin_total, db);
 }
diff --git a/shapegan_amd/csrc/conv_common.h b/shapegan_amd/csrc/conv_common.h
--- a/shapegan_amd/csrc/conv_common.h
+++ b/shapegan_amd/csrc/conv_common.h
@@ -154,16 +154,19 @@
     int nt, actk;
     int bh, units_per_wg;
 };
-EdgeFwdPlan edge_fwd_plan(int batch, int Cin, int Cout, const ConvGeom& g, int act, float slope);
+EdgeFwdPlan edge_fwd_plan(int batch, int Cin, int Cout, const ConvGeom& g, int act, float slope, bool any_batch = false);
 void edge_fwd_launch(const EdgeFwdPlan& p, const float* x, const float* w, const float* bias, float* y, int batch, int Cin_total,
-                     int Cout, const ConvGeom& g, int act, float slope, hipStream_t stream);
+                     int Cout, const ConvGeom& g, int act, float slope, hipStream_t stream, uint32_t* mask = nullptr);
+size_t edge_sign_mask_bytes(int batch, const ConvGeom& g);
 
 struct EdgeWgradPlan : KernelPlan {
     int nt, fuse;
 };
-EdgeWgradPlan edge_wgrad_plan(int batch, int Cin, int Cout, const ConvGeom& g, size_t workspace_bytes, int fuse_act);
+EdgeWgradPlan edge_wgrad_plan(int batch, int Cin, int Cout, const ConvGeom& g, size_t workspace_bytes, int fuse_act,
+                              bool any_batch = false);
 void edge_wgrad_launch(const EdgeWgradPlan& p, const float* dy, const float* y, const float* x, float* dw, float* db, int batch,
-                       int Cin_total, int Cout, const ConvGeom& g, float slope, void* workspace, hipStream_t stream);
+                       int Cin_total, int Cout, const ConvGeom& g, float slope, void* workspace, hipStream_t stream,
+                       const uint32_t* mask = nullptr);
 
 enum class EdgeDgradKernel { walk_one_pair, walk_all_taps, plane_fused, tap_planes };
 struct EdgeDgradPlan : KernelPlan {
diff --git a/shapegan_amd/csrc/elementwise.hip b/shapegan_amd/csrc/elementwise.hip
--- a/shapegan_amd/csrc/elementwise.hip
+++ b/shapegan_amd/csrc/elementwise.hip
@@ -85,6 +85,28 @@
     }
     for (long e = (n4 << 2) + (long)blockIdx.x * 256 + threadIdx.x; e < n; e += (long)gridDim.x * 256)
         dx[e] = act_grad_from_output(y[e], dy[e], act, slope);
+}
+
+__global__ void __launch_bounds__(256) act_bwd_mask_kernel(const uint32_t* __restrict__ mask, const float* __restrict__ dy,
+                                                           float* __restrict__ dx, long n, int act, float slope) {
+    const long n4 = n >> 2;
+    for (long e = (long)blockIdx.x * 256 + threadIdx.x; e < n4; e += (long)gridDim.x * 256) {
+        const uint32_t bits = mask[e >> 3] >> (4 * (int)(e & 7));
+        const float4 g = reinterpret_cast<const float4*>(dy)[e];
+        float4 v;
+        if (act == SG_ACT_LEAKY) {
+            v.x = (bits & 1u) ? g.x : g.x * slope;
+            v.y = (bits & 2u) ? g.y : g.y * slope;
+            v.z = (bits & 4u) ? g.z : g.z * slope;
+            v.w = (bits & 8u) ? g.w : g.w * slope;
+        } else {
+            v.x = (bits & 1u) ? g.x : 0.f;
+            v.y = (bits & 2u) ? g.y : 0.f;
+            v.z = (bits & 4u) ? g.z : 0.f;
+            v.w = (bits & 8u) ? g.w : 0.f;
+        }
+        reinterpret_cast<float4*>(dx)[e] = v;
+    }
 }
 
 __global__ void __launch_bounds__(256) rmsprop_kernel(float* __restrict__ p, const float* __restrict__ g,
@@ -293,6 +315,13 @@
     SG_CHECK_LAUNCH();
     return SG_OK;
 }
+int sg_act_bwd_mask(const void* mask, const float* dy, float* dx, long n, int act, float slope, hipStream_t stream) {
+    SG_CHECK_ARG(mask && dy && dx && n > 0 && n % 32 == 0 && (act == SG_ACT_LEAKY || act == SG_ACT_RELU));
+    SG_CHECK_ARG((((uintptr_t)mask & 3) | (((uintptr_t)dy | (uintptr_t)dx) & 15)) == 0);
+    hipLaunchKernelGGL(act_bwd_mask_kernel, dim3(ew_grid(n, 4)), dim3(256), 0, stream, (const uint32_t*)mask, dy, dx, n, act, slope);
+    SG_CHECK_LAUNCH();
+    return SG_OK;
+}
 int sg_act_bwd_rowsum(const float* y, const float* dy, float* dx, float* rowsum, long rows, long S, int act, float slope,
                       hipStream_t stream) {
     SG_CHECK_ARG(y && dy && dx && rowsum && rows > 0 && rows < (1L << 31) && S > 0);
diff --git a/shapegan_amd/csrc_cpu/shapegan_cpu.cpp b/shapegan_amd/csrc_cpu/shapegan_cpu.cpp
--- a/shapegan_amd/csrc_cpu/shapegan_cpu.cpp
+++ b/shapegan_amd/csrc_cpu/shapegan_cpu.cpp
@@ -653,6 +653,40 @@
         db[co] = (float)t;
     }
     return sg_conv3d_k4s2p1_wgrad_cpu(dz.data(), x, dw, batch, Cin, Cin_total, Cx, Cout, ID, IH, IW, nullptr, 0, nullptr);
+}
+static std::vector<float> sign_mask_to_y(const void* mask, long n) {
+    const uint32_t* m = (const uint32_t*)mask;
+    std::vector<float> y((size_t)n);
+    for (long e = 0; e < n; ++e) y[e] = ((m[e >> 5] >> (e & 31)) & 1u) ? 1.f : -1.f;
+    return y;
+}
+int sg_conv3d_k4s2p1_fwd_sign_mask_cpu(const float* x, const float* w, const float* bias, float* y, void* mask, size_t mask_bytes,
+                                       int batch, int Cin, int Cin_total, int Cx, int Cout, int ID, int IH, int IW, int act, float slope,
+                                       void*) {
+    const long n = (long)batch * Cout * (ID / 2) * (IH / 2) * (IW / 2);
+    CPU_CHECK(mask && n % 32 == 0 && mask_bytes >= (size_t)(n / 8) && (act == ACT_LEAKY || act == ACT_RELU));
+    const int rc = sg_conv3d_k4s2p1_fwd_cpu(x, w, bias, y, batch, Cin, Cin_total, Cx, Cout, ID, IH, IW, act, slope, nullptr, 0, nullptr);
+    if (rc != SG_OK) return rc;
+    uint32_t* m = (uint32_t*)mask;
+    for (long p = 0; p < n / 32; ++p) {
+        uint32_t word = 0;
+        for (int b = 0; b < 32; ++b) word |= (y[32 * p + b] > 0.f ? 1u : 0u) << b;
+        m[p] = word;
+    }
+    return SG_OK;
+}
+int sg_conv3d_k4s2p1_wgrad_act_mask_cpu(const float* dy, const void* mask, size_t mask_bytes, const float* x, float* dw, float* db,
+                                        int batch, int Cin, int Cin_total, int Cx, int Cout, int ID, int IH, int IW, int act, float slope,
+                                        void*, size_t, void*) {
+    const long n = (long)batch * Cout * (ID / 2) * (IH / 2) * (IW / 2);
+    CPU_CHECK(mask && batch > 0 && Cout > 0 && n % 32 == 0 && mask_bytes >= (size_t)(n / 8) && (act == ACT_LEAKY || act == ACT_RELU));
+    const std::vector<float> y = sign_mask_to_y(mask, n);
+    return sg_conv3d_k4s2p1_wgrad_act_cpu(dy, y.data(), x, dw, db, batch, Cin, Cin_total, Cx, Cout, ID, IH, IW, act, slope, nullptr, 0, nullptr);
+}
+int sg_act_bwd_mask_cpu(const void* mask, const float* dy, float* dx, long n, int act, float slope, void*) {
+    CPU_CHECK(mask && dy && dx && n > 0 && n % 32 == 0 && (act == ACT_LEAKY || act == ACT_RELU));
+    const std::vector<float> y = sign_mask_to_y(mask, n);
+    return sg_act_bwd_cpu(y.data(), dy, dx, n, act, slope, nullptr);
 }
 int sg_act_bwd_dy_cpu(const float* y, const float* dy, const float* ggx, float* out, long n, int act, void*) {
     CPU_CHECK(y && dy && ggx && out && n > 0 && (act == ACT_TANH || act == ACT_SIGMOID));
diff --git a/shapegan_amd/ops.py b/shapegan_amd/ops.py
--- a/shapegan_amd/ops.py
+++ b/shapegan_amd/ops.py
@@ -34,6 +34,33 @@
     check(lib.sg_conv3d_k4s2p1_fwd(ptr(x), ptr(w), ptr(bias), ptr(y), N, Cx, Ct, Cx, Co, D, H, W, act, slope, ptr(ws),
                                    ws.numel() if ws is not None else 0, stream()), "conv3d_fwd")
     return y
+
+
+SIGN_MASK = True
+
+
+def sign_mask_bytes(x, w, act, slope):
+    if not (x.is_cuda and x.dim() == 5 and x.shape[1] == 1 and act in (ACT_LEAKY, ACT_RELU)):
+        return 0
+    N, _, D, H, W = x.shape
+    return L._load_hip().sg_conv3d_k4s2p1_sign_mask_workspace_bytes(N, 1, w.shape[0], D // 2, H // 2, W // 2, act, slope)
+
+
+def conv_fwd_sign_mask_raw(x, w, bias, act, slope, forced=False, want_mask=True, mask_out=None):
+    N, Cx, D, H, W = x.shape
+    Co, Ct = w.shape[0], w.shape[1]
+    ptr(x)
+    L.reset_call_state()
+    y = torch.empty((N, Co, D // 2, H // 2, W // 2), dtype=torch.float32, device=x.device)
+    mask = None
+    if want_mask:
+        mask = mask_out if mask_out is not None else torch.empty((N, Co, (D // 2) * (H // 2) * (W // 2) // 32), dtype=torch.int32,
+                                                                 device=x.device)
+    lib = _lib()
+    fn = lib.sg_conv3d_k4s2p1_fwd_sign_mask_impl if forced else lib.sg_conv3d_k4s2p1_fwd_sign_mask
+    check(fn(ptr(x), ptr(w), ptr(bias), ptr(y), ptr(mask), mask.numel() * 4 if want_mask else 0, N, Cx, Ct, Cx, Co, D, H, W, act, slope,
+             stream()), "conv3d_fwd_sign_mask")
+    return y, mask
 
 
 def conv_fwd_impl_raw(x, w, bias, act, slope, impl, debug=0):
@@ -243,7 +270,7 @@
     return dz, gb
 
 
-def conv_wgrad_act_raw(dy, y, x, act, slope, dw_out=None, db_out=None):
+def conv_wgrad_act_raw(dy, y, x, act, slope, dw_out=None, db_out=None, mask=None):
     N, Co, OD, OH, OW = dy.shape
     Cx = x.shape[1]
     dw = dw_out if dw_out is not None else torch.empty((Co, Cx, 4, 4, 4), dtype=torch.float32, device=dy.device)
@@ -251,8 +278,25 @@
     lib = _lib()
     nb = min(lib.sg_conv3d_k4s2p1_wgrad_workspace_bytes(N, Cx, Co, OD, OH, OW), _WGRAD_WS_CAP)
     ws = workspace("splitk", nb, dy.device)
+    if mask is not None:
+        check(lib.sg_conv3d_k4s2p1_wgrad_act_mask(ptr(dy), ptr(mask), mask.numel() * 4, ptr(x), ptr(dw), ptr(db), N, Cx, Cx, Cx, Co, 2 * OD,
+                                                  2 * OH, 2 * OW, act, slope, ptr(ws), ws.numel(), stream()), "conv3d_wgrad_act_mask")
+        return dw, db
     check(lib.sg_conv3d_k4s2p1_wgrad_act(ptr(dy), ptr(y), ptr(x), ptr(dw), ptr(db), N, Cx, Cx, Cx, Co, 2 * OD, 2 * OH, 2 * OW, act,
                                          slope, ptr(ws), ws.numel(), stream()), "conv3d_wgrad_act")
+    return dw, db
+
+
+def conv_wgrad_act_forced_raw(dy, y, mask, x, act, slope):
+    N, Co, OD, OH, OW = dy.shape
+    Cx = x.shape[1]
+    dw = torch.empty((Co, Cx, 4, 4, 4), dtype=torch.float32, device=dy.device)
+    db = torch.empty(Co, dtype=torch.float32, device=dy.device)
+    lib = _lib()
+    ws = workspace("splitk", lib.sg_conv3d_k4s2p1_wgrad_workspace_bytes(N, Cx, Co, OD, OH, OW), dy.device)
+    check(lib.sg_conv3d_k4s2p1_wgrad_act_mask_impl(ptr(dy), ptr(y), ptr(mask), mask.numel() * 4 if mask is not None else 0, ptr(x), ptr(dw),
+                                                   ptr(db), N, Cx, Cx, Cx, Co, 2 * OD, 2 * OH, 2 * OW, act, slope, ptr(ws), ws.numel(),
+                                                   stream()), "conv3d_wgrad_act_mask_impl")
     return dw, db
 
 
@@ -312,6 +356,12 @@
     return dx
 
 
+def act_bwd_mask_raw(mask, dy, act, slope):
+    dx = torch.empty_like(dy)
+    check(_lib().sg_act_bwd_mask(ptr(mask), ptr(dy), ptr(dx), dy.numel(), act, slope, stream()), "act_bwd_mask")
+    return dx
+
+
 def act_bwd_rowsum_raw(y, dy, act, slope, gb_out=None):
     y, dy = f32c(y), f32c(dy)
     N, C = y.shape[0], y.shape[1]
@@ -349,23 +399,25 @@
 class ActBwd(Function):
 
     @staticmethod
-    def forward(ctx, y, dy, act, slope):
+    def forward(ctx, y, dy, act, slope, mask=None):
         y, dy = f32c(y), f32c(dy)
-        ctx.act, ctx.slope = act, slope
+        ctx.act, ctx.slope, ctx.mask = act, slope, mask
         ctx.save_for_backward(y)
         ctx.dy = dy if act in (ACT_TANH, ACT_SIGMOID) else None
+        if mask is not None and SIGN_MASK:
+            return act_bwd_mask_raw(mask, dy, act, slope)
         return act_bwd_raw(y, dy, act, slope)
 
     @staticmethod
     def backward(ctx, ggx):
         (y,) = ctx.saved_tensors
-        g_dy = ActBwd.apply(y, ggx, ctx.act, ctx.slope) if ctx.needs_input_grad[1] else None
+        g_dy = ActBwd.apply(y, ggx, ctx.act, ctx.slope, ctx.mask) if ctx.needs_input_grad[1] else None
         g_y = None
         if ctx.needs_input_grad[0] and ctx.act in (ACT_TANH, ACT_SIGMOID):
             dy, ggc = f32c(ctx.dy.detach()), f32c(ggx.detach())
             g_y = torch.empty_like(y)
             check(_lib().sg_act_bwd_dy(ptr(y), ptr(dy), ptr(ggc), ptr(g_y), y.numel(), ctx.act, stream()), "act_bwd_dy")
-        return g_y, g_dy, None, None
+        return g_y, g_dy, None, None, None
 
 
 class Act(Function):
@@ -403,7 +455,11 @@
     @staticmethod
     def forward(ctx, x, w, b, act, slope):
         x, w = f32c(x), f32c(w)
-        y = conv_fwd_raw(x, w, b, act, slope, keep=True)
+        ctx.mask = None
+        if SIGN_MASK and any(ctx.needs_input_grad[:3]) and sign_mask_bytes(x, w, act, slope):
+            y, ctx.mask = conv_fwd_sign_mask_raw(x, w, b, act, slope)
+        else:
+            y = conv_fwd_raw(x, w, b, act, slope, keep=True)
         ctx.act, ctx.slope, ctx.has_b = act, slope, b is not None
         ctx.save_for_backward(x, w, y if act != ACT_NONE else None, b)
         return y
@@ -417,7 +473,7 @@
         if (ctx.act != ACT_NONE and want_b and plain and ctx.needs_input_grad[1] and not ctx.needs_input_grad[0]
                 and w.shape[1] == x.shape[1] and _wgrad_act_served(x, w, y, ctx.act)):
             gw, gb = conv_wgrad_act_raw(f32c(gy), y, x, ctx.act, ctx.slope, L.grad_destination(w, w.shape),
-                                        L.grad_destination(b, b.shape))
+                                        L.grad_destination(b, b.shape), mask=ctx.mask if SIGN_MASK else None)
             return None, gw, gb, None, None
         image = None
         if (ctx.act in (ACT_LEAKY, ACT_RELU) and want_b and plain and ctx.needs_input_grad[1] and tuple(y.shape[2:]) == (8, 8, 8)
@@ -428,7 +484,7 @@
         elif ctx.act != ACT_NONE and want_b and plain and y.shape[2] * y.shape[3] * y.shape[4] >= 512:
             gz, gb = act_bwd_rowsum_raw(y, gy, ctx.act, ctx.slope, L.grad_destination(b, b.shape))
         else:
-            gz = ActBwd.apply(y, gy, ctx.act, ctx.slope) if ctx.act != ACT_NONE else gy
+            gz = ActBwd.apply(y, gy, ctx.act, ctx.slope, ctx.mask) if ctx.act != ACT_NONE else gy
         gx = None
         if ctx.needs_input_grad[0]:
             gx = conv_dgrad_raw(f32c(gz), w, None, x.shape[1], keep=True) if plain else ConvDgrad.apply(gz, w, None, x.shape[1], ACT_NONE, 0.0)
```

Measured after the change: 62.24 steps/s, median of 6. About the same (+0.6%).
